# Krual-T/OutfitX

Hardware: AMD Instinct MI355X
Metric: outfits/sec CP forward (8-item sets, 224^2, bf16) (higher is better)
Workload: dtype f16

## Files before the change

### include/ofx.h

```cpp
#ifndef OFX_H
#define OFX_H
#include <stddef.h>
#include <stdint.h>

#ifdef __cplusplus
extern "C" {
#endif

#define OFX_ABI_VERSION 6

enum { OFX_OK = 0, OFX_EINVAL = -1, OFX_ESHAPE = -2, OFX_EHIP = -3, OFX_EWORKSPACE = -4, OFX_ESTATE = -5 };
enum ofx_dtype { OFX_F32 = 0, OFX_BF16 = 1, OFX_F16 = 2 };
enum ofx_act { OFX_ACT_NONE = 0, OFX_ACT_QUICK_GELU = 1, OFX_ACT_GELU = 2, OFX_ACT_MISH = 3, OFX_ACT_MISH_GRAD = 4 };
enum ofx_precision { OFX_PREC_BF16 = 0, OFX_PREC_F16 = 1, OFX_PREC_BF16X3 = 2, OFX_PREC_F16W2 = 3 };
enum ofx_out_kind { OFX_OUT_F32 = 0, OFX_OUT_OP = 1, OFX_OUT_SPLIT3 = 2 };

typedef struct ofx_handle ofx_handle;
typedef void* ofx_stream;

const char* ofx_last_error(void);
int ofx_abi_version(void);

typedef struct ofx_model_desc {
    int d_model, n_head, d_ffn, n_layers, max_items;
// ... 36 lines not shown
int ofx_clip_text_fwd_shared(ofx_handle* h, const int64_t* ids, const int64_t* attn_mask, const int* lengths_host,
                             int N, int T, float* emb, int emb_ld, int emb_col, int normalize, int shared_first, void* ws,
                             size_t ws_bytes, ofx_stream stream);

int ofx_fitb_argmin(const float* y_hat, const float* cand, int B, int C, int D, int64_t* idx, float* dist,
                    ofx_stream stream);
int ofx_fitb_argmin_indexed(const float* table, int ld, long long n_table, const int* cand_index, const float* y_hat, int B, int C, int D,
                            const int64_t* answer, int64_t* idx, float* dist, int* n_correct, ofx_stream stream);
int ofx_l2_topk(ofx_handle* h, const float* Q, const float* P, int nq, int np, int D, int k, int64_t index_base,
                int64_t* idx, float* dist, void* ws, size_t ws_bytes, ofx_stream stream);
size_t ofx_l2_topk_grouped_ws(int nq, int np, int max_group_rows);
int ofx_l2_topk_grouped(ofx_handle* h, const float* Q, const float* P, int nq, int np, int D, int k, const int* panels, int n_panels,
                        int max_group_rows, const int64_t* gt, int64_t* idx, float* dist, int* gt_pos, void* ws, size_t ws_bytes,
                        ofx_stream stream);
int ofx_topk_merge(const int64_t* idx_in, const float* dist_in, int parts, int nq, int k, int64_t* idx, float* dist,
                   ofx_stream stream);

size_t ofx_clip_preprocess_ws(const int* heights, const int* widths, int N, int channels, int size);
int ofx_clip_preprocess(const uint8_t* src, const long long* offsets, const int* heights, const int* widths, int N, int channels, int size,
                        const float* mean, const float* stdv, float* out, void* ws, size_t ws_bytes, ofx_stream stream);
int ofx_clip_preprocess_patches(const uint8_t* src, const long long* offsets, const int* heights, const int* widths, int N, int channels, int size,
                                int patch, const float* mean, const float* stdv, void* patches, int op_dtype, void* ws, size_t ws_bytes,
                                ofx_stream stream);
int ofx_patchify(const float* pixels, void* out, int N, int img, int patch, int op_dtype, ofx_stream stream);
size_t ofx_vit_b32_u8_ws_bytes(ofx_handle* h, const int* heights, const int* widths, int N, int channels);
int ofx_vit_b32_fwd_u8(ofx_handle* h, const uint8_t* src, const long long* offsets, const int* heights, const int* widths, int N, int channels,
                       const float* mean, const float* stdv, float* emb, int emb_ld, int emb_col, int normalize, void* ws, size_t ws_bytes,
                       ofx_stream stream);

int ofx_set_encoder_fwd_indexed(ofx_handle* h, const float* table, int ld, long long n_table, const int* item_index, const int* cu_items,
                                const float* prefix, int prefix_stride, int B, int max_len, float* out_row0, void* ws, size_t ws_bytes,
                                ofx_stream stream);

size_t ofx_cp_train_tape_bytes(ofx_handle* h, int B, int L);
size_t ofx_cp_train_ws_bytes(ofx_handle* h, int B, int L);
size_t ofx_cp_train_grad_floats(ofx_handle* h, size_t* offsets, int n_offsets);
int ofx_cp_train_fwd(ofx_handle* h, const float* x, const uint8_t* pad_mask, int B, int L, float* logits, void* tape, size_t tape_bytes,
                     void* ws, size_t ws_bytes, float dropout_p, unsigned seed, ofx_stream stream);
int ofx_cp_train_bwd(ofx_handle* h, void* tape, size_t tape_bytes, const float* dlogits, int B, int L, float* grads, size_t grad_floats,
                     void* ws, size_t ws_bytes, float dropout_p, unsigned seed, ofx_stream stream);
int ofx_cp_train_fwd_indexed(ofx_handle* h, const float* table, int ld, long long n_table, const int* item_index, const int* cu_items,
                             int B, int max_len, float* logits, void* tape, size_t tape_bytes, void* ws, size_t ws_bytes,
                             float dropout_p, unsigned seed, ofx_stream stream);
int ofx_cir_train_fwd(ofx_handle* h, const float* x, const uint8_t* pad_mask, const float* table, int ld, long long n_table,
                      const int* item_index, const int* cu_items, const float* target_text, int B, int L, float* y, void* tape,
                      size_t tape_bytes, void* ws, size_t ws_bytes, float dropout_p, unsigned seed, ofx_stream stream);
int ofx_cir_train_bwd(ofx_handle* h, void* tape, size_t tape_bytes, const float* dy, int B, int L, float* grads, size_t grad_floats,
                      void* ws, size_t ws_bytes, float dropout_p, unsigned seed, ofx_stream stream);
int ofx_cp_train_bwd_into(ofx_handle* h, void* tape, size_t tape_bytes, const float* dlogits, int B, int L, float* const* grad_ptrs,
                          int n_ptrs, int accumulate, void* ws, size_t ws_bytes, float dropout_p, unsigned seed, ofx_stream stream);
int ofx_cir_train_bwd_into(ofx_handle* h, void* tape, size_t tape_bytes, const float* dy, int B, int L, float* const* grad_ptrs,
                           int n_ptrs, int accumulate, void* ws, size_t ws_bytes, float dropout_p, unsigned seed, ofx_stream stream);
int ofx_train_arm_layer_events(ofx_handle* h, void* const* events, int n);
int ofx_dropout_mask(float dropout_p, unsigned seed, int site, int rows, int cols, float* out, ofx_stream stream);
int ofx_focal_loss(const float* logits, const float* labels, int B, float alpha, float gamma, float upstream, float* loss, float* dlogits,
                   ofx_stream stream);
int ofx_focal_loss_ex(const float* logits, const float* labels, int B, float alpha, float gamma, float upstream, int reduction, float* loss,
                      float* per_elem, float* dlogits, ofx_stream stream);
size_t ofx_set_rank_loss_ws_bytes(int B, int K, int D);
int ofx_set_rank_loss(const float* y, const float* y_hat, const float* neg, const uint8_t* neg_mask, int B, int K, int D, float margin,
                      float upstream, float* loss, float* dy_hat, float* d_pos, float* d_neg, void* ws, size_t ws_bytes, ofx_stream stream);
int ofx_set_rank_loss_indexed(const float* table, int ld, long long n_table, const int* pos_index, const int* neg_index, const float* y_hat,
                              int B, int K, int D, float margin, float upstream, float* loss, float* dy_hat, float* d_pos, float* d_neg,
                              void* ws, size_t ws_bytes, ofx_stream stream);

int ofx_cir_sample_batch(const int* outfit_cu, const int* outfit_rows, int n_outfits, int n_outfit_rows, const int* pos_cu, const int* pos_slots,
                         int n_pos_slots, const int* pool_cu, const int* pool_rows, int n_pools, int n_pool_rows, const int* row_pool,
                         const int* row_slot, int n_table, const int* outfit_ids, int B, unsigned seed, unsigned draw, int K, int max_len,
                         int* item_index, int* cu_seqlens, int* target_item_index, int* neg_items_index, ofx_stream stream);

typedef struct ofx_opt_segment { float* param; long long offset; long long numel; } ofx_opt_segment;
size_t ofx_adamw_step_ws_bytes(long long n_arena);
int ofx_adamw_step(const ofx_opt_segment* segments, int n_segments, float* grad, float* exp_avg, float* exp_avg_sq, long long n_arena,
                   float* step, double lr, double beta1, double beta2, double eps, double weight_decay, double max_norm, double grad_scale,
                   float* grad_norm, int* skipped, void* ws, size_t ws_bytes, ofx_stream stream);

void ofx_profile_enable(int on);
int ofx_profile_read(double* ms, double* flops, long long* launches);
typedef struct ofx_prof_record { int cat, M, N, K, kind, kmul; float ms; double flops; double bytes; } ofx_prof_record;
int ofx_profile_records(ofx_prof_record* out, int cap);

int ofx_tune(int knob, int value);
unsigned ofx_config_generation(void);
int ofx_profile_enabled(void);
int ofx_stream_create_low_priority(int device, ofx_stream* out);
int ofx_stream_destroy(ofx_stream stream);

int ofx_gemm(const void* A, const void* W, void* C, const float* bias, const float* resid, int M, int N, int K,
             int lda, int ldc, int ldr, int act, int out_kind, int op_dtype, ofx_stream stream);
int ofx_gemm_w2(const void* A, const void* W2, void* C, const float* bias, const float* resid, int M, int N, int K,
                int lda, int ldc, int ldr, int act, int out_kind, int op_dtype, ofx_stream stream);
int ofx_gemm_x3(const void* A3, const void* W3, void* C, const float* bias, const float* resid, int M, int N, int K,
                int lda, int ldc, int ldr, int act, int out_kind, int op_dtype, ofx_stream stream);
int ofx_pack_lo8(const void* W2, void* W8, void* scale8, int N, int K, ofx_stream stream);
int ofx_gemm_w2f8(const void* A, const void* W2, const void* W8, const void* scale8, void* C, const float* bias, const float* resid, int M, int N, int K,
                  int lda, int ldc, int ldr, int act, int out_kind, ofx_stream stream);
int ofx_gemm_w2f8_fold(const void* A, const void* W2, const void* W8, const void* scale8, void* C, const float* bias, const float* row_stat, const float* col_sum,
                       int M, int N, int K, int lda, int ldc, int act, ofx_stream stream);
size_t ofx_gemm_tn_ws(int M, int N, int K);
int ofx_gemm_tn(const void* A, int lda, const void* B, int ldb, float* C, int ldc, int M, int N, int K, const int* k_dev,
                void* slab, size_t slab_bytes, int op_dtype, ofx_stream stream);
size_t ofx_gemm_splitk_ws(int M, int N, int K);
int ofx_gemm_splitk(const void* A, const void* W, void* C, const float* bias, const float* resid, int M, int N, int K,
                    int lda, int ldc, int ldr, int act, int out_kind, int op_dtype, void* slab, size_t slab_bytes, ofx_stream stream);
int ofx_gemm_train(const void* A, const void* W, void* C, const float* bias, const float* resid, float* aux_out, int M, const int* m_dev,
                   int N, int K, int lda, int ldc, int ldr, int act, int out_kind, float dropout_p, unsigned seed, int site, int op_dtype,
                   void* slab, size_t slab_bytes, ofx_stream stream);
int ofx_gemm_tn_into(const void* A, int lda, const void* B, int ldb, float* C, int ldc, int M, int N, int K, const int* k_dev,
                     int m_valid, int n_valid, int accumulate, void* slab, size_t slab_bytes, int op_dtype, ofx_stream stream);
int ofx_transpose_cast(const float* src, void* dst, int R, int C, int ldd, void* row_dst, int ld_row, int op_dtype, ofx_stream stream);
size_t ofx_layernorm_bwd_ws(int D);
int ofx_layernorm_bwd(const float* dy, const float* x, const float* stats, const float* gamma, const float* add, const int* add_map,
                      float* dx, void* dx_op, float* dgamma, float* dbeta, float* dcols, int M, const int* m_dev, int D, float dropout_p,
                      unsigned seed, int site, int accumulate, int op_dtype, void* ws, size_t ws_bytes, ofx_stream stream);
size_t ofx_colsum_ws(int C);
int ofx_colsum(const void* x, int x_kind, int ld, const int* gather, const float* row_scale, float* out0, float* out1, float* out2, int seg,
               int C, int valid, int M, const int* m_dev, int accumulate, int op_dtype, void* ws, size_t ws_bytes, ofx_stream stream);
int ofx_head_bwd(const float* dlogits, const float* w, const int* cu, float* dX, void* dXb, float* db, int B, int D, float dropout_p,
                 unsigned seed, int head_site, int below_site, int accumulate, int op_dtype, ofx_stream stream);
int ofx_gemm_fold_producer(const void* A, const void* W, const void* W8, const void* scale8, void* xb, void* xlo, float* stat_part, const float* bias,
                           const float* resid, int M, int N, int K, int lda, int ldr, int act, int w_form, int op_dtype, ofx_stream stream);
int ofx_gemm_fold(const void* A, const void* W, void* C, const float* bias, const float* row_stat, int stat_ld, const float* col_sum, int M, int N, int K,
                  int lda, int ldc, int act, int w_form, int op_dtype, ofx_stream stream);
int ofx_stats_finalize(const float* stat_part, int slots, int W, float eps, float* stat, int rows, ofx_stream stream);
int ofx_row_stats_cast(const float* x, void* xb, void* xlo, float* stat, int rows, int W, float eps, int op_dtype, ofx_stream stream);
int ofx_fold_pack(const float* w, const float* gamma, const float* beta, const float* bias, void* wf, float* col_sum, float* bias_f, int N, int K, int split,
                  int op_dtype, ofx_stream stream);
int ofx_vit_embed_ln(const float* patch_out, const float* cls, const float* pos, const float* gamma, const float* beta, float* x, void* xb, void* xlo,
                     float* stat, int N, int S, int D, float eps, int op_dtype, ofx_stream stream);
int ofx_gather_hilo(const void* hi, const void* lo, const int* idx, float* dst, int rows, int W, int op_dtype, ofx_stream stream);
int ofx_layernorm(const float* x, const int* row_idx, const float* gamma, const float* beta, void* y, int rows,
                  int D, int ldy, int out_kind, int op_dtype, float eps, ofx_stream stream);
int ofx_attention(const void* qkv, void* out, const int64_t* key_mask, int nseq, int seq_len, int n_head, int ld,
                  int ldo, int k_off, int v_off, int mask_ld, int causal, float scale, int op_dtype, ofx_stream stream);
int ofx_attention_ex(const void* qkv, void* out, const int64_t* key_mask, int nseq, int seq_len, int n_head, int ld, int ldo, int k_off,
                     int v_off, int mask_ld, int causal, int only_row0, int split3_w, float scale, int op_dtype, ofx_stream stream);
int ofx_set_attention(const float* qkv, void* out, const int* cu_seqlens, int nseq, int n_head, int D, int ldo,
                      int out_kind, int max_len, int only_row0, float scale, int op_dtype, ofx_stream stream);
int ofx_set_attention_slabs(const float* slabs, size_t plane_floats, int splits, const float* bias, void* out, const int* cu_seqlens, int nseq,
                            int n_head, int D, int ldo, int out_kind, int max_len, int only_row0, float scale, int op_dtype, ofx_stream stream);
int ofx_splitk_reduce_ln(const float* slab, size_t plane_floats, int splits, const float* bias, const float* resid, int ldr, float* x, int ldx,
                         const float* gamma, const float* beta, void* y, int ldy, int out_kind, float eps, int rows, const int* m_dev, int D,
                         int op_dtype, ofx_stream stream);
int ofx_attention_varlen(const void* qkv, void* out, const int* cu_seqlens, int nseq, int max_len, int n_head, int ld, int ldo, int k_off,
                         int v_off, int only_row0, float scale, float dropout_p, unsigned seed, int site, int op_dtype, ofx_stream stream);
int ofx_set_attention_op(const void* qkv, void* out, const int* cu_seqlens, int nseq, int n_head, int D, int ldo, int out_kind, int max_len,
                         int only_row0, float scale, float dropout_p, unsigned seed, int site, int op_dtype, ofx_stream stream);
int ofx_set_attention_bwd(const void* qkv, const float* d_o, void* dqkv, const int* cu_seqlens, int nseq, int n_head, int D, int max_len,
                          int only_row0, float scale, float dropout_p, unsigned seed, int site, int mfma, int op_dtype, ofx_stream stream);
int ofx_fused_qkv_attention(const void* X, const void* Wqkv, const float* bias, const float* row_stat, const float* col_sum, void* out,
                            int nseq, int seq_len, int width, int n_head, int ldx, int ldo, float scale, int op_dtype, ofx_stream stream);
int ofx_fused_qkv_attention_w2(const void* X, const void* Wqkv2, const float* bias, const float* row_stat, const float* col_sum, void* out,
                               int nseq, int seq_len, int width, int n_head, int ldx, int ldo, float scale, int op_dtype, ofx_stream stream);
int ofx_attention_f32(const float* qkv, void* out, const int64_t* key_mask, int nseq, int seq_len, int n_head, int D, int ldo, int out_kind,
                      int mask_ld, int causal, float scale, int op_dtype, ofx_stream stream);
int ofx_convert(const float* src, void* dst, int rows, int cols, int mode, int op_dtype, ofx_stream stream);

#ifdef __cplusplus
}
#endif
#endif
```

### outfitx_amd/_lib.py

```python
from __future__ import annotations

import ctypes as C
import os

_HERE = os.path.dirname(os.path.abspath(__file__))
LIB_PATH = os.environ.get("OFX_LIB") or os.path.join(_HERE, "libofx_hip.so")

OFX_OK = 0
ABI_VERSION = 6
F32, BF16, F16 = 0, 1, 2
ACT_NONE, ACT_QUICK_GELU, ACT_GELU, ACT_MISH = 0, 1, 2, 3
PREC_BF16, PREC_F16, PREC_BF16X3 = 0, 1, 2
OUT_F32, OUT_OP, OUT_SPLIT3 = 0, 1, 2
OP_SET_ENCODER, OP_VIT, OP_TEXT, OP_TOPK = 0, 1, 2, 3
PREC_F16W2 = 3
PRECISIONS = {"bf16": PREC_BF16, "f16": PREC_F16, "fp16": PREC_F16, "bf16x3": PREC_BF16X3, "f16w2": PREC_F16W2}
W2_PATCH, W2_QKV, W2_OUT, W2_FC1, W2_FC2 = 1, 2, 4, 8, 16
TOWER_SCHEMES = {
    "bf16": (PREC_BF16, 0, 0, 0, 0), "f16": (PREC_F16, 0, 0, 0, 0), "fp16": (PREC_F16, 0, 0, 0, 0),
    "f16w2": (PREC_F16, W2_PATCH | W2_OUT | W2_FC2, 1, 1, 0),
    "bf16w2": (PREC_BF16, W2_PATCH | W2_OUT | W2_FC2, 1, 1, 0),
    "f16w2q": (PREC_F16, W2_PATCH | W2_QKV | W2_OUT | W2_FC2, 1, 1, 0),
    "f16w2f": (PREC_F16, W2_PATCH | W2_OUT | W2_FC1 | W2_FC2, 1, 1, 0),
    "f16w2x": (PREC_F16, W2_PATCH | W2_QKV | W2_OUT | W2_FC1 | W2_FC2, 1, 1, 0),
    "f16x3": (PREC_F16, W2_PATCH, 1, 1, 1), "bf16x3": (PREC_BF16, W2_PATCH, 1, 1, 1),
}
SCHEME_ALIASES = {"f16w2h": "f16w2x@qkv=0-5"}
DEFAULT_TOWER_PRECISION = "f16w2x"


def _layer_bits(spec: str) -> int:
    m = 0
    for part in spec.split(","):
        a, _, b = part.partition("-")
        for l in range(int(a), int(b or a) + 1):
            m |= 1 << l
    return m


def tower_scheme(name: str) -> dict:
    name = SCHEME_ALIASES.get(name, name)
    base, _, opts = name.partition("@")
    if base not in TOWER_SCHEMES:
        raise ValueError(f"unknown tower_precision {name!r}; one of {sorted(list(TOWER_SCHEMES) + list(SCHEME_ALIASES))} [+ '@txt=w2;qkv=<layers>;fc1=<layers>']")
    prec, mask, txt_x3, proj_x3, vit_x3 = TOWER_SCHEMES[base]
    d = {"tower_precision": prec, "vit_w2_mask": mask, "txt_x3": txt_x3, "proj_x3": proj_x3, "vit_x3": vit_x3,
         "txt_w2_mask": 0, "vit_w2_qkv_layers": 0, "vit_w2_fc1_layers": 0, "vit_w2_out_layers": 0, "vit_w2_fc2_layers": 0}
    for o in filter(None, opts.split(";")):
        k, _, v = o.partition("=")
        try:
            if k == "txt" and v == "w2":
                d["txt_x3"], d["txt_w2_mask"] = 0, W2_QKV | W2_OUT | W2_FC1 | W2_FC2
            elif k in ("qkv", "fc1", "out", "fc2"):
                bits = _layer_bits(v) if v not in ("", "none") else 0
                if bits == 0:
                    d["vit_w2_mask"] &= ~{"qkv": W2_QKV, "fc1": W2_FC1, "out": W2_OUT, "fc2": W2_FC2}[k]
                d[f"vit_w2_{k}_layers"] = bits
            else:
                raise ValueError
        except ValueError:
            raise ValueError(f"tower_precision {name!r}: bad option {o!r} (txt=w2 | qkv= / fc1= / out= / fc2=<layers>, layers like 0-5,8 or none)") from None
    return d
ACTS = {"none": ACT_NONE, "quick_gelu": ACT_QUICK_GELU, "gelu": ACT_GELU, "mish": ACT_MISH}


class OfxError(RuntimeError):
    pass


class ModelDesc(C.Structure):
    _fields_ = [(n, C.c_int) for n in (
        "d_model", "n_head", "d_ffn", "n_layers", "max_items", "outfit_act", "outfit_precision",
        "vit_width", "vit_layers", "vit_heads", "vit_mlp", "vit_patch", "vit_image", "vit_act",
        "txt_width", "txt_layers", "txt_heads", "txt_mlp", "txt_vocab", "txt_max_pos", "txt_act", "txt_eos_id",
        "proj_dim", "tower_precision")] + [("ln_eps", C.c_float)] + [(n, C.c_int) for n in ("vit_w2_mask", "txt_x3", "proj_x3", "vit_x3", "txt_w2_mask", "vit_w2_qkv_layers", "vit_w2_fc1_layers", "vit_w2_out_layers", "vit_w2_fc2_layers")]


class OptSegment(C.Structure):
    _fields_ = [("param", C.c_void_p), ("offset", C.c_longlong), ("numel", C.c_longlong)]


class ProfRecord(C.Structure):
    _fields_ = [("cat", C.c_int), ("M", C.c_int), ("N", C.c_int), ("K", C.c_int), ("kind", C.c_int), ("kmul", C.c_int), ("ms", C.c_float), ("flops", C.c_double), ("bytes", C.c_double)]


_vp, _i, _f, _sz, _i64 = C.c_void_p, C.c_int, C.c_float, C.c_size_t, C.c_int64

SIGNATURES = {
    "ofx_last_error": (C.c_char_p, []),
    "ofx_abi_version": (_i, []),
    "ofx_stream_create_low_priority": (_i, [_i, C.POINTER(_vp)]),
    "ofx_stream_destroy": (_i, [_vp]),
    "ofx_default_desc": (None, [C.POINTER(ModelDesc)]),
    "ofx_create": (_vp, [_i, C.POINTER(ModelDesc)]),
    "ofx_destroy": (None, [_vp]),
    "ofx_pack_outfit_weights": (_i, [_vp, C.POINTER(_vp), _i, _vp]),
    "ofx_pack_vision_weights": (_i, [_vp, C.POINTER(_vp), _i, _vp]),
    "ofx_pack_text_weights": (_i, [_vp, C.POINTER(_vp), _i, _vp]),
    "ofx_workspace_bytes": (_sz, [_vp, _i, _i, _i]),
    "ofx_set_encoder_fwd": (_i, [_vp, _vp, _vp, _vp, _i, _i, _i, _vp, _vp, _sz, _vp]),
    "ofx_cp_head": (_i, [_vp, _vp, _i, _vp, _vp]),
    "ofx_cir_head": (_i, [_vp, _vp, _i, _vp, _vp, _sz, _vp]),
    "ofx_cir_prefix": (_i, [_vp, _vp, _i, _vp, _vp]),
    "ofx_vit_b32_fwd": (_i, [_vp, _vp, _i, _vp, _i, _i, _i, _vp, _sz, _vp]),
    "ofx_clip_text_fwd": (_i, [_vp, _vp, _vp, C.POINTER(_i), _i, _i, _vp, _i, _i, _i, _vp, _sz, _vp]),
    "ofx_clip_text_fwd_shared": (_i, [_vp, _vp, _vp, C.POINTER(_i), _i, _i, _vp, _i, _i, _i, _i, _vp, _sz, _vp]),
    "ofx_fitb_argmin": (_i, [_vp, _vp, _i, _i, _i, _vp, _vp, _vp]),
    "ofx_fitb_argmin_indexed": (_i, [_vp, _i, C.c_longlong, _vp, _vp, _i, _i, _i, _vp, _vp, _vp, _vp, _vp]),
    "ofx_l2_topk": (_i, [_vp, _vp, _vp, _i, _i, _i, _i, _i64, _vp, _vp, _vp, _sz, _vp]),
    "ofx_l2_topk_grouped_ws": (_sz, [_i, _i, _i]),
    "ofx_l2_topk_grouped": (_i, [_vp, _vp, _vp, _i, _i, _i, _i, _vp, _i, _i, _vp, _vp, _vp, _vp, _vp, _sz, _vp]),
    "ofx_topk_merge": (_i, [_vp, _vp, _i, _i, _i, _vp, _vp, _vp]),
    "ofx_clip_preprocess_ws": (_sz, [_vp, _vp, _i, _i, _i]),
    "ofx_clip_preprocess": (_i, [_vp, _vp, _vp, _vp, _i, _i, _i, _vp, _vp, _vp, _vp, _sz, _vp]),
    "ofx_clip_preprocess_patches": (_i, [_vp, _vp, _vp, _vp, _i, _i, _i, _i, _vp, _vp, _vp, _i, _vp, _sz, _vp]),
    "ofx_patchify": (_i, [_vp, _vp, _i, _i, _i, _i, _vp]),
    "ofx_vit_b32_u8_ws_bytes": (_sz, [_vp, _vp, _vp, _i, _i]),
    "ofx_vit_b32_fwd_u8": (_i, [_vp, _vp, _vp, _vp, _vp, _i, _i, _vp, _vp, _vp, _i, _i, _i, _vp, _sz, _vp]),
    "ofx_set_encoder_fwd_indexed": (_i, [_vp, _vp, _i, C.c_longlong, _vp, _vp, _vp, _i, _i, _i, _vp, _vp, _sz, _vp]),
    "ofx_cp_train_fwd_indexed": (_i, [_vp, _vp, _i, C.c_longlong, _vp, _vp, _i, _i, _vp, _vp, _sz, _vp, _sz, _f, C.c_uint, _vp]),
    "ofx_cp_train_tape_bytes": (_sz, [_vp, _i, _i]),
    "ofx_cp_train_ws_bytes": (_sz, [_vp, _i, _i]),
    "ofx_cp_train_grad_floats": (_sz, [_vp, C.POINTER(_sz), _i]),
    "ofx_cp_train_fwd": (_i, [_vp, _vp, _vp, _i, _i, _vp, _vp, _sz, _vp, _sz, _f, C.c_uint, _vp]),
    "ofx_cp_train_bwd": (_i, [_vp, _vp, _sz, _vp, _i, _i, _vp, _sz, _vp, _sz, _f, C.c_uint, _vp]),
    "ofx_cir_train_fwd": (_i, [_vp, _vp, _vp, _vp, _i, C.c_longlong, _vp, _vp, _vp, _i, _i, _vp, _vp, _sz, _vp, _sz, _f, C.c_uint, _vp]),
    "ofx_cir_train_bwd": (_i, [_vp, _vp, _sz, _vp, _i, _i, _vp, _sz, _vp, _sz, _f, C.c_uint, _vp]),
    "ofx_cp_train_bwd_into": (_i, [_vp, _vp, _sz, _vp, _i, _i, C.POINTER(_vp), _i, _i, _vp, _sz, _f, C.c_uint, _vp]),
    "ofx_cir_train_bwd_into": (_i, [_vp, _vp, _sz, _vp, _i, _i, C.POINTER(_vp), _i, _i, _vp, _sz, _f, C.c_uint, _vp]),
    "ofx_train_arm_layer_events": (_i, [_vp, C.POINTER(_vp), _i]),
    "ofx_dropout_mask": (_i, [_f, C.c_uint, _i, _i, _i, _vp, _vp]),
    "ofx_focal_loss": (_i, [_vp, _vp, _i, _f, _f, _f, _vp, _vp, _vp]),
    "ofx_focal_loss_ex": (_i, [_vp, _vp, _i, _f, _f, _f, _i, _vp, _vp, _vp, _vp]),
    "ofx_set_rank_loss_ws_bytes": (_sz, [_i, _i, _i]),
    "ofx_set_rank_loss": (_i, [_vp, _vp, _vp, _vp, _i, _i, _i, _f, _f, _vp, _vp, _vp, _vp, _vp, _sz, _vp]),
    "ofx_set_rank_loss_indexed": (_i, [_vp, _i, C.c_longlong, _vp, _vp, _vp, _i, _i, _i, _f, _f, _vp, _vp, _vp, _vp, _vp, _sz, _vp]),
    "ofx_cir_sample_batch": (_i, [_vp, _vp, _i, _i, _vp, _vp, _i, _vp, _vp, _i, _i, _vp, _vp, _i, _vp, _i, C.c_uint, C.c_uint, _i, _i, _vp, _vp, _vp, _vp, _vp]),
    "ofx_adamw_step_ws_bytes": (_sz, [C.c_longlong]),
    "ofx_adamw_step": (_i, [_vp, _i, _vp, _vp, _vp, C.c_longlong, _vp] + [C.c_double] * 7 + [_vp, _vp, _vp, _sz, _vp]),
    "ofx_profile_enable": (None, [_i]),
    "ofx_profile_read": (_i, [C.POINTER(C.c_double), C.POINTER(C.c_double), C.POINTER(C.c_longlong)]),
    "ofx_profile_records": (_i, [C.POINTER(ProfRecord), _i]),
    "ofx_tune": (_i, [_i, _i]),
    "ofx_config_generation": (C.c_uint, []),
    "ofx_profile_enabled": (_i, []),
    "ofx_gemm": (_i, [_vp, _vp, _vp, _vp, _vp, _i, _i, _i, _i, _i, _i, _i, _i, _i, _vp]),
    "ofx_gemm_w2": (_i, [_vp, _vp, _vp, _vp, _vp, _i, _i, _i, _i, _i, _i, _i, _i, _i, _vp]),
    "ofx_gemm_x3": (_i, [_vp, _vp, _vp, _vp, _vp, _i, _i, _i, _i, _i, _i, _i, _i, _i, _vp]),
    "ofx_pack_lo8": (_i, [_vp, _vp, _vp, _i, _i, _vp]),
    "ofx_gemm_w2f8": (_i, [_vp, _vp, _vp, _vp, _vp, _vp, _vp, _i, _i, _i, _i, _i, _i, _i, _i, _vp]),
    "ofx_gemm_w2f8_fold": (_i, [_vp, _vp, _vp, _vp, _vp, _vp, _vp, _vp, _i, _i, _i, _i, _i, _i, _vp]),
    "ofx_gemm_tn_ws": (_sz, [_i, _i, _i]),
    "ofx_gemm_tn": (_i, [_vp, _i, _vp, _i, _vp, _i, _i, _i, _i, _vp, _vp, _sz, _i, _vp]),
    "ofx_gemm_splitk_ws": (_sz, [_i, _i, _i]),
    "ofx_gemm_splitk": (_i, [_vp, _vp, _vp, _vp, _vp, _i, _i, _i, _i, _i, _i, _i, _i, _i, _vp, _sz, _vp]),
    "ofx_gemm_train": (_i, [_vp, _vp, _vp, _vp, _vp, _vp, _i, _vp, _i, _i, _i, _i, _i, _i, _i, _f, C.c_uint, _i, _i, _vp, _sz, _vp]),
    "ofx_gemm_tn_into": (_i, [_vp, _i, _vp, _i, _vp, _i, _i, _i, _i, _vp, _i, _i, _i, _vp, _sz, _i, _vp]),
    "ofx_transpose_cast": (_i, [_vp, _vp, _i, _i, _i, _vp, _i, _i, _vp]),
    "ofx_layernorm_bwd_ws": (_sz, [_i]),
    "ofx_layernorm_bwd": (_i, [_vp] * 11 + [_i, _vp, _i, _f, C.c_uint, _i, _i, _i, _vp, _sz, _vp]),
    "ofx_colsum_ws": (_sz, [_i]),
    "ofx_colsum": (_i, [_vp, _i, _i, _vp, _vp, _vp, _vp, _vp, _i, _i, _i, _i, _vp, _i, _i, _vp, _sz, _vp]),
    "ofx_head_bwd": (_i, [_vp, _vp, _vp, _vp, _vp, _vp, _i, _i, _f, C.c_uint, _i, _i, _i, _i, _vp]),
    "ofx_gemm_fold_producer": (_i, [_vp] * 9 + [_i] * 8 + [_vp]),
    "ofx_gemm_fold": (_i, [_vp, _vp, _vp, _vp, _vp, _i, _vp, _i, _i, _i, _i, _i, _i, _i, _i, _vp]),
    "ofx_stats_finalize": (_i, [_vp, _i, _i, _f, _vp, _i, _vp]),
    "ofx_row_stats_cast": (_i, [_vp, _vp, _vp, _vp, _i, _i, _f, _i, _vp]),
    "ofx_fold_pack": (_i, [_vp] * 7 + [_i, _i, _i, _i, _vp]),
    "ofx_vit_embed_ln": (_i, [_vp] * 9 + [_i, _i, _i, _f, _i, _vp]),
    "ofx_gather_hilo": (_i, [_vp, _vp, _vp, _vp, _i, _i, _i, _vp]),
    "ofx_layernorm": (_i, [_vp, _vp, _vp, _vp, _vp, _i, _i, _i, _i, _i, _f, _vp]),
    "ofx_attention": (_i, [_vp, _vp, _vp, _i, _i, _i, _i, _i, _i, _i, _i, _i, _f, _i, _vp]),
    "ofx_attention_ex": (_i, [_vp, _vp, _vp, _i, _i, _i, _i, _i, _i, _i, _i, _i, _i, _i, _f, _i, _vp]),
    "ofx_set_attention_slabs": (_i, [_vp, _sz, _i, _vp, _vp, _vp, _i, _i, _i, _i, _i, _i, _i, _f, _i, _vp]),
    "ofx_splitk_reduce_ln": (_i, [_vp, _sz, _i, _vp, _vp, _i, _vp, _i, _vp, _vp, _vp, _i, _i, _f, _i, _vp, _i, _i, _vp]),
    "ofx_fused_qkv_attention": (_i, [_vp, _vp, _vp, _vp, _vp, _vp, _i, _i, _i, _i, _i, _i, _f, _i, _vp]),
    "ofx_fused_qkv_attention_w2": (_i, [_vp, _vp, _vp, _vp, _vp, _vp, _i, _i, _i, _i, _i, _i, _f, _i, _vp]),
    "ofx_set_attention": (_i, [_vp, _vp, _vp, _i, _i, _i, _i, _i, _i, _i, _f, _i, _vp]),
    "ofx_attention_varlen": (_i, [_vp, _vp, _vp, _i, _i, _i, _i, _i, _i, _i, _i, _f, _f, C.c_uint, _i, _i, _vp]),
    "ofx_set_attention_op": (_i, [_vp, _vp, _vp, _i, _i, _i, _i, _i, _i, _i, _f, _f, C.c_uint, _i, _i, _vp]),
    "ofx_set_attention_bwd": (_i, [_vp, _vp, _vp, _vp, _i, _i, _i, _i, _i, _f, _f, C.c_uint, _i, _i, _i, _vp]),
    "ofx_attention_f32": (_i, [_vp, _vp, _vp, _i, _i, _i, _i, _i, _i, _i, _i, _f, _i, _vp]),
    "ofx_convert": (_i, [_vp, _vp, _i, _i, _i, _i, _vp]),
}

_lib = None


def load() -> C.CDLL:
    global _lib
    if _lib is not None:
        return _lib
    if not os.path.exists(LIB_PATH):
        raise OfxError(f"{LIB_PATH} not found: build it with `make` (or __graft_entry__.build()); "
                       "outfitx_amd has no CPU/PyTorch fallback for the scoring path")
    lib = C.CDLL(LIB_PATH)
    for name, (res, args) in SIGNATURES.items():
        fn = getattr(lib, name)
        fn.restype, fn.argtypes = res, args
    if lib.ofx_abi_version() != ABI_VERSION:
        raise OfxError("libofx_hip.so ABI version mismatch; rebuild")
    for kv in filter(None, os.environ.get("OFX_TUNE", "").split(",")):
        knob, _, val = kv.partition(":")
        if lib.ofx_tune(int(knob), int(val)) != OFX_OK:
            raise OfxError(f"OFX_TUNE: ofx_tune({knob}, {val}) was refused")
    _lib = lib
    return lib


def check(rc: int, what: str = "") -> None:
    if rc != OFX_OK:
        msg = load().ofx_last_error()
        raise OfxError(f"{what or 'ofx call'} failed (code {rc}): {msg.decode() if msg else ''}")


def default_desc() -> ModelDesc:
    d = ModelDesc()
    load().ofx_default_desc(C.byref(d))
    return d
```

### outfitx_amd/csrc/api.hip

```cpp
#include <stdarg.h>
#include <string.h>

#include <algorithm>
#include <vector>
#include <mutex>
#include <cstring>

#include "ofx_weights.h"

static thread_local char g_err[512] = "";
void ofx_set_error(const char* fmt, ...) {
    va_list ap;
    va_start(ap, fmt);
    vsnprintf(g_err, sizeof(g_err), fmt, ap);
    va_end(ap);
}
extern "C" const char* ofx_last_error(void) { return g_err; }
extern "C" int ofx_abi_version(void) { return OFX_ABI_VERSION; }
extern "C" int ofx_stream_create_low_priority(int device, ofx_stream* out) {
    OFX_REQUIRE(out, OFX_EINVAL, "stream_create_low_priority: NULL argument");
    int prev = 0, least = 0, greatest = 0;
    OFX_HIP(hipGetDevice(&prev));
    OFX_HIP(hipSetDevice(device));
    hipStream_t s = nullptr;
// ... 340 lines not shown
    size_t r = carve_clip(b, (size_t)n * Tc, n, d.txt_width, d.txt_mlp, d.proj_dim, 0, 0, w, h->txt_x3 ? 3 : 1, h->txt_x3 ? 3 : (h->txt_w2_mask ? 2 : 1), true);
    return align_up(r, 256);
}
constexpr int VIT_CHUNK_MAX = 2048;
}

extern "C" size_t ofx_workspace_bytes(ofx_handle* h, int op, int n, int len) {
    if (!h || n <= 0) return 0;
    switch (op) {
        case OFX_OP_SET_ENCODER: { Bump b(nullptr, ~(size_t)0); return align_up(carve_set(h, b, n, len, nullptr), 256); }
        case OFX_OP_VIT: return vit_bytes(h, std::min(n, VIT_CHUNK_MAX), nullptr, nullptr, ~(size_t)0);
        case OFX_OP_TEXT: return txt_bytes(h, n, len, nullptr, nullptr, ~(size_t)0);
        case OFX_OP_TOPK: return ofx_l2_topk_ws(n, len);
        default: return 0;
    }
}

int g_set_fuse = 3;
int g_train_mfma_attn = 1;

struct SetInput {
    const float* x = nullptr; const uint8_t* pad_mask = nullptr;
    const float* table = nullptr; int ld = 0; long long n_table = 0; const int* item_index = nullptr; const int* cu_items = nullptr;
};
static SetInput dense_set(const float* x, const uint8_t* pad_mask) { SetInput in; in.x = x; in.pad_mask = pad_mask; return in; }
static SetInput indexed_set(const float* table, int ld, long long n_table, const int* item_index, const int* cu_items) {
    SetInput in; in.table = table; in.ld = ld; in.n_table = n_table; in.item_index = item_index; in.cu_items = cu_items;
    return in;
}
static int build_set(const ofx_handle* h, const SetInput& in, const float* prefix, int prefix_stride, int* cu, float* X, int B, int L, hipStream_t s) {
    const int D = h->d.d_model;
    if (in.table) return ofx_launch_set_build_indexed(in.table, in.ld, in.n_table, in.item_index, in.cu_items, prefix, prefix_stride, cu, X, B, D, s);
    return ofx_launch_set_build(in.x, in.pad_mask, prefix, prefix_stride, cu, X, B, L, D, s);
}
static int set_encoder_core(ofx_handle* h, const SetInput& in, const float* prefix, int prefix_stride, int B, int L, float* out_row0, void* ws,
                            size_t ws_bytes, hipStream_t s);
static float set_attn_scale(const ofx_model_desc& d) { return 1.0f / sqrtf((float)(d.d_model / d.n_head)); }
static bool ln_bwd_d_ok(int D);
static bool train_shape_ok(const ofx_model_desc& d) { return d.d_model == d.n_head * 64 && ln_bwd_d_ok(d.d_model); }
#define OFX_REQUIRE_TRAIN_SHAPE(h, who) \
    OFX_REQUIRE(!(h) || train_shape_ok((h)->d), OFX_ESHAPE, who ": training needs heads of 64 and d_model in {512, 768, 1024} (d_model=%d, n_head=%d scores only)", (h)->d.d_model, (h)->d.n_head)

extern "C" int ofx_set_encoder_fwd(ofx_handle* h, const float* x, const uint8_t* pad_mask, const float* prefix,
                                   int prefix_stride, int B, int L, float* out_row0, void* ws, size_t ws_bytes,
                                   ofx_stream stream) {
    OFX_REQUIRE(h && h->out_ready, OFX_ESTATE, "set_encoder_fwd: outfit weights not packed");
    OFX_REQUIRE(B > 0 && L >= 0 && L <= 63, OFX_ESHAPE, "set_encoder_fwd: B=%d L=%d (L must be in [0,63])", B, L);
    OFX_REQUIRE((x || L == 0) && (pad_mask || L == 0) && out_row0 && ws, OFX_EINVAL, "set_encoder_fwd: NULL argument");
    return set_encoder_core(h, dense_set(x, pad_mask), prefix, prefix_stride, B, L, out_row0, ws, ws_bytes, (hipStream_t)stream);
}
extern "C" int ofx_set_encoder_fwd_indexed(ofx_handle* h, const float* table, int ld, long long n_table, const int* item_index, const int* cu_items,
                                           const float* prefix, int prefix_stride, int B, int max_len, float* out_row0, void* ws, size_t ws_bytes,
                                           ofx_stream stream) {
    OFX_REQUIRE(h && h->out_ready, OFX_ESTATE, "set_encoder_fwd_indexed: outfit weights not packed");
    OFX_REQUIRE(B > 0 && max_len >= 0 && max_len <= 63, OFX_ESHAPE, "set_encoder_fwd_indexed: B=%d max_len=%d (must be in [0,63])", B, max_len);
    OFX_REQUIRE(table && item_index && cu_items && out_row0 && ws && n_table > 0, OFX_EINVAL, "set_encoder_fwd_indexed: NULL argument");
    return set_encoder_core(h, indexed_set(table, ld, n_table, item_index, cu_items), prefix, prefix_stride, B, max_len, out_row0, ws, ws_bytes, (hipStream_t)stream);
}
static int set_encoder_core(ofx_handle* h, const SetInput& in, const float* prefix, int prefix_stride, int B, int L, float* out_row0, void* ws,
                            size_t ws_bytes, hipStream_t s) {
    const ofx_model_desc& d = h->d;
    Bump bump(ws, ws_bytes);
    SetWs w;
    carve_set(h, bump, B, L, &w);
    OFX_REQUIRE(bump.ok, OFX_EWORKSPACE, "set_encoder_fwd: workspace %zu < %zu bytes", ws_bytes, bump.off);
    const int D = d.d_model, km = a_kmul(h->ot_form), Fp = h->ot_ffn_pad, dt = h->ot_dtype, M = B * (L + 1);
    const int okind = km == 3 ? OFX_OUT_SPLIT3 : OFX_OUT_OP;
    const float scale = set_attn_scale(d);
    auto slab_gemm = [&](const PackedGemm& c, int K) { GemmArgs g{}; use_gemm(g, c, K); g.slab = w.slab; g.slab_bytes = w.slab_bytes; return g; };
    if (!prefix) { prefix = h->outfit_token; prefix_stride = 0; }
    TRY(build_set(h, in, prefix, prefix_stride, w.cu, w.X, B, L, s));
    const int* m_dev = w.cu + B;
    const bool fuse_att = (g_set_fuse & 1) != 0 && L + 1 <= 32, fuse = (g_set_fuse & 2) != 0;
    bool ln1_done = false;
    for (int l = 0; l < d.n_layers; ++l) {
        const OutfitLayer& Ly = h->ol[l];
        const bool last = l + 1 == d.n_layers;
        if (!ln1_done) {
            LnArgs ln{w.X, nullptr, Ly.g1, Ly.be1, w.H, M, D, km * D, okind, d.ln_eps};
            TRY(ofx_launch_layernorm_dev(ln, m_dev, dt, s));
        }
        ln1_done = false;
        GemmArgs g1 = slab_gemm(Ly.in, D);
        g1.A = w.H; g1.C = w.QKV; g1.m_dev = m_dev; g1.M = M; g1.N = 3 * D; g1.ldc = 3 * D;
        const bool mfma_attn = h->ot_form == W_PLAIN && g_train_mfma_attn && D == d.n_head * 64;
        g1.out_kind = mfma_attn ? OFX_OUT_OP : OFX_OUT_F32;
        int qkv_splits = 1;
        if (fuse_att && !mfma_attn) g1.defer_splits = &qkv_splits;
        TRY(ofx_launch_gemm(g1, dt, s));
        if (mfma_attn) {
            AttnArgs at{w.QKV, w.H, nullptr, B, L + 1, d.n_head, 3 * D, D, D, 2 * D, 0, 0, scale};
            at.cu_seqlens = w.cu; at.only_row0 = last ? 1 : 0;
            TRY(ofx_launch_attention_mfma(at, dt, s));
        } else {
            SetAttnArgs sa{w.QKV, w.H, w.cu, B, d.n_head, D, km * D, okind, L + 1, last ? 1 : 0, scale};
            if (qkv_splits > 1) { sa.qkv = w.slab; sa.splits = qkv_splits; sa.plane = (size_t)M * 3 * D; sa.bias = g1.bias; }
            TRY(ofx_launch_set_attention(sa, dt, s));
        }
        float* X = w.X; char* H = w.H; char* U = w.U; int Ml = M; const int* md = m_dev;
        if (last) {
            TRY(ofx_launch_gather_rows(w.H, w.cu, w.HP, B, km * D * 2, km * D * 2, s));
            TRY(ofx_launch_gather_rows(w.X, w.cu, out_row0, B, D * 4, D * 4, s));
            X = out_row0; H = w.HP; U = w.UP; Ml = B; md = nullptr;
        }
        GemmArgs g2 = slab_gemm(Ly.out, D);
        g2.A = H; g2.C = X; g2.resid = X; g2.m_dev = md; g2.M = Ml; g2.N = D; g2.ldc = D; g2.ldr = D; g2.out_kind = OFX_OUT_F32;
        bool ln2_done = false;
        if (fuse) { g2.ln_gamma = Ly.g2; g2.ln_beta = Ly.be2; g2.ln_out = H; g2.ln_ld = km * D; g2.ln_kind = okind; g2.ln_eps = d.ln_eps; g2.ln_done = &ln2_done; }
        TRY(ofx_launch_gemm(g2, dt, s));
        if (!ln2_done) {
            LnArgs ln2{X, nullptr, Ly.g2, Ly.be2, H, Ml, D, km * D, okind, d.ln_eps};
            TRY(ofx_launch_layernorm_dev(ln2, md, dt, s));
        }
        GemmArgs g3 = slab_gemm(Ly.l1, D);
        g3.A = H; g3.C = U; g3.m_dev = md; g3.M = Ml; g3.N = Fp; g3.ldc = km * Fp; g3.act = d.outfit_act; g3.out_kind = okind;
        TRY(ofx_launch_gemm(g3, dt, s));
        GemmArgs g4 = slab_gemm(Ly.l2, Fp);
        g4.A = U; g4.C = X; g4.resid = X; g4.m_dev = md; g4.M = Ml; g4.N = D; g4.ldc = D; g4.ldr = D; g4.out_kind = OFX_OUT_F32;
        if (fuse && !last) {
            const OutfitLayer& Nx = h->ol[l + 1];
            g4.ln_gamma = Nx.g1; g4.ln_beta = Nx.be1; g4.ln_out = w.H; g4.ln_ld = km * D; g4.ln_kind = okind; g4.ln_eps = d.ln_eps; g4.ln_done = &ln1_done;
        }
        TRY(ofx_launch_gemm(g4, dt, s));
    }
    return OFX_OK;
}

extern "C" int ofx_cp_head(ofx_handle* h, const float* row0, int B, float* logits, ofx_stream stream) {
    OFX_REQUIRE(h && h->out_ready, OFX_ESTATE, "cp_head: outfit weights not packed");
    OFX_REQUIRE(row0 && logits && B > 0, OFX_EINVAL, "cp_head: bad argument");
    return ofx_launch_cp_head(row0, h->cp_w, h->cp_b, logits, B, h->d.d_model, (hipStream_t)stream);
}

extern "C" int ofx_cir_head(ofx_handle* h, const float* row0, int B, float* emb, void* ws, size_t ws_bytes, ofx_stream stream) {
    OFX_REQUIRE(h && h->out_ready, OFX_ESTATE, "cir_head: outfit weights not packed");
    OFX_REQUIRE(row0 && emb && B > 0 && ws, OFX_EINVAL, "cir_head: bad argument");
    const int D = h->d.d_model, km = a_kmul(h->ot_form);
    OFX_REQUIRE(ws_bytes >= (size_t)B * km * D * 2, OFX_EWORKSPACE, "cir_head: workspace too small");
    hipStream_t s = (hipStream_t)stream;
    TRY(ofx_launch_pack_rows(row0, ws, B, B, D, D, D, km == 3 ? 1 : 0, h->ot_dtype, s));
    GemmArgs g{};
    use_cir_head(g, *h);
    g.A = ws; g.C = emb; g.M = B; g.N = D; g.ldc = D; g.out_kind = OFX_OUT_F32;
    return ofx_launch_gemm(g, h->ot_dtype, s);
}

extern "C" int ofx_cir_prefix(ofx_handle* h, const float* txt, int B, float* out, ofx_stream stream) {
    OFX_REQUIRE(h && h->out_ready, OFX_ESTATE, "cir_prefix: outfit weights not packed");
    OFX_REQUIRE(txt && out && B > 0, OFX_EINVAL, "cir_prefix: bad argument");
    return ofx_launch_cir_prefix(h->tgt_img_emb, txt, out, B, h->d.d_model, (hipStream_t)stream);
}

int g_fuse_qkv = 1;
int g_x3_vit_f32_attn = 0;
int g_prune_q = 1;

static int clip_layer(const ClipLayer& L, const ClipWs& w, int rows, int nseq, int S, int W, int MLP, int heads, int act,
                      float eps, int causal, const int64_t* key_mask, int mask_ld, int dt, const int* pool_idx, hipStream_t s, bool pool_first) {
    const bool fused = (g_fuse_qkv & (L.qkv.form == W_SPLIT ? 2 : 1)) && !pool_idx && !causal && !key_mask && S >= 33 && S <= 64 && (256 / S - 1) * S + 64 - 256 <= 16;
    if (fused) {
        TRY(ofx_launch_fused_qkv_attn(w.XB, L.qkv.w, L.qkv.bias, w.S, L.qkv.col_sum, w.H, nseq, S, W, heads, W, W, 0.125f, dt, s, L.qkv.form == W_SPLIT));
    } else {
        GemmArgs g1{}; g1.A = w.XB; g1.C = w.QKV; g1.row_stat = w.S; g1.M = rows; g1.N = 3 * W;
        g1.ldc = 3 * W; g1.act = OFX_ACT_NONE; g1.out_kind = OFX_OUT_OP;
        use_gemm(g1, L.qkv, W);
        const bool prune = pool_idx && pool_first && g_prune_q;
        if (prune) {
            GemmArgs kv = g1;
            kv.W = (const char*)g1.W + (size_t)W * g1.K * 2; kv.bias = g1.bias + W; kv.col_sum = g1.col_sum + W; kv.C = (char*)w.QKV + (size_t)W * 2; kv.N = 2 * W;
            if (g1.W8) { kv.W8 = (const char*)g1.W8 + (size_t)W * W; kv.w8_scale = (const char*)g1.w8_scale + W; }
            TRY(ofx_launch_gemm(kv, dt, s));
            GemmArgs q = g1;
            q.M = nseq; q.N = W; q.lda = S * W; q.ldc = S * 3 * W; q.stat_ld = S;
            TRY(ofx_launch_gemm(q, dt, s));
        } else
            TRY(ofx_launch_gemm(g1, dt, s));
        AttnArgs at{w.QKV, w.H, key_mask, nseq, S, heads, 3 * W, W, W, 2 * W, mask_ld, causal, 0.125f};
        at.only_row0 = prune ? 1 : 0;
        TRY(ofx_launch_attention_mfma(at, dt, s));
    }
    char* H = w.H; char* U = w.U; int M = rows;
    if (pool_idx) {
        TRY(ofx_launch_gather_rows(w.H, pool_idx, w.HP, nseq, W * 2, W * 2, s));
        TRY(ofx_launch_gather_hilo(w.XB, w.XLO, pool_idx, w.XP, nseq, W, dt, s));
        H = w.HP; U = w.UP; M = nseq;
    }
    auto to_stream = [&](GemmArgs& g) {
        g.M = M; g.N = W; g.ldc = W; g.ldr = W; g.act = OFX_ACT_NONE;
        if (pool_idx) { g.C = w.XP; g.resid = w.XP; g.out_kind = OFX_OUT_F32; g.slab = w.slab; g.slab_bytes = w.slab_bytes; }
        else { g.C = w.XB; g.xb_out = w.XB; g.xlo = w.XLO; g.stat_part = w.P; g.out_kind = OFX_OUT_OP; }
    };
    GemmArgs g2{}; g2.A = H;
    use_gemm(g2, L.o, W); to_stream(g2);
    TRY(ofx_launch_gemm(g2, dt, s));
    GemmArgs g3{}; g3.C = U; g3.M = M; g3.N = MLP; g3.ldc = MLP; g3.act = act; g3.out_kind = OFX_OUT_OP;
    if (pool_idx) {
        LnArgs ln2{w.XP, nullptr, L.g2, L.be2, H, M, W, W, OFX_OUT_OP, eps};
        TRY(ofx_launch_layernorm(ln2, dt, s));
        g3.A = H; g3.slab = w.slab; g3.slab_bytes = w.slab_bytes;
    } else {
        TRY(ofx_launch_stats_finalize(w.P, W / 64, W, eps, w.S, M, s));
        g3.A = w.XB; g3.row_stat = w.S;
    }
    use_gemm(g3, L.fc1, W);
    TRY(ofx_launch_gemm(g3, dt, s));
    GemmArgs g4{}; g4.A = U;
    use_gemm(g4, L.fc2, MLP); to_stream(g4);
    TRY(ofx_launch_gemm(g4, dt, s));
    if (!pool_idx) TRY(ofx_launch_stats_finalize(w.P, W / 64, W, eps, w.S, M, s));
    return OFX_OK;
}

static int clip_layer_x3(const ClipLayer& L, const ClipWs& w, int rows, int nseq, int S, int W, int MLP, int heads, int act,
                         float eps, int causal, const int64_t* key_mask, int mask_ld, int dt, const int* pool_idx, hipStream_t s, bool mfma_attn = false,
                         int shared_first = 0) {
    LnArgs ln{w.X, nullptr, L.g1, L.be1, w.H, rows, W, 3 * W, OFX_OUT_SPLIT3, eps};
    TRY(ofx_launch_layernorm(ln, dt, s));
    GemmArgs g1{}; g1.A = w.H; g1.C = w.QKV; g1.M = rows; g1.N = 3 * W;
    use_gemm(g1, L.qkv, W);
    const bool f32_attn = S <= 64 && !mfma_attn;
    OFX_REQUIRE(!shared_first || f32_attn, OFX_EINVAL, "clip_layer_x3: a shared first row needs the fp32 set attention");
    g1.ldc = 3 * W; g1.act = OFX_ACT_NONE; g1.out_kind = f32_attn ? OFX_OUT_F32 : OFX_OUT_OP;
    TRY(ofx_launch_gemm(g1, dt, s));
    if (f32_attn) {
        SetAttnArgs sa{w.QKV, w.H, nullptr, nseq, heads, W, 3 * W, OFX_OUT_SPLIT3, S, 0, 0.125f};
        sa.fixed_len = S; sa.causal = causal; sa.key_mask = key_mask; sa.mask_ld = mask_ld; sa.shared_first = shared_first;
        TRY(ofx_launch_set_attention(sa, dt, s));
    } else {
        AttnArgs at{w.QKV, w.H, key_mask, nseq, S, heads, 3 * W, 3 * W, W, 2 * W, mask_ld, causal, 0.125f};
        at.split3_w = W;
        TRY(ofx_launch_attention_mfma(at, dt, s));
    }
    float* X = w.X; char* H = w.H; char* U = w.U; int M = rows;
    if (pool_idx) {
        TRY(ofx_launch_gather_rows(w.H, pool_idx, w.HP, nseq, 3 * W * 2, 3 * W * 2, s));
        TRY(ofx_launch_gather_rows(w.X, pool_idx, w.XP, nseq, W * 4, W * 4, s));
        X = w.XP; H = w.HP; U = w.UP; M = nseq;
    }
    GemmArgs g2{}; g2.A = H; g2.C = X; g2.resid = X; g2.M = M; g2.N = W; g2.ldc = W; g2.ldr = W; g2.act = OFX_ACT_NONE; g2.out_kind = OFX_OUT_F32;
    use_gemm(g2, L.o, W);
    if (pool_idx) { g2.slab = w.slab; g2.slab_bytes = w.slab_bytes; }
    TRY(ofx_launch_gemm(g2, dt, s));
    LnArgs ln2{X, nullptr, L.g2, L.be2, H, M, W, 3 * W, OFX_OUT_SPLIT3, eps};
    TRY(ofx_launch_layernorm(ln2, dt, s));
    GemmArgs g3{}; g3.A = H; g3.C = U; g3.M = M; g3.N = MLP; g3.ldc = 3 * MLP; g3.act = act; g3.out_kind = OFX_OUT_SPLIT3;
    use_gemm(g3, L.fc1, W);
    if (pool_idx) { g3.slab = w.slab; g3.slab_bytes = w.slab_bytes; }
    TRY(ofx_launch_gemm(g3, dt, s));
    GemmArgs g4{}; g4.A = U; g4.C = X; g4.resid = X; g4.M = M; g4.N = W; g4.ldc = W; g4.ldr = W; g4.act = OFX_ACT_NONE; g4.out_kind = OFX_OUT_F32;
    use_gemm(g4, L.fc2, MLP);
    if (pool_idx) { g4.slab = w.slab; g4.slab_bytes = w.slab_bytes; }
    return ofx_launch_gemm(g4, dt, s);
}

static int clip_layers(const std::vector<ClipLayer>& Ls, const ClipWs& w, int rows, int nseq, int S, int W, int MLP,
                       int heads, int act, float eps, int causal, const int64_t* key_mask, int mask_ld, int dt,
                       const int* pool_idx, hipStream_t s, bool pool_first, bool x3, int shared_first = 0) {
    OFX_REQUIRE(!shared_first || x3, OFX_EINVAL, "clip_layers: a shared first row exists in the three-product path only");
    if (x3) {
        for (size_t l = 0; l < Ls.size(); ++l)
            TRY(clip_layer_x3(Ls[l], w, rows, nseq, S, W, MLP, heads, act, eps, causal, key_mask, mask_ld, dt, l + 1 == Ls.size() ? pool_idx : nullptr, s, !causal && !key_mask && !g_x3_vit_f32_attn,
                              shared_first));
        return OFX_OK;
    }
    for (size_t l = 0; l < Ls.size(); ++l)
        TRY(clip_layer(Ls[l], w, rows, nseq, S, W, MLP, heads, act, eps, causal, key_mask, mask_ld, dt,
                       l + 1 == Ls.size() ? pool_idx : nullptr, s, pool_first));
    return OFX_OK;
}

struct RawImages {
    const uint8_t* src; const long long* offsets; const int* heights; const int* widths; int channels; const float* mean; const float* stdv;
    void* ws; size_t ws_bytes;
};

static int vit_core(ofx_handle* h, const float* pixels, const RawImages* raw, int N, float* emb, int emb_ld, int emb_col,
                    int normalize, void* ws, size_t ws_bytes, ofx_stream stream) {
    OFX_REQUIRE(h && h->vis_ready, OFX_ESTATE, "vit_b32_fwd: vision weights not packed");
    OFX_REQUIRE((pixels || raw) && emb && ws && N > 0, OFX_EINVAL, "vit_b32_fwd: bad argument");
    const ofx_model_desc& d = h->d;
    OFX_REQUIRE(emb_ld >= emb_col + d.proj_dim && emb_ld % 4 == 0 && emb_col % 4 == 0, OFX_ESHAPE, "vit_b32_fwd: bad emb_ld/emb_col");
    hipStream_t s = (hipStream_t)stream;
    const int g = d.vit_image / d.vit_patch, S = g * g + 1, W = d.vit_width, KP = 3 * d.vit_patch * d.vit_patch, dt = h->tw_dtype;
    int chunk = std::min(N, VIT_CHUNK_MAX);
    while (chunk > 1 && vit_bytes(h, chunk, nullptr, nullptr, ~(size_t)0) > ws_bytes) chunk = (chunk + 1) / 2;
    OFX_REQUIRE(vit_bytes(h, chunk, nullptr, nullptr, ~(size_t)0) <= ws_bytes, OFX_EWORKSPACE, "vit_b32_fwd: workspace %zu bytes cannot hold one image", ws_bytes);
    const size_t px_per_img = (size_t)3 * d.vit_image * d.vit_image;
    for (int n0 = 0; n0 < N; n0 += chunk) {
        const int n = std::min(chunk, N - n0);
        ClipWs w;
        vit_bytes(h, n, &w, ws, ws_bytes);
        const int rows = n * S;
        if (raw)
            TRY(ofx_preprocess_to(raw->src, raw->offsets + n0, raw->heights + n0, raw->widths + n0, n, raw->channels, d.vit_image, raw->mean, raw->stdv,
                                  nullptr, w.U, d.vit_patch, dt, raw->ws, raw->ws_bytes, s));
        else
            TRY(ofx_launch_patchify(pixels + (size_t)n0 * px_per_img, w.U, n, d.vit_image, d.vit_patch, dt, s));
        GemmArgs gp{}; gp.A = w.U; gp.C = w.QKV; gp.M = n * g * g; gp.N = W; gp.ldc = W;
        gp.act = OFX_ACT_NONE; gp.out_kind = OFX_OUT_F32;
        use_gemm(gp, h->v_patch, KP);
        TRY(ofx_launch_gemm(gp, dt, s));
        TRY(ofx_launch_vit_embed_ln((const float*)w.QKV, h->v_cls, h->v_pos, h->v_pre_g, h->v_pre_b, w.X, n, S, W, d.ln_eps, s, w.XB, w.S, dt, w.XLO));
        TRY(ofx_launch_iota_rows(w.idx, n, S, s));
        TRY(clip_layers(h->vl, w, rows, n, S, W, d.vit_mlp, d.vit_heads, d.vit_act, d.ln_eps, 0, nullptr, 0, dt, w.idx, s, true, h->vit_x3 != 0));
        const int pk = h->proj_x3 ? 3 : 1;
        LnArgs ln{w.XP, nullptr, h->v_post_g, h->v_post_b, w.PL, n, W, pk * W, pk == 3 ? OFX_OUT_SPLIT3 : OFX_OUT_OP, d.ln_eps};
        TRY(ofx_launch_layernorm(ln, dt, s));
        GemmArgs gj{}; gj.A = w.PL; gj.C = w.E; gj.M = n; gj.N = d.proj_dim; gj.ldc = d.proj_dim;
        use_gemm(gj, h->v_proj, W);
        gj.act = OFX_ACT_NONE; gj.out_kind = OFX_OUT_F32; gj.slab = w.slab; gj.slab_bytes = w.slab_bytes;
        TRY(ofx_launch_gemm(gj, dt, s));
        TRY(ofx_launch_l2norm_store(w.E, emb + (size_t)n0 * emb_ld, n, d.proj_dim, emb_ld, emb_col, normalize, s));
    }
    return OFX_OK;
}

extern "C" int ofx_vit_b32_fwd(ofx_handle* h, const float* pixels, int N, float* emb, int emb_ld, int emb_col,
                               int normalize, void* ws, size_t ws_bytes, ofx_stream stream) {
// ... 316 lines not shown
        return ofx_launch_gemm_tn(dY, n_w, X, k_w, out, ldc ? ldc : k_w, n_w, k_w, rows, md, w.slab, w.slab_bytes, dt, s, mv, nv, acc);
    };
    auto dgrad = [&](int rows, const int* md, const void* dY, const PackedGemm& rec, void* C, int n, int k, int out_kind = OFX_OUT_F32, int act = OFX_ACT_NONE,
                     const float* resid = nullptr, const DropArgs& drop = DropArgs()) {
        PackedGemm wt; wt.w = rec.wt;
        GemmArgs g{}; use_gemm(g, wt, k); g.slab = w.slab; g.slab_bytes = w.slab_bytes;
        g.A = dY; g.C = C; g.M = rows; g.N = n; g.ldc = n; g.out_kind = out_kind; g.act = act; g.resid = resid; g.ldr = resid ? n : 0; g.m_dev = md; g.drop = drop;
        return ofx_launch_gemm(g, dt, s);
    };
    const auto attention_bwd = g_train_mfma_attn ? ofx_launch_set_attention_bwd_mfma : ofx_launch_set_attention_bwd;
    float* dX = w.dXa; float* dX2 = w.dXb_f;
    const int lastl = d.n_layers - 1;
    if (head == 1) {
        TRY(ofx_launch_pack_rows(dlogits, w.dyb, B, B, D, D, D, 0, dt, s));
        TRY(wgrad(B, nullptr, w.dyb, D, T.row0b, D, G(4)));
        TRY(dgrad(B, nullptr, w.dyb, h->cir, w.d_row0, D, D));
        TRY(ofx_launch_cp_head_bwd(nullptr, w.d_row0, nullptr, w.d_row0, w.gXb, nullptr, B, D, dt, nodrop, site(lastl, 3), s));
    } else {
        TRY(ofx_launch_cp_head_bwd(dlogits, h->cp_w, nullptr, w.d_row0, w.gXb, G(3), B, D, dt, site(d.n_layers, 0), site(lastl, 3), s, acc));
        TRY(ofx_launch_colsum(T.row0, 0, D, nullptr, dlogits, G(2), nullptr, nullptr, D, w.part, D, nullptr, B, dt, s, 0, acc));
    }
    TRY(ofx_launch_row_map(T.cu, w.rowmap, B, M, s));
    for (int l = lastl; l >= 0; --l) {
        const OutfitLayer& Ly = h->ol[l];
        const TapeLayer& t = T.L[l];
        const int g0 = 5 + 12 * l;
        const bool last = l == lastl;
        const int rows = last ? B : M;
        const int* md = last ? nullptr : m_dev;
        const void* O = last ? T.pO : t.O;
        const float* dXout = last ? w.d_row0 : dX;
        if (last) TRY(ofx_launch_colsum(w.gXb, 1, D, nullptr, nullptr, G(g0 + 7), nullptr, nullptr, D, w.part, D, nullptr, B, dt, s, 0, acc));
        TRY(wgrad(rows, md, w.gXb, D, t.A, Fp, G(g0 + 6), Fv, D, Fv));
        TRY(dgrad(rows, md, w.gXb, Ly.l2, w.dU, Fp, D, OFX_OUT_OP, OFX_ACT_MISH_GRAD, t.Upre, site(l, 2)));
        TRY(ofx_launch_colsum(w.dU, 1, Fp, nullptr, nullptr, G(g0 + 5), nullptr, nullptr, Fp, w.part, Fp, md, rows, dt, s, Fv, acc));
        TRY(wgrad(rows, md, w.dU, Fp, t.H2, D, G(g0 + 4), D, Fv, D));
        TRY(dgrad(rows, md, w.dU, Ly.l1, w.dH, D, Fp));
        TRY(ofx_launch_ln_bwd(w.dH, t.Xmid, t.st2, Ly.g2, dXout, nullptr, dX2, w.gXb, G(g0 + 10), G(g0 + 11), G(g0 + 3), w.part, D, md, rows, dt, site(l, 1), s, acc));
        TRY(wgrad(rows, md, w.gXb, D, O, D, G(g0 + 2)));
        TRY(dgrad(rows, md, w.gXb, Ly.out, w.dO, D, D));
        TRY(attention_bwd(t.QKV, w.dO, w.gQb, T.cu, B, d.n_head, D, L + 1, set_attn_scale(d), dt, site(l, 0), last ? 1 : 0, s));
        TRY(ofx_launch_colsum(w.gQb, 1, 3 * D, nullptr, nullptr, G(g0 + 1), nullptr, nullptr, 3 * D, w.part, 3 * D, m_dev, M, dt, s, 0, acc));
        TRY(wgrad(M, m_dev, w.gQb, 3 * D, t.H1, D, G(g0 + 0)));
        TRY(dgrad(M, m_dev, w.gQb, Ly.in, w.dH, D, 3 * D));
        TRY(ofx_launch_ln_bwd(w.dH, t.Xin, t.st1, Ly.g1, dX2, last ? w.rowmap : nullptr, dX, w.gXb, G(g0 + 8), G(g0 + 9), l > 0 ? G(g0 - 12 + 7) : nullptr, w.part, D,
                              m_dev, M, dt, l > 0 ? site(l - 1, 3) : nodrop, s, acc));
        if (!layer_ev.empty()) OFX_HIP(hipEventRecord(layer_ev[l], s));
    }
    if (head == 1) return ofx_launch_colsum(dX, 0, D, T.cu, nullptr, G(1), nullptr, nullptr, D / 2, w.part, D / 2, nullptr, B, dt, s, 0, acc);
    return ofx_launch_colsum(dX, 0, D, T.cu, nullptr, G(0), nullptr, nullptr, D, w.part, D, nullptr, B, dt, s, 0, acc);
}

extern "C" int ofx_dropout_mask(float dropout_p, unsigned seed, int site, int rows, int cols, float* out, ofx_stream stream) {
    OFX_REQUIRE(out && rows > 0 && cols > 0 && dropout_p >= 0.f && dropout_p < 1.f, OFX_EINVAL, "dropout_mask: bad argument");
    hipStream_t s = (hipStream_t)stream;
    TRY(ofx_launch_fill_f32(out, (size_t)rows * cols, 1.0f, s));
    return ofx_launch_drop_rows(out, rows, cols, make_drop(dropout_p, seed, (unsigned)site), s);
}

extern "C" int ofx_focal_loss(const float* logits, const float* labels, int B, float alpha, float gamma, float upstream, float* loss, float* dlogits,
                              ofx_stream stream) {
    OFX_REQUIRE(logits && labels && B > 0, OFX_EINVAL, "focal_loss: bad argument");
    return ofx_launch_focal_loss(logits, labels, B, alpha, gamma, upstream, loss, dlogits, (hipStream_t)stream);
}
extern "C" int ofx_focal_loss_ex(const float* logits, const float* labels, int B, float alpha, float gamma, float upstream, int reduction, float* loss,
                                 float* per_elem, float* dlogits, ofx_stream stream) {
    OFX_REQUIRE(logits && labels && B > 0 && reduction >= 0 && reduction <= 2, OFX_EINVAL, "focal_loss_ex: bad argument");
    OFX_REQUIRE(reduction != 0 || per_elem, OFX_EINVAL, "focal_loss_ex: reduction 'none' needs per_elem");
    return ofx_launch_focal_loss(logits, labels, B, alpha, gamma, upstream, loss, dlogits, (hipStream_t)stream, reduction, per_elem);
}

static bool rank_loss_shape_ok(int B, int K, int D) { return B >= 1 && K >= 0 && D >= 4 && D <= 4096 && D % 4 == 0; }
extern "C" size_t ofx_set_rank_loss_ws_bytes(int B, int K, int D) { return rank_loss_shape_ok(B, K, D) ? ofx_set_rank_loss_ws(B, K) : 0; }
extern "C" int ofx_set_rank_loss(const float* y, const float* y_hat, const float* neg, const uint8_t* neg_mask, int B, int K, int D, float margin,
                                 float upstream, float* loss, float* dy_hat, float* d_pos, float* d_neg, void* ws, size_t ws_bytes, ofx_stream stream) {
    OFX_REQUIRE(rank_loss_shape_ok(B, K, D), OFX_ESHAPE, "set_rank_loss: B = %d, K = %d, D = %d; needs B >= 1, K >= 0, D %% 4 == 0, 4 <= D <= 4096", B, K, D);
    OFX_REQUIRE(y && y_hat && loss && ws && (neg || K == 0), OFX_EINVAL, "set_rank_loss: NULL argument");
    OFX_REQUIRE((((uintptr_t)y | (uintptr_t)y_hat | (uintptr_t)neg | (uintptr_t)dy_hat | (uintptr_t)ws) & 15) == 0, OFX_EINVAL,
                "set_rank_loss: y, y_hat, neg, dy_hat and ws must be 16-byte aligned");
    OFX_REQUIRE(ws_bytes >= ofx_set_rank_loss_ws(B, K), OFX_EWORKSPACE, "set_rank_loss: workspace %zu < %zu bytes", ws_bytes, ofx_set_rank_loss_ws(B, K));
    return ofx_launch_set_rank_loss(y, y_hat, neg, neg_mask, B, K, D, margin, upstream, loss, dy_hat, d_pos, d_neg, ws, (hipStream_t)stream);
}

extern "C" int ofx_set_rank_loss_indexed(const float* table, int ld, long long n_table, const int* pos_index, const int* neg_index, const float* y_hat,
                                         int B, int K, int D, float margin, float upstream, float* loss, float* dy_hat, float* d_pos, float* d_neg,
                                         void* ws, size_t ws_bytes, ofx_stream stream) {
    OFX_REQUIRE(rank_loss_shape_ok(B, K, D), OFX_ESHAPE,
                "set_rank_loss_indexed: B = %d, K = %d, D = %d; needs B >= 1, K >= 0, D %% 4 == 0, 4 <= D <= 4096", B, K, D);
    OFX_REQUIRE(ld >= D && ld % 4 == 0 && n_table >= 1 && n_table <= INT_MAX, OFX_ESHAPE,
                "set_rank_loss_indexed: ld = %d, n_table = %lld; needs ld >= D = %d, ld %% 4 == 0, 1 <= n_table <= INT_MAX", ld, n_table, D);
    OFX_REQUIRE(table && pos_index && y_hat && loss && ws && (neg_index || K == 0), OFX_EINVAL, "set_rank_loss_indexed: NULL argument");
    OFX_REQUIRE((((uintptr_t)table | (uintptr_t)y_hat | (uintptr_t)dy_hat | (uintptr_t)ws) & 15) == 0 &&
                    (((uintptr_t)pos_index | (uintptr_t)neg_index) & 3) == 0,
                OFX_EINVAL, "set_rank_loss_indexed: table, y_hat, dy_hat and ws must be 16-byte aligned, the index arrays 4-byte aligned");
    OFX_REQUIRE(ws_bytes >= ofx_set_rank_loss_ws(B, K), OFX_EWORKSPACE, "set_rank_loss_indexed: workspace %zu < %zu bytes", ws_bytes,
                ofx_set_rank_loss_ws(B, K));
    return ofx_launch_set_rank_loss_indexed(table, ld, (int)n_table, pos_index, neg_index, y_hat, B, K, D, margin, upstream, loss, dy_hat, d_pos, d_neg, ws,
                                            (hipStream_t)stream);
}

extern "C" int ofx_cir_sample_batch(const int* outfit_cu, const int* outfit_rows, int n_outfits, int n_outfit_rows, const int* pos_cu, const int* pos_slots,
                                    int n_pos_slots, const int* pool_cu, const int* pool_rows, int n_pools, int n_pool_rows, const int* row_pool,
                                    const int* row_slot, int n_table, const int* outfit_ids, int B, unsigned seed, unsigned draw, int K, int max_len,
                                    int* item_index, int* cu_seqlens, int* target_item_index, int* neg_items_index, ofx_stream stream) {
    OFX_REQUIRE(B >= 1, OFX_EINVAL, "cir_sample_batch: B = %d; needs B >= 1", B);
    OFX_REQUIRE(K >= 0 && K <= 64 && max_len >= 1 && max_len <= 31, OFX_ESHAPE, "cir_sample_batch: K = %d, max_len = %d; needs 0 <= K <= 64, 1 <= max_len <= 31",
                K, max_len);
    OFX_REQUIRE(n_outfits >= 1 && n_table >= 1 && n_outfit_rows >= 0 && n_pos_slots >= 0 && n_pools >= 0 && n_pool_rows >= 0, OFX_ESHAPE,
                "cir_sample_batch: n_outfits = %d, n_table = %d (both >= 1), n_outfit_rows = %d, n_pos_slots = %d, n_pools = %d, n_pool_rows = %d (all >= 0)",
                n_outfits, n_table, n_outfit_rows, n_pos_slots, n_pools, n_pool_rows);
    OFX_REQUIRE((long long)B * std::max(K, max_len) <= INT_MAX, OFX_ESHAPE, "cir_sample_batch: B * max(K, max_len) = %lld exceeds INT_MAX",
                (long long)B * std::max(K, max_len));
    const void* ptrs[] = {outfit_cu, outfit_rows, pos_cu, pos_slots, pool_cu, pool_rows, row_pool, row_slot, outfit_ids, item_index, cu_seqlens, target_item_index};
    uintptr_t bits = (uintptr_t)neg_items_index;
    for (const void* p : ptrs) {
        OFX_REQUIRE(p, OFX_EINVAL, "cir_sample_batch: NULL argument");
        bits |= (uintptr_t)p;
    }
    OFX_REQUIRE(neg_items_index || K == 0, OFX_EINVAL, "cir_sample_batch: NULL neg_items_index with K = %d", K);
    OFX_REQUIRE((bits & 15) == 0, OFX_EINVAL, "cir_sample_batch: every array must be 16-byte aligned");
    CirSampleArgs a{outfit_cu, outfit_rows, pos_cu, pos_slots, pool_cu, pool_rows, row_pool, row_slot, outfit_ids,
                    n_outfits, n_outfit_rows, n_pos_slots, n_pools, n_pool_rows, n_table, B, K, max_len, seed, draw,
                    item_index, cu_seqlens, target_item_index, neg_items_index};
    return ofx_launch_cir_sample_batch(a, (hipStream_t)stream);
}

static bool adamw_shape_ok(long long n_arena) { return n_arena > 0 && n_arena % 64 == 0; }
extern "C" size_t ofx_adamw_step_ws_bytes(long long n_arena) { return adamw_shape_ok(n_arena) ? ofx_adamw_step_ws(n_arena) : 0; }
extern "C" int ofx_adamw_step(const ofx_opt_segment* segments, int n_segments, float* grad, float* exp_avg, float* exp_avg_sq, long long n_arena,
                              float* step, double lr, double beta1, double beta2, double eps, double weight_decay, double max_norm, double grad_scale,
                              float* grad_norm, int* skipped, void* ws, size_t ws_bytes, ofx_stream stream) {
    OFX_REQUIRE(segments && grad && exp_avg && exp_avg_sq && step && grad_norm && skipped && ws, OFX_EINVAL, "adamw_step: NULL argument");
    OFX_REQUIRE(n_segments >= 1 && n_segments <= 1024, OFX_ESHAPE, "adamw_step: n_segments = %d; needs 1 <= n_segments <= 1024", n_segments);
    OFX_REQUIRE(adamw_shape_ok(n_arena), OFX_ESHAPE, "adamw_step: n_arena = %lld; needs a positive multiple of 64", n_arena);
    OFX_REQUIRE((((uintptr_t)grad | (uintptr_t)exp_avg | (uintptr_t)exp_avg_sq | (uintptr_t)ws) & 15) == 0 && ((uintptr_t)segments & 7) == 0, OFX_EINVAL,
                "adamw_step: grad, exp_avg, exp_avg_sq and ws must be 16-byte aligned, segments 8-byte aligned");
    OFX_REQUIRE(ws_bytes >= ofx_adamw_step_ws(n_arena), OFX_EWORKSPACE, "adamw_step: workspace %zu < %zu bytes", ws_bytes, ofx_adamw_step_ws(n_arena));
    return ofx_launch_adamw_step(segments, n_segments, grad, exp_avg, exp_avg_sq, n_arena, step, lr, beta1, beta2, eps, weight_decay, max_norm,
                                 grad_scale, grad_norm, skipped, ws, (hipStream_t)stream);
}

extern "C" int ofx_tune(int knob, int value) {
    ++g_config_generation;
    switch (knob) {
        case 2: case 5: case 11: case 15: case 16: case 18: return ofx_gemm_tune(knob, value);
        case 6: if (value != 2) { ofx_set_error("ofx_tune(6): %d is not 2 (the towers' LayerNorms are always folded)", value); return OFX_EINVAL; } return OFX_OK;
        case 7: g_train_mfma_attn = value; return OFX_OK;
        case 8: g_prune_q = value; return OFX_OK;
        case 9: g_fuse_qkv = value; return OFX_OK;
        case 10: g_set_fuse = value; return OFX_OK;
        case 17: g_topk_filter = value != 0; return OFX_OK;
        case 20: g_x3_vit_f32_attn = value != 0; return OFX_OK;
        case 21: g_text_shared_first = value != 0; return OFX_OK;
        default: ofx_set_error("ofx_tune: unknown knob %d", knob); return OFX_EINVAL;
    }
}

static GemmArgs op_gemm(const void* A, const void* W, void* C, const float* bias, const float* resid, int M, int N, int K, int lda, int ldc, int ldr,
                        int act, int out_kind) {
    GemmArgs g{}; g.A = A; g.W = W; g.C = C; g.bias = bias; g.resid = resid; g.M = M; g.N = N; g.K = K; g.lda = lda; g.ldc = ldc;
    g.ldr = ldr; g.act = act; g.out_kind = out_kind;
    return g;
}
extern "C" int ofx_gemm(const void* A, const void* W, void* C, const float* bias, const float* resid, int M, int N, int K,
                        int lda, int ldc, int ldr, int act, int out_kind, int op_dtype, ofx_stream stream) {
    return ofx_launch_gemm(op_gemm(A, W, C, bias, resid, M, N, K, lda, ldc, ldr, act, out_kind), op_dtype, (hipStream_t)stream);
}
extern "C" int ofx_gemm_w2(const void* A, const void* W2, void* C, const float* bias, const float* resid, int M, int N, int K,
                           int lda, int ldc, int ldr, int act, int out_kind, int op_dtype, ofx_stream stream) {
    GemmArgs g = op_gemm(A, W2, C, bias, resid, M, N, 2 * K, lda, ldc, ldr, act, out_kind); g.a_wrap = K;
    return ofx_launch_gemm(g, op_dtype, (hipStream_t)stream);
}
extern "C" int ofx_gemm_x3(const void* A3, const void* W3, void* C, const float* bias, const float* resid, int M, int N, int K,
                           int lda, int ldc, int ldr, int act, int out_kind, int op_dtype, ofx_stream stream) {
    GemmArgs g = op_gemm(A3, W3, C, bias, resid, M, N, 3 * K, lda, ldc, ldr, act, out_kind); g.k_mult = 3;
    return ofx_launch_gemm(g, op_dtype, (hipStream_t)stream);
}
extern "C" int ofx_pack_lo8(const void* W2, void* W8, void* scale8, int N, int K, ofx_stream stream) {
    return ofx_launch_pack_lo8(W2, W8, scale8, N, K, (hipStream_t)stream);
}
extern "C" int ofx_gemm_w2f8(const void* A, const void* W2, const void* W8, const void* scale8, void* C, const float* bias, const float* resid, int M, int N, int K,
                             int lda, int ldc, int ldr, int act, int out_kind, ofx_stream stream) {
    GemmArgs g = op_gemm(A, W2, C, bias, resid, M, N, 2 * K, lda, ldc, ldr, act, out_kind); g.a_wrap = K; g.W8 = W8; g.w8_scale = scale8;
    return ofx_launch_gemm(g, OFX_F16, (hipStream_t)stream);
}
extern "C" int ofx_gemm_w2f8_fold(const void* A, const void* W2, const void* W8, const void* scale8, void* C, const float* bias, const float* row_stat, const float* col_sum,
                                  int M, int N, int K, int lda, int ldc, int act, ofx_stream stream) {
    OFX_REQUIRE(row_stat && col_sum, OFX_EINVAL, "gemm_w2f8_fold: row_stat and col_sum are required");
    GemmArgs g = op_gemm(A, W2, C, bias, nullptr, M, N, 2 * K, lda, ldc, 0, act, OFX_OUT_OP); g.a_wrap = K; g.W8 = W8; g.w8_scale = scale8;
    g.row_stat = row_stat; g.col_sum = col_sum; g.stat_ld = 1;
    return ofx_launch_gemm(g, OFX_F16, (hipStream_t)stream);
}
extern "C" size_t ofx_gemm_splitk_ws(int M, int N, int K) { return ofx_gemm_splitk_bytes(M, N, K); }
extern "C" int ofx_gemm_splitk(const void* A, const void* W, void* C, const float* bias, const float* resid, int M, int N, int K,
                               int lda, int ldc, int ldr, int act, int out_kind, int op_dtype, void* slab, size_t slab_bytes, ofx_stream stream) {
    GemmArgs g = op_gemm(A, W, C, bias, resid, M, N, K, lda, ldc, ldr, act, out_kind); g.slab = slab; g.slab_bytes = slab_bytes;
    return ofx_launch_gemm(g, op_dtype, (hipStream_t)stream);
}
extern "C" size_t ofx_gemm_tn_ws(int M, int N, int K) { return ofx_gemm_tn_slab_bytes(M, N, K); }
extern "C" int ofx_gemm_tn(const void* A, int lda, const void* B, int ldb, float* C, int ldc, int M, int N, int K, const int* k_dev,
                           void* slab, size_t slab_bytes, int op_dtype, ofx_stream stream) {
    return ofx_launch_gemm_tn(A, lda, B, ldb, C, ldc, M, N, K, k_dev, slab, slab_bytes, op_dtype, (hipStream_t)stream);
}
static bool op_dtype_ok(int op_dtype) { return op_dtype == OFX_BF16 || op_dtype == OFX_F16; }
static bool drop_p_ok(float p) { return p >= 0.f && p < 1.f; }
static bool aligned_to(size_t mask, std::initializer_list<const void*> ptrs) {
    for (const void* p : ptrs) if ((uintptr_t)p & mask) return false;
    return true;
}
extern "C" int ofx_gemm_train(const void* A, const void* W, void* C, const float* bias, const float* resid, float* aux_out, int M, const int* m_dev,
                              int N, int K, int lda, int ldc, int ldr, int act, int out_kind, float dropout_p, unsigned seed, int site, int op_dtype,
                              void* slab, size_t slab_bytes, ofx_stream stream) {
    OFX_REQUIRE(A && W && C && drop_p_ok(dropout_p) && (act != OFX_ACT_MISH_GRAD || resid), OFX_EINVAL, "gemm_train: bad argument");
    OFX_REQUIRE(aligned_to(15, {bias, resid, aux_out, slab}) && aligned_to(3, {m_dev}), OFX_EINVAL,
                "gemm_train: bias, resid, aux_out and slab must be 16-byte aligned");
    GemmArgs g = op_gemm(A, W, C, bias, resid, M, N, K, lda, ldc, ldr, act, out_kind); g.slab = slab; g.slab_bytes = slab_bytes;
    g.aux_out = aux_out; g.m_dev = m_dev; g.drop = make_drop(dropout_p, seed, (unsigned)site);
    return ofx_launch_gemm(g, op_dtype, (hipStream_t)stream);
}
extern "C" int ofx_gemm_tn_into(const void* A, int lda, const void* B, int ldb, float* C, int ldc, int M, int N, int K, const int* k_dev,
                                int m_valid, int n_valid, int accumulate, void* slab, size_t slab_bytes, int op_dtype, ofx_stream stream) {
    OFX_REQUIRE(A && B && C && m_valid >= 0 && n_valid >= 0, OFX_EINVAL, "gemm_tn_into: bad argument");
    OFX_REQUIRE(aligned_to(15, {slab}) && aligned_to(3, {k_dev}), OFX_EINVAL, "gemm_tn_into: slab must be 16-byte aligned");
    return ofx_launch_gemm_tn(A, lda, B, ldb, C, ldc, M, N, K, k_dev, slab, slab_bytes, op_dtype, (hipStream_t)stream, m_valid, n_valid, accumulate ? 1 : 0);
}
extern "C" int ofx_transpose_cast(const float* src, void* dst, int R, int C, int ldd, void* row_dst, int ld_row, int op_dtype, ofx_stream stream) {
    OFX_REQUIRE(src && dst && op_dtype_ok(op_dtype), OFX_EINVAL, "transpose_cast: bad argument");
    OFX_REQUIRE(aligned_to(3, {src}) && aligned_to(1, {dst, row_dst}), OFX_EINVAL, "transpose_cast: misaligned pointer");
    OFX_REQUIRE(R > 0 && C > 0, OFX_ESHAPE, "transpose_cast: R=%d C=%d", R, C);
    return ofx_launch_transpose_cast(src, dst, R, C, ldd, op_dtype, (hipStream_t)stream, row_dst, ld_row);
}
static bool ln_bwd_d_ok(int D) { return D == 512 || D == 768 || D == 1024; }
extern "C" size_t ofx_layernorm_bwd_ws(int D) { return ln_bwd_d_ok(D) ? ofx_ln_bwd_part_floats(D) * sizeof(float) : 0; }
extern "C" int ofx_layernorm_bwd(const float* dy, const float* x, const float* stats, const float* gamma, const float* add, const int* add_map,
                                 float* dx, void* dx_op, float* dgamma, float* dbeta, float* dcols, int M, const int* m_dev, int D, float dropout_p,
                                 unsigned seed, int site, int accumulate, int op_dtype, void* ws, size_t ws_bytes, ofx_stream stream) {
    OFX_REQUIRE(dy && x && stats && gamma && dx && dx_op && ws && (add || !add_map) && drop_p_ok(dropout_p) && op_dtype_ok(op_dtype), OFX_EINVAL,
                "layernorm_bwd: bad argument");
    OFX_REQUIRE(M > 0 && ln_bwd_d_ok(D), OFX_ESHAPE, "layernorm_bwd: M = %d, D = %d; needs M >= 1, D in {512, 768, 1024}", M, D);
    OFX_REQUIRE(aligned_to(15, {dy, x, gamma, add, dx, ws}) && aligned_to(7, {dx_op}) && aligned_to(3, {stats, add_map, dgamma, dbeta, dcols, m_dev}), OFX_EINVAL,
                "layernorm_bwd: dy, x, gamma, add, dx and ws must be 16-byte aligned, dx_op 8-byte aligned");
    OFX_REQUIRE(ws_bytes >= ofx_layernorm_bwd_ws(D), OFX_EWORKSPACE, "layernorm_bwd: workspace %zu < %zu bytes", ws_bytes, ofx_layernorm_bwd_ws(D));
    return ofx_launch_ln_bwd(dy, x, stats, gamma, add, add_map, dx, dx_op, dgamma, dbeta, dcols, (float*)ws, D, m_dev, M, op_dtype,
                             make_drop(dropout_p, seed, (unsigned)site), (hipStream_t)stream, accumulate ? 1 : 0);
}
static bool colsum_c_ok(int C) { return C > 0 && C % 4 == 0; }
extern "C" size_t ofx_colsum_ws(int C) { return colsum_c_ok(C) ? ofx_colsum_part_floats(C) * sizeof(float) : 0; }
extern "C" int ofx_colsum(const void* x, int x_kind, int ld, const int* gather, const float* row_scale, float* out0, float* out1, float* out2, int seg,
                          int C, int valid, int M, const int* m_dev, int accumulate, int op_dtype, void* ws, size_t ws_bytes, ofx_stream stream) {
    OFX_REQUIRE(x && ws && (out0 || out1 || out2) && (x_kind == 0 || (x_kind == 1 && op_dtype_ok(op_dtype))), OFX_EINVAL, "colsum: bad argument");
    OFX_REQUIRE(colsum_c_ok(C) && M > 0 && ld >= C && ld % 4 == 0 && seg > 0 && C <= 3 * (long long)seg && valid >= 0 && valid <= seg, OFX_ESHAPE,
                "colsum: C = %d, ld = %d, seg = %d, valid = %d, M = %d; needs C %% 4 == 0, ld >= C, ld %% 4 == 0, C <= 3 seg, valid <= seg, M >= 1", C, ld,
                seg, valid, M);
    OFX_REQUIRE(aligned_to(x_kind == 0 ? 15 : 7, {x}) && aligned_to(15, {ws}) && aligned_to(3, {gather, row_scale, out0, out1, out2, m_dev}), OFX_EINVAL,
                "colsum: x must be aligned to four of its elements, ws to 16 bytes");
    OFX_REQUIRE(ws_bytes >= ofx_colsum_ws(C), OFX_EWORKSPACE, "colsum: workspace %zu < %zu bytes", ws_bytes, ofx_colsum_ws(C));
    return ofx_launch_colsum(x, x_kind, ld, gather, row_scale, out0, out1, out2, seg, (float*)ws, C, m_dev, M, op_dtype, (hipStream_t)stream, valid,
                             accumulate ? 1 : 0);
}
extern "C" int ofx_head_bwd(const float* dlogits, const float* w, const int* cu, float* dX, void* dXb, float* db, int B, int D, float dropout_p,
                            unsigned seed, int head_site, int below_site, int accumulate, int op_dtype, ofx_stream stream) {
    OFX_REQUIRE(w && dX && dXb && (dlogits || !db) && drop_p_ok(dropout_p) && op_dtype_ok(op_dtype), OFX_EINVAL, "head_bwd: bad argument");
    OFX_REQUIRE(B > 0 && D > 0 && D % 4 == 0, OFX_ESHAPE, "head_bwd: B = %d, D = %d; needs B >= 1, D a positive multiple of 4", B, D);
    OFX_REQUIRE(aligned_to(15, {w, dX}) && aligned_to(7, {dXb}) && aligned_to(3, {dlogits, cu, db}), OFX_EINVAL,
                "head_bwd: w and dX must be 16-byte aligned, dXb 8-byte aligned");
    const DropArgs none;
    return ofx_launch_cp_head_bwd(dlogits, w, cu, dX, dXb, db, B, D, op_dtype, head_site < 0 ? none : make_drop(dropout_p, seed, (unsigned)head_site),
                                  below_site < 0 ? none : make_drop(dropout_p, seed, (unsigned)below_site), (hipStream_t)stream, accumulate ? 1 : 0);
}
static int fold_gemm_args(GemmArgs& g, const char* who, const void* A, const void* W, const void* W8, const void* scale8, int K, int w_form, int& op_dtype) {
    OFX_REQUIRE(w_form >= 0 && w_form <= 2 && op_dtype_ok(op_dtype) && (w_form != 2 || op_dtype == OFX_F16), OFX_EINVAL,
                "%s: w_form = %d (0 plain, 1 split, 2 split + fp8 lo copy, f16 only), op_dtype = %d", who, w_form, op_dtype);
    OFX_REQUIRE(A && W && (w_form != 2 || (W8 && scale8)), OFX_EINVAL, "%s: NULL operand", who);
    const WeightForm f = w_form ? W_SPLIT : W_PLAIN;
    g.A = A; g.W = W; g.K = w_kmul(f) * K;
    if (f == W_SPLIT) g.a_wrap = K;
    if (w_form == 2) { g.W8 = W8; g.w8_scale = scale8; }
    return OFX_OK;
}
extern "C" int ofx_gemm_fold_producer(const void* A, const void* W, const void* W8, const void* scale8, void* xb, void* xlo, float* stat_part,
                                      const float* bias, const float* resid, int M, int N, int K, int lda, int ldr, int act, int w_form, int op_dtype,
                                      ofx_stream stream) {
    GemmArgs g = op_gemm(nullptr, nullptr, xb, bias, resid, M, N, K, lda, N, ldr, act, OFX_OUT_OP);
    TRY(fold_gemm_args(g, "gemm_fold_producer", A, W, W8, scale8, K, w_form, op_dtype));
    OFX_REQUIRE(xb && xlo && stat_part, OFX_EINVAL, "gemm_fold_producer: xb, xlo and stat_part are all required");
    OFX_REQUIRE(aligned_to(15, {A, W, W8, xb, xlo, bias, resid}) && aligned_to(7, {stat_part}), OFX_EINVAL,
                "gemm_fold_producer: A, W, W8, xb, xlo, bias must be 16-byte aligned, stat_part 8-byte aligned");
    g.xb_out = xb; g.xlo = xlo; g.stat_part = stat_part;
    return ofx_launch_gemm(g, op_dtype, (hipStream_t)stream);
}
extern "C" int ofx_gemm_fold(const void* A, const void* W, void* C, const float* bias, const float* row_stat, int stat_ld, const float* col_sum,
                             int M, int N, int K, int lda, int ldc, int act, int w_form, int op_dtype, ofx_stream stream) {
    GemmArgs g = op_gemm(nullptr, nullptr, C, bias, nullptr, M, N, K, lda, ldc, 0, act, OFX_OUT_OP);
    OFX_REQUIRE(w_form != 2, OFX_EINVAL, "gemm_fold: w_form 2 is ofx_gemm_w2f8_fold");
    TRY(fold_gemm_args(g, "gemm_fold", A, W, nullptr, nullptr, K, w_form, op_dtype));
    OFX_REQUIRE(C && row_stat && col_sum, OFX_EINVAL, "gemm_fold: C, row_stat and col_sum are required");
    OFX_REQUIRE(aligned_to(15, {A, W, C, bias, col_sum}) && aligned_to(7, {row_stat}), OFX_EINVAL,
                "gemm_fold: A, W, C, bias and col_sum must be 16-byte aligned, row_stat 8-byte aligned");
    OFX_REQUIRE(stat_ld >= 1, OFX_ESHAPE, "gemm_fold: stat_ld = %d; needs >= 1", stat_ld);
    g.row_stat = row_stat; g.col_sum = col_sum; g.stat_ld = stat_ld;
    return ofx_launch_gemm(g, op_dtype, (hipStream_t)stream);
}
extern "C" int ofx_stats_finalize(const float* stat_part, int slots, int W, float eps, float* stat, int rows, ofx_stream stream) {
    OFX_REQUIRE(stat_part && stat && aligned_to(7, {stat_part, stat}), OFX_EINVAL, "stats_finalize: stat_part and stat are required, 8-byte aligned");
    OFX_REQUIRE(rows > 0 && slots > 0 && W > 0, OFX_ESHAPE, "stats_finalize: rows = %d, slots = %d, W = %d; all must be positive", rows, slots, W);
    return ofx_launch_stats_finalize(stat_part, slots, W, eps, stat, rows, (hipStream_t)stream);
}
extern "C" int ofx_row_stats_cast(const float* x, void* xb, void* xlo, float* stat, int rows, int W, float eps, int op_dtype, ofx_stream stream) {
    OFX_REQUIRE(x && xb && xlo && stat && op_dtype_ok(op_dtype), OFX_EINVAL, "row_stats_cast: bad argument");
    OFX_REQUIRE(aligned_to(15, {x}) && aligned_to(7, {xb, xlo, stat}), OFX_EINVAL, "row_stats_cast: x must be 16-byte aligned, xb, xlo and stat 8-byte aligned");
    OFX_REQUIRE(rows > 0 && W > 0 && W % 4 == 0, OFX_ESHAPE, "row_stats_cast: rows = %d, W = %d; needs rows >= 1, W a positive multiple of 4", rows, W);
    return ofx_launch_row_stats_cast(x, xb, xlo, stat, rows, W, eps, op_dtype, (hipStream_t)stream);
}
extern "C" int ofx_fold_pack(const float* w, const float* gamma, const float* beta, const float* bias, void* wf, float* col_sum, float* bias_f, int N, int K,
                             int split, int op_dtype, ofx_stream stream) {
    OFX_REQUIRE(w && gamma && beta && bias && wf && col_sum && bias_f && op_dtype_ok(op_dtype), OFX_EINVAL, "fold_pack: bad argument");
    OFX_REQUIRE(aligned_to(3, {w, gamma, beta, bias, col_sum, bias_f}) && aligned_to(1, {wf}), OFX_EINVAL, "fold_pack: misaligned pointer");
    OFX_REQUIRE(N > 0 && K > 0, OFX_ESHAPE, "fold_pack: N = %d, K = %d; both must be positive", N, K);
    return ofx_launch_fold_pack(w, gamma, beta, bias, wf, col_sum, bias_f, N, K, op_dtype, (hipStream_t)stream, split ? 1 : 0);
}
extern "C" int ofx_vit_embed_ln(const float* patch_out, const float* cls, const float* pos, const float* gamma, const float* beta, float* x, void* xb,
                                void* xlo, float* stat, int N, int S, int D, float eps, int op_dtype, ofx_stream stream) {
    OFX_REQUIRE(patch_out && cls && pos && gamma && beta && op_dtype_ok(op_dtype), OFX_EINVAL, "vit_embed_ln: bad argument");
    OFX_REQUIRE(x ? !xb && !xlo && !stat : xb && xlo && stat, OFX_EINVAL, "vit_embed_ln: writes either x or (xb, xlo, stat)");
    OFX_REQUIRE(aligned_to(15, {patch_out, cls, pos, gamma, beta, x}) && aligned_to(7, {xb, xlo, stat}), OFX_EINVAL,
                "vit_embed_ln: the fp32 arrays must be 16-byte aligned, xb, xlo and stat 8-byte aligned");
    OFX_REQUIRE(N > 0 && S > 0 && (long long)N * S <= INT_MAX, OFX_ESHAPE, "vit_embed_ln: N = %d, S = %d", N, S);
    return ofx_launch_vit_embed_ln(patch_out, cls, pos, gamma, beta, x, N, S, D, eps, (hipStream_t)stream, xb, stat, op_dtype, xlo);
}
extern "C" int ofx_gather_hilo(const void* hi, const void* lo, const int* idx, float* dst, int rows, int W, int op_dtype, ofx_stream stream) {
    OFX_REQUIRE(hi && lo && idx && dst && op_dtype_ok(op_dtype), OFX_EINVAL, "gather_hilo: bad argument");
    OFX_REQUIRE(aligned_to(7, {hi, lo}) && aligned_to(15, {dst}) && aligned_to(3, {idx}), OFX_EINVAL,
                "gather_hilo: hi and lo must be 8-byte aligned, dst 16-byte aligned");
    OFX_REQUIRE(rows > 0 && W > 0 && W % 4 == 0, OFX_ESHAPE, "gather_hilo: rows = %d, W = %d; needs rows >= 1, W a positive multiple of 4", rows, W);
    return ofx_launch_gather_hilo(hi, lo, idx, dst, rows, W, op_dtype, (hipStream_t)stream);
}
extern "C" int ofx_clip_preprocess_patches(const uint8_t* src, const long long* offsets, const int* heights, const int* widths, int N, int channels, int size,
                                           int patch, const float* mean, const float* stdv, void* patches, int op_dtype, void* ws, size_t ws_bytes,
                                           ofx_stream stream) {
    OFX_REQUIRE(src && offsets && heights && widths && mean && stdv && patches && ws && op_dtype_ok(op_dtype), OFX_EINVAL,
                "clip_preprocess_patches: bad argument (a NULL pointer or op_dtype = %d)", op_dtype);
    OFX_REQUIRE(patch > 0 && size > 0 && size % patch == 0, OFX_ESHAPE, "clip_preprocess_patches: size=%d patch=%d", size, patch);
    return ofx_preprocess_to(src, offsets, heights, widths, N, channels, size, mean, stdv, nullptr, patches, patch, op_dtype, ws, ws_bytes, (hipStream_t)stream);
}
extern "C" int ofx_patchify(const float* pixels, void* out, int N, int img, int patch, int op_dtype, ofx_stream stream) {
    OFX_REQUIRE(pixels && out && op_dtype_ok(op_dtype), OFX_EINVAL, "patchify: bad argument (a NULL pointer or op_dtype = %d)", op_dtype);
    OFX_REQUIRE(aligned_to(15, {pixels, out}), OFX_EINVAL, "patchify: pixels and out must be 16-byte aligned");
    OFX_REQUIRE(N > 0 && img > 0 && patch > 0, OFX_ESHAPE, "patchify: N = %d, img = %d, patch = %d; all must be positive", N, img, patch);
    return ofx_launch_patchify(pixels, out, N, img, patch, op_dtype, (hipStream_t)stream);
}
extern "C" int ofx_layernorm(const float* x, const int* row_idx, const float* gamma, const float* beta, void* y, int rows,
                             int D, int ldy, int out_kind, int op_dtype, float eps, ofx_stream stream) {
    LnArgs a{x, row_idx, gamma, beta, y, rows, D, ldy, out_kind, eps};
    return ofx_launch_layernorm(a, op_dtype, (hipStream_t)stream);
}
extern "C" int ofx_attention(const void* qkv, void* out, const int64_t* key_mask, int nseq, int seq_len, int n_head, int ld,
                             int ldo, int k_off, int v_off, int mask_ld, int causal, float scale, int op_dtype, ofx_stream stream) {
    AttnArgs a{qkv, out, key_mask, nseq, seq_len, n_head, ld, ldo, k_off, v_off, mask_ld, causal, scale};
    return ofx_launch_attention_mfma(a, op_dtype, (hipStream_t)stream);
}
extern "C" int ofx_attention_ex(const void* qkv, void* out, const int64_t* key_mask, int nseq, int seq_len, int n_head, int ld, int ldo, int k_off,
                                int v_off, int mask_ld, int causal, int only_row0, int split3_w, float scale, int op_dtype, ofx_stream stream) {
    OFX_REQUIRE(qkv && out && op_dtype_ok(op_dtype), OFX_EINVAL, "attention_ex: bad argument (a NULL pointer or op_dtype = %d)", op_dtype);
    OFX_REQUIRE(split3_w >= 0 && (!key_mask || mask_ld >= seq_len), OFX_ESHAPE, "attention_ex: split3_w=%d mask_ld=%d", split3_w, mask_ld);
    AttnArgs a{qkv, out, key_mask, nseq, seq_len, n_head, ld, ldo, k_off, v_off, mask_ld, causal ? 1 : 0, scale};
    a.only_row0 = only_row0 ? 1 : 0; a.split3_w = split3_w;
    return ofx_launch_attention_mfma(a, op_dtype, (hipStream_t)stream);
}
extern "C" int ofx_set_attention_slabs(const float* slabs, size_t plane_floats, int splits, const float* bias, void* out, const int* cu_seqlens, int nseq,
                                       int n_head, int D, int ldo, int out_kind, int max_len, int only_row0, float scale, int op_dtype, ofx_stream stream) {
    OFX_REQUIRE(slabs && out && cu_seqlens && nseq > 0 && n_head > 0 && splits >= 1 && op_dtype_ok(op_dtype) && aligned_to(15, {slabs, bias, out}) && plane_floats % 4 == 0,
                OFX_EINVAL, "set_attention_slabs: bad argument (a NULL or misaligned pointer, nseq = %d, splits = %d, op_dtype = %d)", nseq, splits, op_dtype);
    OFX_REQUIRE(out_kind >= 0 && out_kind <= 2, OFX_ESHAPE, "set_attention_slabs: out_kind=%d", out_kind);
    SetAttnArgs a{slabs, out, cu_seqlens, nseq, n_head, D, ldo, out_kind, max_len, only_row0 ? 1 : 0, scale};
    a.splits = splits; a.plane = plane_floats; a.bias = bias;
    return ofx_launch_set_attention(a, op_dtype, (hipStream_t)stream);
}
extern "C" int ofx_splitk_reduce_ln(const float* slab, size_t plane_floats, int splits, const float* bias, const float* resid, int ldr, float* x, int ldx,
                                    const float* gamma, const float* beta, void* y, int ldy, int out_kind, float eps, int rows, const int* m_dev, int D,
                                    int op_dtype, ofx_stream stream) {
    OFX_REQUIRE(slab && x && gamma && beta && y && op_dtype_ok(op_dtype) && aligned_to(15, {slab, bias, resid, x, gamma, beta}) && aligned_to(out_kind == 0 ? 15 : 7, {y}) && aligned_to(3, {m_dev}) &&
                    plane_floats % 4 == 0,
                OFX_EINVAL, "splitk_reduce_ln: bad argument (a NULL or misaligned pointer or op_dtype = %d)", op_dtype);
    OFX_REQUIRE(out_kind >= 0 && out_kind <= 2 && (splits <= 1 || plane_floats >= (size_t)rows * D), OFX_ESHAPE, "splitk_reduce_ln: out_kind=%d, or slabs that overlap", out_kind);
    SplitKLnArgs a{slab, plane_floats, splits, bias, resid, ldr, x, ldx, gamma, beta, y, ldy, out_kind, eps, rows, D, m_dev};
    return ofx_launch_splitk_reduce_ln(a, op_dtype, (hipStream_t)stream);
}
extern "C" int ofx_fused_qkv_attention(const void* X, const void* Wqkv, const float* bias, const float* row_stat, const float* col_sum, void* out,
                                       int nseq, int seq_len, int width, int n_head, int ldx, int ldo, float scale, int op_dtype, ofx_stream stream) {
    return ofx_launch_fused_qkv_attn(X, Wqkv, bias, row_stat, col_sum, out, nseq, seq_len, width, n_head, ldx, ldo, scale, op_dtype, (hipStream_t)stream);
}
extern "C" int ofx_fused_qkv_attention_w2(const void* X, const void* Wqkv2, const float* bias, const float* row_stat, const float* col_sum, void* out,
                                          int nseq, int seq_len, int width, int n_head, int ldx, int ldo, float scale, int op_dtype, ofx_stream stream) {
    return ofx_launch_fused_qkv_attn(X, Wqkv2, bias, row_stat, col_sum, out, nseq, seq_len, width, n_head, ldx, ldo, scale, op_dtype, (hipStream_t)stream, true);
}
extern "C" int ofx_set_attention(const float* qkv, void* out, const int* cu_seqlens, int nseq, int n_head, int D, int ldo,
                                 int out_kind, int max_len, int only_row0, float scale, int op_dtype, ofx_stream stream) {
    SetAttnArgs a{qkv, out, cu_seqlens, nseq, n_head, D, ldo, out_kind, max_len, only_row0, scale};
    return ofx_launch_set_attention(a, op_dtype, (hipStream_t)stream);
}
static bool train_attn_args_ok(const void* a, const void* b, const void* c, int nseq, float dropout_p) {
    return a && b && c && nseq > 0 && dropout_p >= 0.f && dropout_p < 1.f;
}
extern "C" int ofx_attention_varlen(const void* qkv, void* out, const int* cu_seqlens, int nseq, int max_len, int n_head, int ld, int ldo, int k_off,
                                    int v_off, int only_row0, float scale, float dropout_p, unsigned seed, int site, int op_dtype, ofx_stream stream) {
    OFX_REQUIRE(train_attn_args_ok(qkv, out, cu_seqlens, nseq, dropout_p), OFX_EINVAL, "attention_varlen: bad argument");
    OFX_REQUIRE(n_head > 0 && k_off == n_head * 64 && v_off == 2 * k_off && ld >= 3 * k_off, OFX_ESHAPE,
                "attention_varlen: q | k | v rows of D = n_head * 64 columns (k_off=%d v_off=%d ld=%d n_head=%d); heads of 96 take ofx_set_attention", k_off, v_off, ld, n_head);
    AttnArgs a{qkv, out, nullptr, nseq, max_len, n_head, ld, ldo, k_off, v_off, 0, 0, scale};
    a.cu_seqlens = cu_seqlens; a.only_row0 = only_row0 ? 1 : 0; a.drop = make_drop(dropout_p, seed, (unsigned)site);
    return ofx_launch_attention_mfma(a, op_dtype, (hipStream_t)stream);
}
extern "C" int ofx_set_attention_op(const void* qkv, void* out, const int* cu_seqlens, int nseq, int n_head, int D, int ldo, int out_kind, int max_len,
                                    int only_row0, float scale, float dropout_p, unsigned seed, int site, int op_dtype, ofx_stream stream) {
    OFX_REQUIRE(train_attn_args_ok(qkv, out, cu_seqlens, nseq, dropout_p) && n_head > 0, OFX_EINVAL, "set_attention_op: bad argument");
    SetAttnArgs a{qkv, out, cu_seqlens, nseq, n_head, D, ldo, out_kind, max_len, only_row0 ? 1 : 0, scale};
    a.drop = make_drop(dropout_p, seed, (unsigned)site); a.qkv_op = 1;
    return ofx_launch_set_attention(a, op_dtype, (hipStream_t)stream);
}
extern "C" int ofx_set_attention_bwd(const void* qkv, const float* d_o, void* dqkv, const int* cu_seqlens, int nseq, int n_head, int D, int max_len,
                                     int only_row0, float scale, float dropout_p, unsigned seed, int site, int mfma, int op_dtype, ofx_stream stream) {
    OFX_REQUIRE(train_attn_args_ok(qkv, d_o, dqkv, nseq, dropout_p) && cu_seqlens && n_head > 0, OFX_EINVAL, "set_attention_bwd: bad argument");
    const auto launch = mfma ? ofx_launch_set_attention_bwd_mfma : ofx_launch_set_attention_bwd;
    return launch(qkv, d_o, dqkv, cu_seqlens, nseq, n_head, D, max_len, scale, op_dtype, make_drop(dropout_p, seed, (unsigned)site), only_row0 ? 1 : 0, (hipStream_t)stream);
}
extern "C" int ofx_attention_f32(const float* qkv, void* out, const int64_t* key_mask, int nseq, int seq_len, int n_head, int D, int ldo, int out_kind,
                                 int mask_ld, int causal, float scale, int op_dtype, ofx_stream stream) {
    SetAttnArgs a{qkv, out, nullptr, nseq, n_head, D, ldo, out_kind, seq_len, 0, scale};
    a.fixed_len = seq_len; a.causal = causal; a.key_mask = key_mask; a.mask_ld = mask_ld;
    return ofx_launch_set_attention(a, op_dtype, (hipStream_t)stream);
}
extern "C" int ofx_convert(const float* src, void* dst, int rows, int cols, int mode, int op_dtype, ofx_stream stream) {
    return ofx_launch_pack_rows(src, dst, rows, rows, cols, cols, cols, mode, op_dtype, (hipStream_t)stream);
}
```

### outfitx_amd/csrc/fused_qkv_attn.hip

```cpp
#include "attn_wave.h"
#include "gemm_common.h"

namespace {

struct FusedK {
    const char* X;
    const char* Wqkv;
    char* out;
    const float* bias;
    const float* row_stat;
    const float* col_sum;
    int n_img, S, Wm, heads, ldx, ldo, G, nwg;
    float scale;
};

constexpr int FQ_TM = 256, FQ_TN = 192, FQ_STAGE = (FQ_TM + FQ_TN) * BK * 2;
constexpr int FQ_QK_ROW = 144;
constexpr int FQ_NT = 4;
static_assert(FQ_TN == 3 * ATTN_D && 16 * FQ_NT == ATTN_D, "the tail runs the attention core at NT = 4 on one head's 64 q, 64 k and 64 v columns");
constexpr int FQ_Q_OFF = 0, FQ_K_OFF = FQ_TM * FQ_QK_ROW, FQ_V_OFF = 2 * FQ_TM * FQ_QK_ROW;
constexpr int FQ_LDS = 2 * FQ_STAGE + 16 * ATTN_V_ROW;
constexpr int FQ2_BK = 32, FQ2_A = FQ_TM * FQ2_BK * 2, FQ2_W = FQ_TN * FQ2_BK * 2, FQ2_STAGE = FQ2_A + 2 * FQ2_W, FQ2_NST = 3;
constexpr int FQ2_LDS = FQ2_NST * FQ2_STAGE;
static_assert(FQ2_LDS >= FQ_LDS, "q | k | v image must fit the dual-weight stages");

template <typename T, bool W2 = false>
__global__ __launch_bounds__(512, 2) void fused_qkv_attn_kernel(FusedK p) {
    typedef typename OpT<T>::v8 v8;
    typedef typename OpT<T>::v4 v4;
    extern __shared__ __attribute__((aligned(16))) char smem[];
    OFX_LDS char* lds = (OFX_LDS char*)smem;
    const int tid = threadIdx.x, lane = tid & 63;
    const int wave = __builtin_amdgcn_readfirstlane(tid >> 6);
    const int wr = wave >> 2, wc = wave & 3;

    const int bid = xcd_remap(blockIdx.x, p.nwg);
    const int hh = p.heads % 2 == 0 ? p.heads / 2 : p.heads, halves = p.heads / hh, per_unit = 6 * hh;
    const int unit = bid / per_unit, in_unit = bid % per_unit;
    const int grp = (unit / halves) * 6 + in_unit / hh, head = (unit % halves) * hh + in_unit % hh;
    if (grp * p.G >= p.n_img) return;
    const int M = p.n_img * p.S;
    const int m0 = grp * p.G * p.S;
    const int n_live_img = min(p.G, p.n_img - grp * p.G);

    f32x4 acc[8][3];
#pragma unroll
    for (int i = 0; i < 8; ++i)
#pragma unroll
        for (int j = 0; j < 3; ++j) acc[i][j] = f32x4{0.f, 0.f, 0.f, 0.f};
    const int fr = lane & 15, fq = lane >> 4;

    if constexpr (W2) {
    const PpLane32 L(lane);
    const int prow = L.prow, pchk = L.pchk;
    const char* a_base = p.X + (size_t)m0 * p.ldx * 2;
    const char* w_base = p.Wqkv + (size_t)head * 64 * (2 * p.Wm) * 2;
    unsigned a_off[2], w_off[3];
#pragma unroll
    for (int i = 0; i < 2; ++i) {
        const int row = (wave * 2 + i) * 16 + prow;
        const int rr = m0 + row < M ? row : M - 1 - m0;
        a_off[i] = ((unsigned)rr * p.ldx + pchk * 8) * 2;
    }
    int w_dst[3];
#pragma unroll
    for (int i = 0; i < 3; ++i) {
        const int q = wave * 3 + i;
        const int row = (q % 12) * 16 + prow;
        const unsigned grow = (unsigned)(row >> 6) * p.Wm + (row & 63);
        w_off[i] = (grow * (2 * p.Wm) + (q >= 12 ? p.Wm : 0) + pchk * 8) * 2;
        w_dst[i] = FQ2_A + (q >= 12 ? FQ2_W : 0) + (q % 12) * 1024;
    }
    const int a_dst = wave * 2 * 1024;
    const int nk = p.Wm / FQ2_BK;
    auto issue_all = [&](int step) {
        const int sc = step < nk ? step : nk - 1;
        OFX_LDS char* base = lds + (step % FQ2_NST) * FQ2_STAGE;
        const char* ak = a_base + (size_t)sc * FQ2_BK * 2;
        const char* wk = w_base + (size_t)sc * FQ2_BK * 2;
#pragma unroll
        for (int i = 0; i < 2; ++i) glds16(ak + a_off[i], base + a_dst + i * 1024);
#pragma unroll
        for (int i = 0; i < 3; ++i) glds16(wk + w_off[i], base + w_dst[i]);
    };
    const int a_frag = (wr * 128 + fr) * 64 + L.fchk;
    const int w_frag = FQ2_A + (wc * 48 + fr) * 64 + L.fchk;
    v8 af[8], wh[3], wl[3];
    auto read = [&](int t) { pp_w2_read<3>(lds + (t % FQ2_NST) * FQ2_STAGE, a_frag, w_frag, FQ2_W, af, wh, wl); };
    auto mfma = [&] { pp_w2_mfma<T, 3>(acc, af, wh, wl); };
    issue_all(0); issue_all(1);
    asm volatile("s_waitcnt vmcnt(5)" ::: "memory");
    __builtin_amdgcn_s_barrier();
    if (wr == 0) {
        for (int t = 0; t < nk; ++t) pp_slot<0, 5>([&] { issue_all(t + 2); }, [&] { read(t); }, mfma);
        pp_group_end<0>();
    } else {
        pp_group_begin<1>();
        for (int t = 0; t < nk; ++t) pp_slot<1, 5>([&] { issue_all(t + 2); }, [&] { read(t); }, mfma);
    }
    asm volatile("s_waitcnt vmcnt(0)" ::: "memory");
    __builtin_amdgcn_s_barrier();
    if (tid < 16 * ATTN_V_ROW / 16) *(OFX_LDS f32x4*)(lds + 2 * FQ_STAGE + tid * 16) = f32x4{0.f, 0.f, 0.f, 0.f};
    } else {
    if (tid < 16 * ATTN_V_ROW / 16) *(OFX_LDS f32x4*)(lds + 2 * FQ_STAGE + tid * 16) = f32x4{0.f, 0.f, 0.f, 0.f};

    const int lrow = lane >> 3, lchk = lane & 7;
    const char* a_base = p.X + (size_t)m0 * p.ldx * 2;
    const char* w_base = p.Wqkv + (size_t)head * 64 * p.Wm * 2;
    unsigned a_off[4], w_off[3];
#pragma unroll
    for (int i = 0; i < 4; ++i) {
        const int row = (wave * 4 + i) * 8 + lrow;
        const int rr = m0 + row < M ? row : M - 1 - m0;
        a_off[i] = ((unsigned)rr * p.ldx + (lchk ^ ((row >> 1) & 7)) * 8) * 2;
    }
#pragma unroll
    for (int i = 0; i < 3; ++i) {
        const int row = (wave * 3 + i) * 8 + lrow;
        const unsigned grow = (unsigned)(row >> 6) * p.Wm + (row & 63);
        w_off[i] = (grow * p.Wm + (lchk ^ ((row >> 1) & 7)) * 8) * 2;
    }
    const int a_dst = wave * 4 * 1024, w_dst = FQ_TM * BK * 2 + wave * 3 * 1024;
    auto issue_all = [&](int kt, int stage) {
        OFX_LDS char* base = lds + stage * FQ_STAGE;
        const char* ak = a_base + (size_t)kt * BK * 2;
        const char* wk = w_base + (size_t)kt * BK * 2;
#pragma unroll
        for (int i = 0; i < 4; ++i) glds16(ak + a_off[i], base + a_dst + i * 1024);
#pragma unroll
        for (int i = 0; i < 3; ++i) glds16(wk + w_off[i], base + w_dst + i * 1024);
    };

    const int fsw = fr >> 1;
    const int a_frag = (wr * 128 + fr) * 128;
    const int w_frag = FQ_TM * BK * 2 + (wc * 48 + fr) * 128;
    v8 af[2][8], wf[2][3];

#define FQ_READ_FRAGS(STG)                                                                                    \
    {                                                                                                         \
        OFX_LDS char* base_ = lds + (STG) * FQ_STAGE;                                                         \
        _Pragma("unroll") for (int ks = 0; ks < 2; ++ks) {                                                    \
            const int chk = ((ks * 4 + fq) ^ fsw) * 16;                                                       \
            _Pragma("unroll") for (int j = 0; j < 3; ++j) wf[ks][j] = *(OFX_LDS v8*)(base_ + w_frag + j * 16 * 128 + chk); \
            _Pragma("unroll") for (int i = 0; i < 8; ++i) af[ks][i] = *(OFX_LDS v8*)(base_ + a_frag + i * 16 * 128 + chk); \
        }                                                                                                     \
    }

    const int nk = p.Wm / BK;
    issue_all(0, 0);
    issue_all(nk > 1 ? 1 : 0, 1);
    asm volatile("s_waitcnt vmcnt(7)" ::: "memory");
    __builtin_amdgcn_s_barrier();
    if (wr == 0) {
        for (int t = 0; t < nk; ++t) {
            if (t >= 1 && t + 1 < nk) issue_all(t + 1, (t + 1) & 1);
            FQ_READ_FRAGS(t & 1)
            asm volatile("s_waitcnt lgkmcnt(0)" ::: "memory");
            __builtin_amdgcn_s_barrier();
            __builtin_amdgcn_s_setprio(1);
#pragma unroll
            for (int m = 0; m < 48; ++m) {
                const int ks = m / 24, i = (m % 24) / 3, j = m % 3;
                acc[i][j] = OpT<T>::mfma16(wf[ks][j], af[ks][i], acc[i][j]);
            }
            __builtin_amdgcn_s_setprio(0);
            asm volatile("s_waitcnt vmcnt(0)" ::: "memory");
            __builtin_amdgcn_s_barrier();
        }
        __builtin_amdgcn_s_barrier();
    } else {
        __builtin_amdgcn_s_barrier();
        for (int t = 0; t < nk; ++t) {
            FQ_READ_FRAGS(t & 1)
            asm volatile("s_waitcnt vmcnt(0)" ::: "memory");
            asm volatile("s_waitcnt lgkmcnt(0)" ::: "memory");
            __builtin_amdgcn_s_barrier();
            OFX_LDS char* nbase = lds + (t & 1) * FQ_STAGE;
            const int kn = t + 2 < nk ? t + 2 : nk - 1;
            const char* ak = a_base + (size_t)kn * BK * 2;
            const char* wk = w_base + (size_t)kn * BK * 2;
            __builtin_amdgcn_s_setprio(1);
#pragma unroll
            for (int m = 0; m < 48; ++m) {
                if (m % 6 == 0 && m / 6 < 7) {
                    const int q = m / 6;
                    if (q < 4) glds16(ak + a_off[q], nbase + a_dst + q * 1024);
                    else glds16(wk + w_off[q - 4], nbase + w_dst + (q - 4) * 1024);
                }
                const int ks = m / 24, i = (m % 24) / 3, j = m % 3;
                acc[i][j] = OpT<T>::mfma16(wf[ks][j], af[ks][i], acc[i][j]);
            }
            __builtin_amdgcn_s_setprio(0);
            __builtin_amdgcn_s_barrier();
        }
    }
#undef FQ_READ_FRAGS
    asm volatile("s_waitcnt vmcnt(0)" ::: "memory");
    __builtin_amdgcn_s_barrier();
    }

    {
        float mu[8], rs[8];
#pragma unroll
        for (int i = 0; i < 8; ++i) {
            mu[i] = 0.f; rs[i] = 1.f;
            if (p.row_stat) {
                const int gm = min(m0 + wr * 128 + i * 16 + fr, M - 1);
                const f32x2 ms = *(const f32x2*)(p.row_stat + 2 * (size_t)gm);
                mu[i] = ms[0]; rs[i] = ms[1];
            }
        }
#pragma unroll
        for (int j = 0; j < 3; ++j) {
            const int c = wc * 48 + j * 16 + fq * 4, which = c >> 6, d = c & 63;
            const int gn = which * p.Wm + head * 64 + d;
            const f32x4 b4 = *(const f32x4*)(p.bias + gn);
            f32x4 cs4 = {0.f, 0.f, 0.f, 0.f};
            if (p.row_stat) cs4 = *(const f32x4*)(p.col_sum + gn);
            OFX_LDS char* reg = lds + (which == 0 ? FQ_Q_OFF : which == 1 ? FQ_K_OFF : FQ_V_OFF);
            const int stride = which == 2 ? ATTN_V_ROW : FQ_QK_ROW;
#pragma unroll
            for (int i = 0; i < 8; ++i) {
                const int row = wr * 128 + i * 16 + fr;
                const f32x4 v = (acc[i][j] - cs4 * mu[i]) * rs[i] + b4;
                v4 o;
#pragma unroll
                for (int e = 0; e < 4; ++e) o[e] = (T)v[e];
                *(OFX_LDS v4*)(reg + row * stride + d * 2) = o;
            }
        }
    }
    asm volatile("s_waitcnt lgkmcnt(0)" ::: "memory");
    __builtin_amdgcn_s_barrier();

    if (wave >= n_live_img) return;
    constexpr int NT = FQ_NT;
    const int S = p.S, r0 = wave * S;
    const int r16 = lane & 15, q4 = lane >> 4;
    OFX_LDS char* ql = lds + FQ_Q_OFF + r0 * FQ_QK_ROW;
    OFX_LDS char* kl = lds + FQ_K_OFF + r0 * FQ_QK_ROW;
    OFX_LDS char* vl = lds + FQ_V_OFF + r0 * ATTN_V_ROW;
    v8 kf[NT][2], qf[NT][2];
#pragma unroll
    for (int t = 0; t < NT; ++t) {
        int row = 16 * t + r16;
        row = row < S ? row : S - 1;
#pragma unroll
        for (int ks = 0; ks < 2; ++ks) {
            kf[t][ks] = *(OFX_LDS v8*)(kl + row * FQ_QK_ROW + (q4 * 8 + ks * 32) * 2);
            qf[t][ks] = *(OFX_LDS v8*)(ql + row * FQ_QK_ROW + (q4 * 8 + ks * 32) * 2);
        }
    }
    float neg[NT][4];
#pragma unroll
    for (int t = 0; t < NT; ++t)
#pragma unroll
        for (int r = 0; r < 4; ++r) neg[t][r] = (16 * t + 4 * q4 + r >= S) ? -INFINITY : 0.f;
    f32x4 st[NT][NT];
    attn_scores<T, NT>(st, kf, qf, neg, NT);
    v8 pf[NT][attn_ksteps(NT)];
    attn_softmax_p<T, NT, false>(pf, st, p.scale, NT);
    attn_pv_store<T, NT>(vl, pf, NT, true, (T*)p.out, m0 + r0, p.ldo, head * 64, S, 0);
}

}

int ofx_launch_fused_qkv_attn(const void* X, const void* Wqkv, const float* bias, const float* row_stat, const float* col_sum, void* out,
                              int n_img, int S, int Wm, int heads, int ldx, int ldo, float scale, int op_dtype, hipStream_t s, bool w2) {
    OFX_REQUIRE(X && Wqkv && bias && out && n_img > 0, OFX_EINVAL, "fused_qkv_attn: NULL argument");
    OFX_REQUIRE(S >= 33 && S <= 64 && Wm == heads * 64 && Wm % BK == 0 && Wm / BK >= 2, OFX_ESHAPE, "fused_qkv_attn: S=%d must be in [33,64], width %d = heads * 64", S, Wm);
    OFX_REQUIRE((FQ_TM / S - 1) * S + 64 - FQ_TM <= 16, OFX_ESHAPE, "fused_qkv_attn: S=%d would read %d key rows past the tile's 16 pad rows (supported: 33, 34, 37..41, 43..64)", S,
                (FQ_TM / S - 1) * S + 64 - FQ_TM);
    OFX_REQUIRE(ldx >= Wm && ldx % 8 == 0 && ldo >= Wm && ldo % 8 == 0, OFX_ESHAPE, "fused_qkv_attn: bad strides");
    OFX_REQUIRE(!row_stat || col_sum, OFX_EINVAL, "fused_qkv_attn: row_stat needs col_sum");
    FusedK k;
    k.X = (const char*)X; k.Wqkv = (const char*)Wqkv; k.out = (char*)out; k.bias = bias; k.row_stat = row_stat; k.col_sum = col_sum;
    k.n_img = n_img; k.S = S; k.Wm = Wm; k.heads = heads; k.ldx = ldx; k.ldo = ldo; k.G = FQ_TM / S; k.scale = scale;
    const int groups = (n_img + k.G - 1) / k.G;
    k.nwg = ((groups + 5) / 6) * 6 * heads;
    static DeviceOnce attr;
    TRY(attr.run([]() -> int {
        OFX_HIP(hipFuncSetAttribute((const void*)fused_qkv_attn_kernel<bf16_t, false>, hipFuncAttributeMaxDynamicSharedMemorySize, FQ_LDS));
        OFX_HIP(hipFuncSetAttribute((const void*)fused_qkv_attn_kernel<f16_t, false>, hipFuncAttributeMaxDynamicSharedMemorySize, FQ_LDS));
        OFX_HIP(hipFuncSetAttribute((const void*)fused_qkv_attn_kernel<bf16_t, true>, hipFuncAttributeMaxDynamicSharedMemorySize, FQ2_LDS));
        OFX_HIP(hipFuncSetAttribute((const void*)fused_qkv_attn_kernel<f16_t, true>, hipFuncAttributeMaxDynamicSharedMemorySize, FQ2_LDS));
        return OFX_OK;
    }));
    if (g_ofx_prof_on) ofx_prof_set_tag(n_img * S, 3 * Wm, Wm, 7, w2 ? 2 : 1, 2.0 * n_img * S * Wm + 2.0 * (w2 ? 2 : 1) * 3.0 * Wm * Wm + 2.0 * n_img * S * Wm);
    ProfScope prof(PROF_GEMM, s, (w2 ? 2.0 : 1.0) * 2.0 * n_img * S * 3.0 * Wm * Wm + 4.0 * n_img * S * S * Wm, true);
    if (w2) {
        if (op_dtype == OFX_F16) OFX_PLAUNCH(true, (fused_qkv_attn_kernel<f16_t, true>), dim3(k.nwg), dim3(512), FQ2_LDS, s, k);
        else OFX_PLAUNCH(true, (fused_qkv_attn_kernel<bf16_t, true>), dim3(k.nwg), dim3(512), FQ2_LDS, s, k);
    } else {
        if (op_dtype == OFX_F16) OFX_PLAUNCH(true, (fused_qkv_attn_kernel<f16_t, false>), dim3(k.nwg), dim3(512), FQ_LDS, s, k);
        else OFX_PLAUNCH(true, (fused_qkv_attn_kernel<bf16_t, false>), dim3(k.nwg), dim3(512), FQ_LDS, s, k);
    }
    OFX_LAUNCH_CHECK();
    return OFX_OK;
}
```

### outfitx_amd/csrc/gemm.hip

```cpp
#include "gemm_common.h"

namespace {
template <typename T, int MT = 4>
__global__ __launch_bounds__(256, 2) void gemm_128x128_kernel(KArgs p) {
    constexpr int BMT = 32 * MT, STAGE_T = (BMT + BN) * BK * 2, EPI_T = 16 * MT * EPI_STRIDE * 4;
    typedef typename OpT<T>::v8 v8;
    extern __shared__ __attribute__((aligned(16))) char smem[];
    OFX_LDS char* lds = (OFX_LDS char*)smem;

    const int tid = threadIdx.x, lane = tid & 63;
    const int wave = __builtin_amdgcn_readfirstlane(tid >> 6);
    const int wm = wave >> 1, wn = wave & 1;

    int tm, tn;
    grouped_tile(xcd_remap(blockIdx.x, p.nwg), p.group_m, p.tiles_m, p.tiles_n, tm, tn);
    const int m0 = tm * BMT, n0 = tn * BN;
    if (clamp_live_rows(p.m_dev, p.M, m0)) return;

    const int lrow = lane >> 3, lchk = lane & 7;
    const char* a_src[MT];
    const char* w_src[4];
#pragma unroll
    for (int i = 0; i < 4; ++i) {
        const int c = wave * 4 + i;
        const int row = c * 8 + lrow;
        const int kch = lchk ^ ((row >> 1) & 7);
        w_src[i] = p.W + ((size_t)(n0 + row) * p.K + kch * 8) * 2;
    }
#pragma unroll
    for (int i = 0; i < MT; ++i) {
        const int row = (wave * MT + i) * 8 + lrow;
        const int kch = lchk ^ ((row >> 1) & 7);
        int gm = m0 + row; gm = gm < p.M ? gm : p.M - 1;
        a_src[i] = p.A + ((size_t)gm * p.lda + kch * 8) * 2;
    }
    const int a_dst = wave * MT * 1024, w_dst = BMT * BK * 2 + wave * 4 * 1024;

    auto issue = [&](int kt, int stage) {
        OFX_LDS char* base = lds + stage * STAGE_T;
        const size_t koff = (size_t)kt * BK * 2, koff_a = (size_t)(kt % p.ka_tiles) * BK * 2;
#pragma unroll
        for (int i = 0; i < MT; ++i) glds16(a_src[i] + koff_a, base + a_dst + i * 1024);
#pragma unroll
        for (int i = 0; i < 4; ++i) glds16(w_src[i] + koff, base + w_dst + i * 1024);
    };

    const int fr = lane & 15, fq = lane >> 4, fsw = fr >> 1;
    const int a_frag = (wm * 16 * MT + fr) * 128;
    const int w_frag = BMT * BK * 2 + (wn * 64 + fr) * 128;

    f32x4 acc[MT][4];
#pragma unroll
    for (int i = 0; i < MT; ++i)
#pragma unroll
        for (int j = 0; j < 4; ++j) acc[i][j] = f32x4{0.f, 0.f, 0.f, 0.f};

    v8 af[2][MT], wf[2][4];
    const int kt0 = p.splits > 1 ? blockIdx.y * p.kt_per_split : 0;
    const int nk = p.splits > 1 ? min(p.K / BK, kt0 + p.kt_per_split) : p.K / BK;
    issue(kt0, kt0 & 1);
    for (int kt = kt0; kt < nk; ++kt) {
        const int cur = kt & 1;
        if (kt + 1 < nk) {
            issue(kt + 1, cur ^ 1);
            if (MT == 4) asm volatile("s_waitcnt vmcnt(8)" ::: "memory");
            else asm volatile("s_waitcnt vmcnt(6)" ::: "memory");
        } else {
            asm volatile("s_waitcnt vmcnt(0)" ::: "memory");
        }
        __builtin_amdgcn_s_barrier();
        OFX_LDS char* base = lds + cur * STAGE_T;
#pragma unroll
        for (int ks = 0; ks < 2; ++ks) {
            const int chk = ((ks * 4 + fq) ^ fsw) * 16;
#pragma unroll
            for (int j = 0; j < 4; ++j) wf[ks][j] = *(OFX_LDS v8*)(base + w_frag + j * 16 * 128 + chk);
#pragma unroll
            for (int i = 0; i < MT; ++i) af[ks][i] = *(OFX_LDS v8*)(base + a_frag + i * 16 * 128 + chk);
        }
        __builtin_amdgcn_s_setprio(1);
#pragma unroll
        for (int ks = 0; ks < 2; ++ks)
#pragma unroll
            for (int i = 0; i < MT; ++i)
#pragma unroll
                for (int j = 0; j < 4; ++j) acc[i][j] = OpT<T>::mfma16(wf[ks][j], af[ks][i], acc[i][j]);
        __builtin_amdgcn_s_setprio(0);
        asm volatile("s_waitcnt lgkmcnt(0)" ::: "memory");
        __builtin_amdgcn_s_barrier();
    }

    OFX_LDS float* ep = (OFX_LDS float*)(lds + wave * EPI_T);
#pragma unroll
    for (int i = 0; i < MT; ++i)
#pragma unroll
        for (int j = 0; j < 4; ++j)
            *(OFX_LDS f32x4*)(ep + (i * 16 + fr) * EPI_STRIDE + j * 16 + fq * 4) = acc[i][j];
    asm volatile("s_waitcnt lgkmcnt(0)" ::: "memory");
    if (p.splits > 1) {
        KArgs q = p;
        q.C = (char*)(p.slab + (size_t)blockIdx.y * p.m_slab * p.N); q.ldc = p.N; q.out_kind = 0; q.bias = nullptr; q.resid = nullptr; q.aux_out = nullptr; q.drop.thresh = 0;
        epilogue<T, OFX_ACT_NONE>(q, ep, m0 + wm * 16 * MT, n0 + wn * 64, lane, 16 * MT);
        return;
    }
    switch (p.act) {
        case OFX_ACT_QUICK_GELU: epilogue<T, OFX_ACT_QUICK_GELU>(p, ep, m0 + wm * 16 * MT, n0 + wn * 64, lane, 16 * MT); break;
        case OFX_ACT_GELU: epilogue<T, OFX_ACT_GELU>(p, ep, m0 + wm * 16 * MT, n0 + wn * 64, lane, 16 * MT); break;
        case OFX_ACT_MISH: epilogue<T, OFX_ACT_MISH>(p, ep, m0 + wm * 16 * MT, n0 + wn * 64, lane, 16 * MT); break;
        case OFX_ACT_MISH_GRAD: epilogue<T, OFX_ACT_MISH_GRAD>(p, ep, m0 + wm * 16 * MT, n0 + wn * 64, lane, 16 * MT); break;
        default: epilogue<T, OFX_ACT_NONE>(p, ep, m0 + wm * 16 * MT, n0 + wn * 64, lane, 16 * MT); break;
    }
}


}

static GemmKnobs g_knobs;
int ofx_gemm_tune(int knob, int value) {
    switch (knob) {
        case 2: g_knobs.kernel = value; return OFX_OK;
        case 5:
            if (value >= 2 && (value & 0xff) == 0) { ofx_set_error("ofx_tune(5): %d forces a split-K plan of 0 slices (low byte = slices, 1-16)", value); return OFX_EINVAL; }
            g_knobs.splitk = value; return OFX_OK;
        case 11: g_knobs.w2_persist = value; return OFX_OK;
        case 15: g_knobs.x3_kernel = value; return OFX_OK;
        case 16: g_knobs.x3_persist = value != 0; return OFX_OK;
        case 18: if (value != 0 && value != 1) { ofx_set_error("ofx_tune(18): %d is not 0 or 1", value); return OFX_EINVAL; } g_knobs.epi_direct = value; return OFX_OK;
        default: ofx_set_error("ofx_tune: unknown knob %d", knob); return OFX_EINVAL;
    }
}
size_t ofx_gemm_splitk_bytes(int M, int N, int K) { return gemm_splitk_slab_bytes(M, N, K, g_knobs); }

int ofx_launch_gemm(const GemmArgs& g, int op_dtype, hipStream_t s) {
    OFX_REQUIRE(g.M > 0 && g.N > 0 && g.K > 0, OFX_ESHAPE, "gemm: empty problem M=%d N=%d K=%d", g.M, g.N, g.K);
    OFX_REQUIRE(g.N % BN == 0, OFX_ESHAPE, "gemm: N=%d must be a multiple of %d (pad the weight at pack time)", g.N, BN);
    OFX_REQUIRE(g.K % BK == 0, OFX_ESHAPE, "gemm: K=%d must be a multiple of %d", g.K, BK);
    OFX_REQUIRE(g.a_wrap == 0 || (g.a_wrap > 0 && g.a_wrap % BK == 0 && g.K % g.a_wrap == 0), OFX_ESHAPE, "gemm: a_wrap=%d must be a multiple of %d dividing K=%d", g.a_wrap, BK, g.K);
    const int ka = g.a_wrap ? g.a_wrap : g.K;
    OFX_REQUIRE(g.lda >= ka && g.lda % 8 == 0, OFX_ESHAPE, "gemm: lda=%d must be >= K and a multiple of 8", g.lda);
    OFX_REQUIRE(g.ldc % (g.out_kind == 0 ? 4 : 8) == 0 && g.ldc >= (g.out_kind == 2 ? 3 * g.N : g.N), OFX_ESHAPE, "gemm: bad ldc=%d", g.ldc);
    OFX_REQUIRE(!g.resid || (g.ldr % 4 == 0 && g.ldr >= g.N), OFX_ESHAPE, "gemm: bad ldr=%d", g.ldr);
    OFX_REQUIRE(((uintptr_t)g.A % 16 == 0) && ((uintptr_t)g.W % 16 == 0) && ((uintptr_t)g.C % 16 == 0), OFX_EINVAL,
                "gemm: operands must be 16-byte aligned");
    OFX_REQUIRE(op_dtype == OFX_BF16 || op_dtype == OFX_F16, OFX_EINVAL, "gemm: operand dtype must be bf16 or f16");
    if (g.defer_splits) *g.defer_splits = 1;
    if (g.ln_done) *g.ln_done = false;
    const bool producer = g.xb_out || g.stat_part || g.xlo;
    OFX_REQUIRE(!producer || (g.xb_out && g.stat_part && g.xlo && g.C == g.xb_out && g.out_kind == 1 && g.ldc == g.N && g.N % 64 == 0), OFX_EINVAL,
                "gemm: a LayerNorm-fold producer takes xb_out, stat_part and xlo together, with C == xb_out in the operand type");
    OFX_REQUIRE(!g.row_stat || g.col_sum, OFX_EINVAL, "gemm: row_stat needs col_sum");
    OFX_REQUIRE(!(g.row_stat || producer) || (!g.aux_out && !g.drop.thresh && g.act != OFX_ACT_MISH && g.act != OFX_ACT_MISH_GRAD), OFX_EINVAL,
                "gemm: LayerNorm folding does not combine with the training epilogue features");
    OFX_REQUIRE(!(g.row_stat || producer) || !g.resid, OFX_EINVAL, "gemm: LayerNorm folding takes no residual (a producer's stream is (xb_out, xlo))");
    OFX_REQUIRE(!producer || g.act == OFX_ACT_NONE, OFX_EINVAL, "gemm: a LayerNorm-fold producer has no activation");

    GemmShape sh;
    sh.M = g.M; sh.N = g.N; sh.K = g.K; sh.lda = g.lda; sh.a_wrap = g.a_wrap; sh.k_mult = g.k_mult;
    sh.f16 = op_dtype == OFX_F16; sh.has_w8 = g.W8 && g.w8_scale; sh.has_m_dev = g.m_dev != nullptr;
    sh.can_split = g.slab && !producer && !g.row_stat; sh.defer = g.defer_splits != nullptr;
    sh.ln_fusable = g.ln_gamma && g.out_kind == 0 && g.act == OFX_ACT_NONE && !g.aux_out && !g.drop.thresh;
    sh.out_kind = g.out_kind; sh.resid = g.resid != nullptr; sh.aux = g.aux_out != nullptr; sh.xlo = g.xlo != nullptr;
    const GemmPlan pl = gemm_plan(sh, g_knobs, device_cu_count());
    if (pl.splits > 1) OFX_REQUIRE(g.slab_bytes >= (size_t)pl.splits * g.M * g.N * 4, OFX_EWORKSPACE, "gemm: split-K slab too small");

    if (g_ofx_prof_on) ofx_prof_set_tag(g.M, g.N, pl.k_logical, pl.kind, pl.kmul, pl.bytes);
    ProfScope prof(PROF_GEMM, s, pl.flops, true);
    KArgs k;
    k.A = (const char*)g.A; k.W = (const char*)g.W; k.C = (char*)g.C; k.bias = g.bias; k.resid = g.resid; k.aux_out = g.aux_out; k.m_dev = g.m_dev;
    k.M = g.M; k.N = g.N; k.K = g.K; k.lda = g.lda; k.ldc = g.ldc; k.ldr = g.ldr; k.act = g.act; k.out_kind = g.out_kind; k.drop = g.drop; k.n_valid = g.N;
    k.ka_tiles = ka / BK;
    k.xb_out = (char*)g.xb_out; k.stat_part = g.stat_part; k.row_stat = g.row_stat; k.col_sum = g.col_sum; k.stat_ld = g.stat_ld > 0 ? g.stat_ld : 1; k.xlo = (char*)g.xlo;
    k.tiles_m = pl.tiles_m; k.tiles_n = pl.tiles_n; k.nwg = pl.nwg; k.group_m = pl.group_m; k.epi_direct = pl.epi_direct;
    k.splits = pl.splits; k.kt_per_split = pl.kt_per_split; k.slab = (float*)g.slab; k.m_slab = g.M;
    if (gemm_kind_big_tile(pl.kind)) {
        if (pl.kind == GEMM_W2F8) { k.W8 = (const char*)g.W8; k.w8_scale = (const char*)g.w8_scale; TRY(ofx_gemm_launch_w2f8(&k, pl, s)); }
        else if (pl.kind == GEMM_X3) TRY(ofx_gemm_launch_x3(&k, pl, op_dtype, s));
        else if (pl.kind == GEMM_W2) TRY(ofx_gemm_launch_w2(&k, pl, op_dtype, s));
        else if (pl.kind == GEMM_PP) TRY(ofx_gemm_launch_pp(&k, pl, op_dtype, s));
        else TRY(ofx_gemm_launch_big(&k, pl, op_dtype, s));
        OFX_LAUNCH_CHECK();
        return OFX_OK;
    }
    static DeviceOnce attr_set;
    TRY(attr_set.run([]() -> int {
        OFX_HIP(hipFuncSetAttribute((const void*)gemm_128x128_kernel<bf16_t>, hipFuncAttributeMaxDynamicSharedMemorySize, GEMM_LDS_BYTES));
        OFX_HIP(hipFuncSetAttribute((const void*)gemm_128x128_kernel<f16_t>, hipFuncAttributeMaxDynamicSharedMemorySize, GEMM_LDS_BYTES));
        OFX_HIP(hipFuncSetAttribute((const void*)gemm_128x128_kernel<bf16_t, 2>, hipFuncAttributeMaxDynamicSharedMemorySize, GEMM64_LDS_BYTES));
        OFX_HIP(hipFuncSetAttribute((const void*)gemm_128x128_kernel<f16_t, 2>, hipFuncAttributeMaxDynamicSharedMemorySize, GEMM64_LDS_BYTES));
        return OFX_OK;
    }));
    const dim3 grid(pl.grid_x, pl.grid_y);
    const bool one = pl.second_pass == GEMM_PASS_NONE || pl.second_pass == GEMM_PASS_DEFERRED;
    if (pl.tile_m == 64) {
        if (op_dtype == OFX_F16) OFX_PLAUNCH(one, (gemm_128x128_kernel<f16_t, 2>), grid, dim3(256), GEMM64_LDS_BYTES, s, k);
        else OFX_PLAUNCH(one, (gemm_128x128_kernel<bf16_t, 2>), grid, dim3(256), GEMM64_LDS_BYTES, s, k);
    } else if (op_dtype == OFX_F16) OFX_PLAUNCH(one, gemm_128x128_kernel<f16_t>, grid, dim3(256), GEMM_LDS_BYTES, s, k);
    else OFX_PLAUNCH(one, gemm_128x128_kernel<bf16_t>, grid, dim3(256), GEMM_LDS_BYTES, s, k);
    if (pl.second_pass == GEMM_PASS_DEFERRED) *g.defer_splits = pl.splits;
    else if (pl.second_pass == GEMM_PASS_REDUCE_LN) {
        SplitKLnArgs a{(const float*)g.slab, (size_t)g.M * g.N, pl.splits, g.bias, g.resid, g.ldr, (float*)g.C, g.ldc,
                       g.ln_gamma, g.ln_beta, g.ln_out, g.ln_ld, g.ln_kind, g.ln_eps, g.M, g.N, g.m_dev};
        TRY(ofx_launch_splitk_reduce_ln(a, op_dtype, s, true));
        if (g.ln_done) *g.ln_done = true;
    } else if (pl.second_pass == GEMM_PASS_REDUCE) {
        if (op_dtype == OFX_F16) OFX_PLAUNCH(true, splitk_reduce_kernel<f16_t>, dim3(pl.reduce_grid), dim3(256), 0, s, k);
        else OFX_PLAUNCH(true, splitk_reduce_kernel<bf16_t>, dim3(pl.reduce_grid), dim3(256), 0, s, k);
    }
    OFX_LAUNCH_CHECK();
    return OFX_OK;
}
```

### outfitx_amd/csrc/ofx_common.h

```cpp
#pragma once
#include <hip/hip_runtime.h>
#include <hip/hip_ext.h>
#include <mutex>
#include <stdint.h>
#include <stdio.h>

#include "../../include/ofx.h"
#include "gemm_plan.h"

typedef __bf16 bf16_t;
typedef _Float16 f16_t;
typedef __bf16 bf16x8 __attribute__((ext_vector_type(8)));
typedef __bf16 bf16x4 __attribute__((ext_vector_type(4)));
typedef _Float16 f16x8 __attribute__((ext_vector_type(8)));
typedef _Float16 f16x4 __attribute__((ext_vector_type(4)));
typedef float f32x4 __attribute__((ext_vector_type(4)));
typedef float f32x2 __attribute__((ext_vector_type(2)));
typedef float f32x16 __attribute__((ext_vector_type(16)));
typedef short s16x4 __attribute__((ext_vector_type(4)));
typedef short s16x8 __attribute__((ext_vector_type(8)));

#define OFX_LDS __attribute__((address_space(3)))
#define OFX_GLB __attribute__((address_space(1)))

// ... 100 lines not shown
}

__device__ __forceinline__ float row16_sum_to_lane15(float v) {
    v += __builtin_bit_cast(float, __builtin_amdgcn_update_dpp(0, __builtin_bit_cast(int, v), 0x111, 0xf, 0xf, true));
    v += __builtin_bit_cast(float, __builtin_amdgcn_update_dpp(0, __builtin_bit_cast(int, v), 0x112, 0xf, 0xf, true));
    v += __builtin_bit_cast(float, __builtin_amdgcn_update_dpp(0, __builtin_bit_cast(int, v), 0x114, 0xf, 0xf, true));
    v += __builtin_bit_cast(float, __builtin_amdgcn_update_dpp(0, __builtin_bit_cast(int, v), 0x118, 0xf, 0xf, true));
    return v;
}
__device__ __forceinline__ float row8_sum(float v) {
    v += __builtin_bit_cast(float, __builtin_amdgcn_update_dpp(0, __builtin_bit_cast(int, v), 0xB1, 0xf, 0xf, true));
    v += __builtin_bit_cast(float, __builtin_amdgcn_update_dpp(0, __builtin_bit_cast(int, v), 0x4E, 0xf, 0xf, true));
    v += __builtin_bit_cast(float, __builtin_amdgcn_update_dpp(0, __builtin_bit_cast(int, v), 0x141, 0xf, 0xf, true));
    return v;
}
__device__ __forceinline__ float wave_sum(float v) {
#pragma unroll
    for (int o = 32; o > 0; o >>= 1) v += __shfl_xor(v, o, 64);
    return v;
}
__device__ __forceinline__ float wave_max(float v) {
#pragma unroll
    for (int o = 32; o > 0; o >>= 1) v = fmaxf(v, __shfl_xor(v, o, 64));
    return v;
}

enum { PROF_GEMM = 0, PROF_NORM = 1, PROF_ATTN = 2, PROF_OTHER = 3, PROF_NCAT = 4 };
extern bool g_ofx_prof_on;
extern int g_ofx_prof_mask;
void ofx_prof_begin(int cat, hipStream_t s, double flops);
void ofx_prof_end(hipStream_t s);
void ofx_prof_set_tag(int M, int N, int K, int kind, int kmul, double bytes);
bool ofx_prof_ext_begin(int cat, double flops);
void ofx_prof_ext_end();
extern hipEvent_t g_ofx_launch_e0, g_ofx_launch_e1;
struct ProfScope {
    hipStream_t s; bool on, ext;
    ProfScope(int cat, hipStream_t st, double flops = 0.0, bool ext_ = false, bool enable = true) : s(st), on(enable && g_ofx_prof_on && ((g_ofx_prof_mask >> cat) & 1)), ext(ext_) {
        if (on && ext) on = ofx_prof_ext_begin(cat, flops);
        else if (on) ofx_prof_begin(cat, s, flops);
    }
    ~ProfScope() {
        if (on && ext) ofx_prof_ext_end();
        else if (on) ofx_prof_end(s);
    }
};
#define OFX_PLAUNCH(last, kernel, grid, block, lds, stream, ...)                                                                  \
    do {                                                                                                                          \
        hipEvent_t pe0_ = g_ofx_launch_e0, pe1_ = (last) ? g_ofx_launch_e1 : nullptr;                                             \
        g_ofx_launch_e0 = nullptr;                                                                                                \
        if (last) g_ofx_launch_e1 = nullptr;                                                                                      \
        if (pe0_ || pe1_) hipExtLaunchKernelGGL(kernel, grid, block, lds, stream, pe0_, pe1_, 0, __VA_ARGS__);                      \
        else hipLaunchKernelGGL(kernel, grid, block, lds, stream, __VA_ARGS__);                                                   \
    } while (0)

inline size_t align_up(size_t v, size_t a) { return (v + a - 1) / a * a; }
inline int pad128(int v) { return (v + 127) / 128 * 128; }

struct DeviceOnce {
    std::mutex mu;
    unsigned long long done = 0;
    template <typename F>
    int run(F&& f) {
        int dev = 0;
        if (hipGetDevice(&dev) != hipSuccess) dev = 0;
        const unsigned long long bit = 1ull << (dev & 63);
        std::lock_guard<std::mutex> lk(mu);
        if (done & bit) return OFX_OK;
        const int rc = f();
        if (rc == OFX_OK) done |= bit;
        return rc;
    }
};
template <typename K>
int set_max_dynamic_lds(DeviceOnce& once, K kernel, int bytes) {
    return once.run([&]() -> int {
        OFX_HIP(hipFuncSetAttribute((const void*)kernel, hipFuncAttributeMaxDynamicSharedMemorySize, bytes));
        return OFX_OK;
    });
}

int device_cu_count();

struct Bump {
    char* base; size_t cap, off = 0; bool ok = true;
    Bump(void* p, size_t c) : base((char*)p), cap(c) {}
    template <typename T> T* take(size_t n) {
        off = align_up(off, 256);
        T* r = (T*)(base + off);
        off += n * sizeof(T);
        if (off > cap) ok = false;
        return r;
    }
};
#define TRY(x) do { int rc_ = (x); if (rc_ != OFX_OK) return rc_; } while (0)

struct DropArgs {
    unsigned seed = 0, site = 0, thresh = 0;
    float scale = 1.0f;
};
__host__ __device__ __forceinline__ unsigned ofx_fmix32(unsigned h) {
    h ^= h >> 16; h *= 0x85EBCA6Bu; h ^= h >> 13; h *= 0xC2B2AE35u; h ^= h >> 16;
    return h;
}
__host__ __device__ __forceinline__ float drop_mul(const DropArgs& d, unsigned row, unsigned col) {
    unsigned h = ofx_fmix32(d.seed + d.site * 0x9E3779B9u + row * 0x632BE5ABu);
    h = ofx_fmix32(h ^ (col * 0x9E3779B1u + 0x7F4A7C15u));
    return h >= d.thresh ? d.scale : 0.0f;
}
__host__ __device__ __forceinline__ unsigned ofx_draw_u32(unsigned seed, unsigned draw, unsigned stream, unsigned b, unsigned i) {
    unsigned h = ofx_fmix32(seed + 0x6A09E667u);
    h = ofx_fmix32(h ^ draw);
    h = ofx_fmix32(h + stream * 0x9E3779B9u + 0x7F4A7C15u);
    h = ofx_fmix32(h ^ (b * 0x632BE5ABu));
    return ofx_fmix32(h + i * 0x9E3779B1u);
}
__host__ __device__ __forceinline__ unsigned ofx_draw_below(unsigned u, unsigned n) { return (unsigned)(((unsigned long long)u * n) >> 32); }
inline DropArgs make_drop(float p, unsigned seed, unsigned site) {
    DropArgs d;
    if (p > 0.f) { d.seed = seed; d.site = site; d.thresh = (unsigned)((double)p * 4294967296.0); d.scale = 1.0f / (1.0f - p); }
    return d;
}

struct GemmArgs {
    const void* A;
    const void* W;
    void* C;
    const float* bias;
    const float* resid;
    const int* m_dev = nullptr;
    float* aux_out = nullptr;
    void* slab = nullptr;
    size_t slab_bytes = 0;
    int M, N, K, lda, ldc, ldr;
    int act;
    int out_kind;
    DropArgs drop;
    void* xb_out = nullptr;
    float* stat_part = nullptr;
    const float* row_stat = nullptr;
    int stat_ld = 1;
    void* xlo = nullptr;
    const float* col_sum = nullptr;
    int a_wrap = 0;
    const void* W8 = nullptr; const void* w8_scale = nullptr;
    int k_mult = 1;
    int* defer_splits = nullptr;
    const float* ln_gamma = nullptr; const float* ln_beta = nullptr; void* ln_out = nullptr; int ln_ld = 0, ln_kind = 0; float ln_eps = 0.f;
    bool* ln_done = nullptr;
};
int ofx_launch_gemm(const GemmArgs& g, int op_dtype , hipStream_t s);
size_t ofx_gemm_splitk_bytes(int M, int N, int K);
int ofx_gemm_tune(int knob, int value);

struct LnArgs {
    const float* x;
    const int* row_idx;
    const float* gamma;
    const float* beta;
    void* y;
    int rows, D, ldy;
    int out_kind;
    float eps;
    float* stats = nullptr;
};
size_t ofx_gemm_tn_slab_bytes(int M, int N, int K);
int ofx_launch_gemm_tn(const void* A, int lda, const void* B, int ldb, float* C, int ldc, int M, int N, int K, const int* k_dev,
                       void* slab, size_t slab_bytes, int op_dtype, hipStream_t s, int m_valid = 0, int n_valid = 0, int accumulate = 0);
int ofx_launch_layernorm(const LnArgs& a, int op_dtype, hipStream_t s);
struct SplitKLnArgs {
    const float* slab; size_t plane; int splits;
    const float* bias; const float* resid; int ldr;
    float* x; int ldx;
    const float* gamma; const float* beta; void* y; int ldy, out_kind; float eps;
    int rows, D; const int* m_dev;
};
int ofx_launch_splitk_reduce_ln(const SplitKLnArgs& a, int op_dtype, hipStream_t s, bool in_gemm_scope = false);
int ofx_launch_layernorm_dev(const LnArgs& a, const int* rows_dev, int op_dtype, hipStream_t s);
int ofx_launch_pack_lo8(const void* w2_rows, void* dst8, void* scale8, int N, int K, hipStream_t s);
int ofx_launch_pack_rows(const float* src, void* dst, int rows_src, int rows_dst, int K_src, int K_dst, int ld_src,
                         int mode, int op_dtype, hipStream_t s);
int ofx_launch_patchify(const float* px, void* out, int N, int img, int patch, int op_dtype, hipStream_t s);
int ofx_launch_vit_embed_ln(const float* patch_out, const float* cls, const float* pos, const float* g, const float* b,
                            float* x, int N, int S, int D, float eps, hipStream_t s, void* xb, float* stat, int op_dtype, void* xlo);
int ofx_launch_text_embed(const int64_t* ids, const float* tok, const float* pos, float* x, int N, int T, int Tc, int D,
                          int vocab, int shared_first, hipStream_t s);
int ofx_launch_text_eos_index(const int64_t* ids, int* row_idx, int N, int T, int Tc, int eos_id, int shared_first, hipStream_t s);
int ofx_launch_iota_rows(int* idx, int n, int stride, hipStream_t s);
int ofx_launch_l2norm_store(const float* src, float* dst, int rows, int D, int ld, int col, int normalize, hipStream_t s);
int ofx_launch_set_build(const float* x, const uint8_t* mask, const float* prefix, int prefix_stride, int* cu, float* X,
                         int B, int L, int D, hipStream_t s);
int ofx_launch_gather_rows(const void* src, const int* idx, void* dst, int rows, int row_bytes, int src_ld_bytes, hipStream_t s);
int ofx_launch_set_build_indexed(const float* table, int ld, long long n_table, const int* idx, const int* cu_items, const float* prefix,
                                 int prefix_stride, int* cu_rows, float* X, int B, int D, hipStream_t s);
int ofx_preprocess_to(const uint8_t* src, const long long* offsets, const int* heights, const int* widths, int N, int channels, int size,
                      const float* mean, const float* stdv, float* out, void* patches, int patch, int op_dtype, void* ws, size_t ws_bytes, hipStream_t stream);
int ofx_launch_row_stats_cast(const float* X, void* Xb, void* Xlo, float* stat, int rows, int W, float eps, int op_dtype, hipStream_t s);
int ofx_launch_gather_hilo(const void* hi, const void* lo, const int* idx, float* dst, int rows, int W, int op_dtype, hipStream_t s);
int ofx_launch_stats_finalize(const float* part, int slots, int W, float eps, float* stat, int rows, hipStream_t s);
int ofx_launch_fold_pack(const float* Wsrc, const float* gamma, const float* beta, const float* bias, void* Wf, float* col_sum, float* bias_f,
                         int N, int K, int op_dtype, hipStream_t s, int split = 0);
int ofx_launch_cir_prefix(const float* img_emb, const float* txt, float* out, int B, int D, hipStream_t s);
int ofx_launch_cp_head(const float* row0, const float* w, const float* bias, float* logits, int B, int D, hipStream_t s);

struct CirSampleArgs {
    const int *outfit_cu, *outfit_rows, *pos_cu, *pos_slots, *pool_cu, *pool_rows, *row_pool, *row_slot, *outfit_ids;
    int n_outfits, n_outfit_rows, n_pos_slots, n_pools, n_pool_rows, n_table, B, K, max_len;
    unsigned seed, draw;
    int *item_index, *cu_seqlens, *target_item_index, *neg_items_index;
};
int ofx_launch_cir_sample_batch(const CirSampleArgs& a, hipStream_t s);

struct AttnArgs {
    const void* qkv;
    void* out;
    const int64_t* key_mask;
    int nseq, seq_len, n_head, ld, ldo, k_off, v_off, mask_ld;
    int causal;
    float scale;
    const int* cu_seqlens = nullptr;
    int only_row0 = 0;
    DropArgs drop;
    int split3_w = 0;
};
int ofx_launch_attention_mfma(const AttnArgs& a, int op_dtype, hipStream_t s);

struct SetAttnArgs {
    const void* qkv;
    void* out;
    const int* cu_seqlens;
    int nseq, n_head, D, ldo, out_kind;
    int max_len;
    int only_row0;
    float scale;
    DropArgs drop;
    int qkv_op = 0;
    int fixed_len = 0, causal = 0, mask_ld = 0;
    const int64_t* key_mask = nullptr;
    int shared_first = 0;
    int splits = 1; size_t plane = 0; const float* bias = nullptr;
};
int ofx_launch_set_attention(const SetAttnArgs& a, int op_dtype, hipStream_t s);
int ofx_launch_fused_qkv_attn(const void* X, const void* Wqkv, const float* bias, const float* row_stat, const float* col_sum, void* out,
                              int n_img, int S, int Wm, int heads, int ldx, int ldo, float scale, int op_dtype, hipStream_t s, bool w2 = false);

int ofx_launch_multi_copy(const void* table_host, int n, hipStream_t s);
int ofx_launch_fill_f32(float* p, size_t n, float v, hipStream_t s);
int ofx_launch_transpose_cast(const float* src, void* dst, int R, int C, int ldd, int op_dtype, hipStream_t s, void* row_dst = nullptr, int ld_row = 0);
size_t ofx_colsum_part_floats(int C);
int ofx_launch_colsum(const void* x, int x_kind, int ld, const int* gather, const float* row_scale, float* out0, float* out1, float* out2, int seg,
                      float* part, int C, const int* m_dev, int M, int op_dtype, hipStream_t s, int valid = 0, int accumulate = 0);
size_t ofx_ln_bwd_part_floats(int D);
int ofx_launch_row_map(const int* cu, int* map, int B, int M, hipStream_t s);
int ofx_launch_ln_bwd(const float* dy, const float* x, const float* stats, const float* gamma, const float* add, const int* add_map, float* dx_out, void* dx_op,
                      float* dgamma, float* dbeta, float* dcols, float* part, int D, const int* m_dev, int M, int op_dtype, const DropArgs& drop, hipStream_t s,
                      int accumulate = 0);
int ofx_launch_set_attention_bwd(const void* qkv, const float* d_o, void* dqkv, const int* cu, int nseq, int n_head, int D, int max_len,
                                 float scale, int op_dtype, const DropArgs& drop, int only_row0, hipStream_t s);
int ofx_launch_set_attention_bwd_mfma(const void* qkv, const float* d_o, void* dqkv, const int* cu, int nseq, int n_head, int D, int max_len,
                                      float scale, int op_dtype, const DropArgs& drop, int only_row0, hipStream_t s);
int ofx_launch_drop_rows(float* x, int rows, int cols, const DropArgs& d, hipStream_t s);
int ofx_launch_focal_loss(const float* logits, const float* labels, int B, float alpha, float gamma, float upstream, float* loss, float* dlogits, hipStream_t s,
                          int reduction = 1, float* per_elem = nullptr);
size_t ofx_set_rank_loss_ws(int B, int K);
int ofx_launch_set_rank_loss(const float* y, const float* y_hat, const float* neg, const uint8_t* mask, int B, int K, int D, float margin, float upstream,
                             float* loss, float* dy_hat, float* d_pos, float* d_neg, void* ws, hipStream_t s);
int ofx_launch_set_rank_loss_indexed(const float* table, int ld, int n_table, const int* pos_index, const int* neg_index, const float* y_hat, int B, int K,
                                     int D, float margin, float upstream, float* loss, float* dy_hat, float* d_pos, float* d_neg, void* ws, hipStream_t s);
size_t ofx_adamw_step_ws(long long n_arena);
int ofx_launch_adamw_step(const ofx_opt_segment* segments, int n_segments, float* grad, float* exp_avg, float* exp_avg_sq, long long n_arena,
                          float* step, double lr, double beta1, double beta2, double eps, double weight_decay, double max_norm, double grad_scale,
                          float* grad_norm, int* skipped, void* ws, hipStream_t s);
int ofx_launch_cp_head_bwd(const float* dlogits, const float* w_or_rows, const int* cu, float* dX, void* dXb, float* db, int B, int D, int op_dtype,
                           const DropArgs& head, const DropArgs& below, hipStream_t s, int accumulate = 0);
int ofx_launch_fitb(const float* y, const float* cand, int B, int C, int D, int64_t* idx, float* dist, hipStream_t s);
int ofx_launch_fitb_indexed(const float* table, int ld, int n_table, const int* cand_index, const float* y, int B, int C, int D, const int64_t* answer,
                            int64_t* idx, float* dist, int* n_correct, hipStream_t s);
int ofx_launch_l2_topk(const float* Q, const float* P, int nq, int np, int D, int k, int64_t index_base, int64_t* idx,
                       float* dist, void* ws, size_t ws_bytes, hipStream_t s);
size_t ofx_l2_topk_ws(int nq, int np);
int ofx_launch_l2_topk_grouped(const float* Q, const float* P, int nq, int np, int D, int k, const int* panels, int n_panels, int max_group_rows,
                               const int64_t* gt, int64_t* idx, float* dist, int* gt_pos, void* ws, size_t ws_bytes, hipStream_t s);
int ofx_launch_topk_merge(const int64_t* idx_in, const float* dist_in, int parts, int nq, int k, int64_t* idx, float* dist,
                          hipStream_t s);

extern int g_topk_filter;
```

Baseline: 8140.

## Add persistent fused QKV-attention kernel using w2 fp8 weight scheme

Adds a fused QKV-projection-plus-attention kernel for the split-weight (w2) form whose low-order weight part is stored in fp8 with per-block scales. It is persistent, prefetches the next tile's constants, and converts activations to bf8 on the fly to feed the fp8 residual product. It is enabled by default when the GEMM planner would pick the W2F8 path and the shape fits. The aim is to replace the separate QKV GEMM plus attention with a single kernel that moves fewer weight bytes, at the cost of a complex LDS layout and a new precision path.

```diff
diff --git a/include/ofx.h b/include/ofx.h
--- a/include/ofx.h
+++ b/include/ofx.h
@@ -212,6 +212,9 @@
                             int nseq, int seq_len, int width, int n_head, int ldx, int ldo, float scale, int op_dtype, ofx_stream stream);
 int ofx_fused_qkv_attention_w2(const void* X, const void* Wqkv2, const float* bias, const float* row_stat, const float* col_sum, void* out,
                                int nseq, int seq_len, int width, int n_head, int ldx, int ldo, float scale, int op_dtype, ofx_stream stream);
+int ofx_fused_qkv_attention_w2f8(const void* X, const void* Wqkv2, const void* W8, const void* scale8, const float* bias, const float* row_stat,
+                                 const float* col_sum, void* out, int nseq, int seq_len, int width, int n_head, int ldx, int ldo, float scale,
+                                 ofx_stream stream);
 int ofx_attention_f32(const float* qkv, void* out, const int64_t* key_mask, int nseq, int seq_len, int n_head, int D, int ldo, int out_kind,
                       int mask_ld, int causal, float scale, int op_dtype, ofx_stream stream);
 int ofx_convert(const float* src, void* dst, int rows, int cols, int mode, int op_dtype, ofx_stream stream);
diff --git a/outfitx_amd/_lib.py b/outfitx_amd/_lib.py
--- a/outfitx_amd/_lib.py
+++ b/outfitx_amd/_lib.py
@@ -176,6 +176,7 @@
     "ofx_splitk_reduce_ln": (_i, [_vp, _sz, _i, _vp, _vp, _i, _vp, _i, _vp, _vp, _vp, _i, _i, _f, _i, _vp, _i, _i, _vp]),
     "ofx_fused_qkv_attention": (_i, [_vp, _vp, _vp, _vp, _vp, _vp, _i, _i, _i, _i, _i, _i, _f, _i, _vp]),
     "ofx_fused_qkv_attention_w2": (_i, [_vp, _vp, _vp, _vp, _vp, _vp, _i, _i, _i, _i, _i, _i, _f, _i, _vp]),
+    "ofx_fused_qkv_attention_w2f8": (_i, [_vp, _vp, _vp, _vp, _vp, _vp, _vp, _vp, _i, _i, _i, _i, _i, _i, _f, _vp]),
     "ofx_set_attention": (_i, [_vp, _vp, _vp, _i, _i, _i, _i, _i, _i, _i, _f, _i, _vp]),
     "ofx_attention_varlen": (_i, [_vp, _vp, _vp, _i, _i, _i, _i, _i, _i, _i, _i, _f, _f, C.c_uint, _i, _i, _vp]),
     "ofx_set_attention_op": (_i, [_vp, _vp, _vp, _i, _i, _i, _i, _i, _i, _i, _f, _f, C.c_uint, _i, _i, _vp]),
diff --git a/outfitx_amd/csrc/api.hip b/outfitx_amd/csrc/api.hip
--- a/outfitx_amd/csrc/api.hip
+++ b/outfitx_amd/csrc/api.hip
@@ -516,18 +516,24 @@
 }
 
 int g_fuse_qkv = 1;
+int g_fuse_qkv_w2f8 = 1;
 int g_x3_vit_f32_attn = 0;
 int g_prune_q = 1;
 
 static int clip_layer(const ClipLayer& L, const ClipWs& w, int rows, int nseq, int S, int W, int MLP, int heads, int act,
                       float eps, int causal, const int64_t* key_mask, int mask_ld, int dt, const int* pool_idx, hipStream_t s, bool pool_first) {
-    const bool fused = (g_fuse_qkv & (L.qkv.form == W_SPLIT ? 2 : 1)) && !pool_idx && !causal && !key_mask && S >= 33 && S <= 64 && (256 / S - 1) * S + 64 - 256 <= 16;
-    if (fused) {
-        TRY(ofx_launch_fused_qkv_attn(w.XB, L.qkv.w, L.qkv.bias, w.S, L.qkv.col_sum, w.H, nseq, S, W, heads, W, W, 0.125f, dt, s, L.qkv.form == W_SPLIT));
+    const bool fits = !pool_idx && !causal && !key_mask && S >= 33 && S <= 64 && (256 / S - 1) * S + 64 - 256 <= 16;
+    const bool fused = (g_fuse_qkv & (L.qkv.form == W_SPLIT ? 2 : 1)) && fits;
+    GemmArgs g1{}; g1.A = w.XB; g1.C = w.QKV; g1.row_stat = w.S; g1.M = rows; g1.N = 3 * W;
+    g1.ldc = 3 * W; g1.act = OFX_ACT_NONE; g1.out_kind = OFX_OUT_OP;
+    use_gemm(g1, L.qkv, W);
+    const bool fused8 = !fused && g_fuse_qkv_w2f8 && fits && L.qkv.form == W_SPLIT && L.qkv.f8.w8 && L.qkv.f8.s8 && dt == OFX_F16 && W % 128 == 0 &&
+                        ofx_gemm_plan_kind(g1, dt) == GEMM_W2F8;
+    if (fused8) {
+        TRY(ofx_launch_fused_qkv_attn(w.XB, L.qkv.w, L.qkv.bias, w.S, L.qkv.col_sum, w.H, nseq, S, W, heads, W, W, 0.125f, dt, s, FUSED_QKV_W2F8, L.qkv.f8.w8, L.qkv.f8.s8));
+    } else if (fused) {
+        TRY(ofx_launch_fused_qkv_attn(w.XB, L.qkv.w, L.qkv.bias, w.S, L.qkv.col_sum, w.H, nseq, S, W, heads, W, W, 0.125f, dt, s, L.qkv.form == W_SPLIT ? FUSED_QKV_W2 : FUSED_QKV_PLAIN));
     } else {
-        GemmArgs g1{}; g1.A = w.XB; g1.C = w.QKV; g1.row_stat = w.S; g1.M = rows; g1.N = 3 * W;
-        g1.ldc = 3 * W; g1.act = OFX_ACT_NONE; g1.out_kind = OFX_OUT_OP;
-        use_gemm(g1, L.qkv, W);
         const bool prune = pool_idx && pool_first && g_prune_q;
         if (prune) {
             GemmArgs kv = g1;
@@ -1150,6 +1156,7 @@
         case 17: g_topk_filter = value != 0; return OFX_OK;
         case 20: g_x3_vit_f32_attn = value != 0; return OFX_OK;
         case 21: g_text_shared_first = value != 0; return OFX_OK;
+        case 22: g_fuse_qkv_w2f8 = value != 0; return OFX_OK;
         default: ofx_set_error("ofx_tune: unknown knob %d", knob); return OFX_EINVAL;
     }
 }
@@ -1390,7 +1397,11 @@
 }
 extern "C" int ofx_fused_qkv_attention_w2(const void* X, const void* Wqkv2, const float* bias, const float* row_stat, const float* col_sum, void* out,
                                           int nseq, int seq_len, int width, int n_head, int ldx, int ldo, float scale, int op_dtype, ofx_stream stream) {
-    return ofx_launch_fused_qkv_attn(X, Wqkv2, bias, row_stat, col_sum, out, nseq, seq_len, width, n_head, ldx, ldo, scale, op_dtype, (hipStream_t)stream, true);
+    return ofx_launch_fused_qkv_attn(X, Wqkv2, bias, row_stat, col_sum, out, nseq, seq_len, width, n_head, ldx, ldo, scale, op_dtype, (hipStream_t)stream, FUSED_QKV_W2);
+}
+extern "C" int ofx_fused_qkv_attention_w2f8(const void* X, const void* Wqkv2, const void* W8, const void* scale8, const float* bias, const float* row_stat,
+                                            const float* col_sum, void* out, int nseq, int seq_len, int width, int n_head, int ldx, int ldo, float scale, ofx_stream stream) {
+    return ofx_launch_fused_qkv_attn(X, Wqkv2, bias, row_stat, col_sum, out, nseq, seq_len, width, n_head, ldx, ldo, scale, OFX_F16, (hipStream_t)stream, FUSED_QKV_W2F8, W8, scale8);
 }
 extern "C" int ofx_set_attention(const float* qkv, void* out, const int* cu_seqlens, int nseq, int n_head, int D, int ldo,
                                  int out_kind, int max_len, int only_row0, float scale, int op_dtype, ofx_stream stream) {
diff --git a/outfitx_amd/csrc/fused_qkv_attn.hip b/outfitx_amd/csrc/fused_qkv_attn.hip
--- a/outfitx_amd/csrc/fused_qkv_attn.hip
+++ b/outfitx_amd/csrc/fused_qkv_attn.hip
@@ -12,6 +12,7 @@
     const float* col_sum;
     int n_img, S, Wm, heads, ldx, ldo, G, nwg;
     float scale;
+    const char* W8 = nullptr; const char* scale8 = nullptr;
 };
 
 constexpr int FQ_TM = 256, FQ_TN = 192, FQ_STAGE = (FQ_TM + FQ_TN) * BK * 2;
@@ -23,6 +24,15 @@
 constexpr int FQ2_BK = 32, FQ2_A = FQ_TM * FQ2_BK * 2, FQ2_W = FQ_TN * FQ2_BK * 2, FQ2_STAGE = FQ2_A + 2 * FQ2_W, FQ2_NST = 3;
 constexpr int FQ2_LDS = FQ2_NST * FQ2_STAGE;
 static_assert(FQ2_LDS >= FQ_LDS, "q | k | v image must fit the dual-weight stages");
+constexpr int FQ8_A = FQ_TM * 32 * 2, FQ8_W = FQ_TN * 32 * 2, FQ8_STAGE = FQ8_A + FQ8_W, FQ8_NST = 4;
+constexpr int FQ8_W8BASE = FQ8_NST * FQ8_STAGE, FQ8_W8 = FQ_TN * 128;
+constexpr int FQ8_IMG = FQ8_STAGE, FQ8_CST = FQ8_IMG + FQ_LDS, FQ8_CST_WAVE = (2 * 64 + 2 * 96) * 4;
+constexpr int FQ8_LDS = FQ8_CST + 8 * FQ8_CST_WAVE;
+static_assert(FQ8_CST >= FQ8_W8BASE + FQ8_W8 && FQ8_IMG + 2 * FQ_STAGE >= FQ8_W8BASE + FQ8_W8, "the V pad rows and the constants lie behind everything LDS-DMA fills");
+static_assert(FQ8_LDS <= 160 * 1024, "one block per CU");
+
+template <typename T>
+__device__ __forceinline__ void fq_attention(OFX_LDS char* lds, const FusedK& p, int wave, int lane, int m0, int head);
 
 template <typename T, bool W2 = false>
 __global__ __launch_bounds__(512, 2) void fused_qkv_attn_kernel(FusedK p) {
@@ -234,6 +244,12 @@
     __builtin_amdgcn_s_barrier();
 
     if (wave >= n_live_img) return;
+    fq_attention<T>(lds, p, wave, lane, m0, head);
+}
+
+template <typename T>
+__device__ __forceinline__ void fq_attention(OFX_LDS char* lds, const FusedK& p, int wave, int lane, int m0, int head) {
+    typedef typename OpT<T>::v8 v8;
     constexpr int NT = FQ_NT;
     const int S = p.S, r0 = wave * S;
     const int r16 = lane & 15, q4 = lane >> 4;
@@ -263,12 +279,271 @@
     attn_pv_store<T, NT>(vl, pf, NT, true, (T*)p.out, m0 + r0, p.ldo, head * 64, S, 0);
 }
 
+typedef int fq_i32x8 __attribute__((ext_vector_type(8)));
+typedef int fq_i32x4 __attribute__((ext_vector_type(4)));
+typedef short fq_i16x2 __attribute__((ext_vector_type(2)));
+typedef _Float16 fq_f16x2 __attribute__((ext_vector_type(2)));
+
+__global__ __launch_bounds__(512, 2) void fused_qkv_attn_w2f8_kernel(FusedK p) {
+    typedef f16_t T;
+    typedef OpT<T>::v8 v8;
+    typedef OpT<T>::v4 v4;
+    constexpr int BK2 = 32, PART = FQ8_A, STAGE = FQ8_STAGE;
+    extern __shared__ __attribute__((aligned(16))) char smem[];
+    OFX_LDS char* lds = (OFX_LDS char*)smem;
+    OFX_LDS char* img = lds + FQ8_IMG;
+    const int tid = threadIdx.x, lane = tid & 63;
+    const int wave = __builtin_amdgcn_readfirstlane(tid >> 6);
+    const int wr = wave >> 1, wc = wave & 1;
+    int grp = wave >> 2;
+    asm volatile("" : "+s"(grp));
+    const int Kh = p.Wm, nk = Kh / BK2, nsup = nk >> 2;
+    const int M = p.n_img * p.S;
+    const float a_scale = 1.0f;
+    const int a_e8 = 127;
+
+    const int hh = p.heads % 2 == 0 ? p.heads / 2 : p.heads, halves = p.heads / hh, per_unit = 6 * hh;
+    auto decode = [&](int v, int& g, int& h) {
+        const int bid = xcd_remap(v, p.nwg), unit = bid / per_unit, in_unit = bid % per_unit;
+        g = (unit / halves) * 6 + in_unit / hh;
+        h = (unit % halves) * hh + in_unit % hh;
+    };
+    auto next_live = [&](int v) {
+        for (; v < p.nwg; v += (int)gridDim.x) {
+            int g, h;
+            decode(v, g, h);
+            if (g * p.G < p.n_img) break;
+        }
+        return v;
+    };
+    int vb = next_live(blockIdx.x);
+    if (vb >= p.nwg) return;
+
+    int ln = lane;
+    asm volatile("" : "+v"(ln));
+    OFX_LDS float* cst = (OFX_LDS float*)(lds + FQ8_CST + wave * FQ8_CST_WAVE);
+
+    auto load_consts = [&](int m0_, int head_, f32x2& ms, f32x4& c4, unsigned long long (&sw)[3]) {
+        ms = f32x2{0.f, 1.f};
+        c4 = f32x4{0.f, 0.f, 0.f, 0.f};
+        if (p.row_stat) ms = *(const f32x2*)(p.row_stat + 2 * (size_t)min(m0_ + wr * 64 + ln, M - 1));
+        const float* cb = ln >= 32 ? (p.row_stat ? p.col_sum : nullptr) : p.bias;
+        const int c = wc * 96 + (ln & 31) * 4;
+        if (cb && (ln & 31) < 24) c4 = *(const f32x4*)(cb + (c >> 6) * Kh + head_ * 64 + (c & 63));
+#pragma unroll
+        for (int w = 0; w < 3; ++w) sw[w] = *(const unsigned long long*)(p.scale8 + ((size_t)(w * (Kh >> 7) + (head_ >> 1)) * 16 + (ln & 15)) * 8);
+    };
+    auto stash_consts = [&](int head_, f32x2 ms, f32x4 c4, const unsigned long long (&sw)[3], int& sa, int& sb) {
+        *(OFX_LDS f32x2*)(cst + 2 * ln) = ms;
+        if ((ln & 31) < 24) *(OFX_LDS f32x4*)(cst + 128 + (ln >> 5) * 96 + (ln & 31) * 4) = c4;
+        const int sh = (head_ & 1) * 32;
+        const unsigned q_ = (unsigned)(sw[0] >> sh), k_ = (unsigned)(sw[1] >> sh), v_ = (unsigned)(sw[2] >> sh);
+        sa = (int)(wc == 0 ? q_ : (k_ >> 16) | (v_ << 16));
+        sb = (int)(wc == 0 ? k_ : v_ >> 16);
+    };
+
+    const size_t a_row = (size_t)p.ldx * 2;
+    const unsigned w_head = 64u * (2 * Kh) * 2;
+    const __amdgpu_buffer_rsrc_t r_w = make_rsrc(p.Wqkv), r_w8 = make_rsrc(p.W8);
+    int grp_t, head, sc_a, sc_b;
+    decode(vb, grp_t, head);
+    {
+        f32x2 ms; f32x4 c4; unsigned long long sw[3];
+        load_consts(grp_t * p.G * p.S, head, ms, c4, sw);
+        stash_consts(head, ms, c4, sw, sc_a, sc_b);
+    }
+    if (tid < 16 * ATTN_V_ROW / 16) *(OFX_LDS f32x4*)(img + 2 * FQ_STAGE + tid * 16) = f32x4{0.f, 0.f, 0.f, 0.f};
+    bool first = true;
+
+    for (;;) {
+        const int vn = next_live(vb + (int)gridDim.x);
+        const bool has_next = vn < p.nwg;
+        int grp_n = grp_t, head_n = head;
+        if (has_next) decode(vn, grp_n, head_n);
+        const int m0 = grp_t * p.G * p.S, m1 = grp_n * p.G * p.S;
+        const int n_live_img = min(p.G, p.n_img - grp_t * p.G);
+        int l2 = ln;
+        asm volatile("" : "+v"(l2));
+        const PpLane32 L(l2);
+        const int fr = L.fr, fq = L.fq;
+        const int wp0 = grp == 0 ? wave * 2 : 4 + wave;
+        unsigned a_off[2], w_off[2], w8_off[3];
+#pragma unroll
+        for (int i = 0; i < 2; ++i) {
+            a_off[i] = ((unsigned)((wave * 2 + i) * 16 + L.prow) * p.ldx + L.pchk * 8) * 2;
+            const int row = ((wp0 + i) * 16 + L.prow) % FQ_TN;
+            w_off[i] = (((unsigned)(row >> 6) * Kh + (row & 63)) * (2 * Kh) + L.pchk * 8) * 2;
+        }
+#pragma unroll
+        for (int q = 0; q < 3; ++q) {
+            const int P = wave * 3 + q;
+            w8_off[q] = (unsigned)((P >> 3) * Kh + (P & 7) * 8 + (l2 >> 3)) * Kh + ((((l2 & 7) ^ (((l2 >> 4) & 3) << 1)) ^ (P & 1)) << 4);
+        }
+        const int a_dst = wave * 2 * 1024, w_dst = PART + wp0 * 1024, w8_dst = FQ8_W8BASE + wave * 3 * 1024;
+        const int a_frag = (wr * 64 + fr) * 64 + L.fchk;
+        const int w_frag = PART + (wc * 96 + fr) * 64 + L.fchk;
+        const int x8 = (((fr >> 1) & 3) << 1) | (fr >> 3);
+        const int w8_frag0 = (wc * 96 + fr) * 128 + (((2 * fq) ^ x8) << 4), w8_frag1 = (wc * 96 + fr) * 128 + (((2 * fq + 1) ^ x8) << 4);
+        const __amdgpu_buffer_rsrc_t r_a = make_rsrc(p.X + (size_t)m0 * a_row, (size_t)(M - m0) * a_row), r_a1 = make_rsrc(p.X + (size_t)m1 * a_row, (size_t)(M - m1) * a_row);
+        auto issue_step = [&](int x, bool two_w) {
+            OFX_LDS char* stg = lds + (x & 3) * STAGE;
+            const bool nx = x == nk;
+            const __amdgpu_buffer_rsrc_t ra = nx ? r_a1 : r_a;
+            const unsigned koff = (unsigned)(nx ? 0 : (x > nk ? nk - 1 : x)) * BK2 * 2;
+            const unsigned sw = (unsigned)(nx ? head_n : head) * w_head + koff;
+            bload16(ra, a_off[0], koff, stg + a_dst); bload16(ra, a_off[1], koff, stg + a_dst + 1024);
+            bload16(r_w, w_off[0], sw, stg + w_dst);
+            if (two_w) bload16(r_w, w_off[1], sw, stg + w_dst + 1024);
+        };
+#define FQ8_ISSUE_W8(SUP, Q) bload16(r_w8, w8_off[Q], (unsigned)head * 64u * (unsigned)Kh + (unsigned)(SUP) * 128u, lds + w8_dst + (Q) * 1024);
+
+        f32x4 acc[4][6];
+#pragma unroll
+        for (int i = 0; i < 4; ++i)
+#pragma unroll
+            for (int j = 0; j < 6; ++j) acc[i][j] = f32x4{0.f, 0.f, 0.f, 0.f};
+        v8 af[4], wh[6];
+        fq_i32x8 a8[4];
+#pragma unroll
+        for (int i = 0; i < 4; ++i) a8[i] = fq_i32x8{0, 0, 0, 0, 0, 0, 0, 0};
+        auto read = [&](int step) {
+            OFX_LDS char* stg = lds + (step & 3) * STAGE;
+#pragma unroll
+            for (int j = 0; j < 6; ++j) wh[j] = *(OFX_LDS v8*)(stg + w_frag + j * 16 * 64);
+#pragma unroll
+            for (int i = 0; i < 4; ++i) af[i] = *(OFX_LDS v8*)(stg + a_frag + i * 16 * 64);
+        };
+#define FQ8_CVT1(I, S)                                                                                        \
+    {                                                                                                         \
+        fq_i16x2 lo_ = __builtin_bit_cast(fq_i16x2, a8[I][2 * (S)]), hi_ = __builtin_bit_cast(fq_i16x2, a8[I][2 * (S) + 1]); \
+        lo_ = __builtin_amdgcn_cvt_scalef32_pk_bf8_f16(lo_, fq_f16x2{af[I][0], af[I][1]}, a_scale, false);    \
+        lo_ = __builtin_amdgcn_cvt_scalef32_pk_bf8_f16(lo_, fq_f16x2{af[I][2], af[I][3]}, a_scale, true);     \
+        hi_ = __builtin_amdgcn_cvt_scalef32_pk_bf8_f16(hi_, fq_f16x2{af[I][4], af[I][5]}, a_scale, false);    \
+        hi_ = __builtin_amdgcn_cvt_scalef32_pk_bf8_f16(hi_, fq_f16x2{af[I][6], af[I][7]}, a_scale, true);     \
+        a8[I][2 * (S)] = __builtin_bit_cast(int, lo_); a8[I][2 * (S) + 1] = __builtin_bit_cast(int, hi_);      \
+    }
+#define FQ8_MFMA16(S)                                                                                         \
+    {                                                                                                         \
+        __builtin_amdgcn_s_setprio(1);                                                                        \
+        _Pragma("unroll") for (int j = 0; j < 6; ++j) {                                                       \
+            _Pragma("unroll") for (int i = 0; i < 4; ++i) acc[i][j] = OpT<T>::mfma16(wh[j], af[i], acc[i][j]); \
+            if (j >= 2) FQ8_CVT1(j - 2, S)                                                                    \
+        }                                                                                                     \
+        __builtin_amdgcn_s_setprio(0);                                                                        \
+    }
+#define FQ8_LD(J)                                                                                             \
+    {                                                                                                         \
+        const fq_i32x4 c0_ = *(OFX_LDS fq_i32x4*)(b8_ + w8_frag0 + (J) * 16 * 128), c1_ = *(OFX_LDS fq_i32x4*)(b8_ + w8_frag1 + (J) * 16 * 128); \
+        w8_[(J) % 3] = fq_i32x8{c0_[0], c0_[1], c0_[2], c0_[3], c1_[0], c1_[1], c1_[2], c1_[3]};              \
+    }
+#define FQ8_MF(J, SEL, SC)                                                                                    \
+    if ((J) + 2 < 6) { FQ8_LD((J) + 2) __builtin_amdgcn_sched_barrier(0); }                                   \
+    _Pragma("unroll") for (int i = 0; i < 4; ++i)                                                             \
+        acc[i][J] = __builtin_amdgcn_mfma_scale_f32_16x16x128_f8f6f4(w8_[(J) % 3], a8[i], acc[i][J], 0, 1, SEL, SC, 0, a_e8);
+#define FQ8_MFMA8()                                                                                           \
+    {                                                                                                         \
+        __builtin_amdgcn_sched_barrier(0);                                                                    \
+        OFX_LDS char* b8_ = lds + FQ8_W8BASE;                                                                 \
+        fq_i32x8 w8_[3];                                                                                      \
+        FQ8_LD(0) FQ8_LD(1)                                                                                   \
+        __builtin_amdgcn_s_setprio(1);                                                                        \
+        FQ8_MF(0, 0, sc_a) FQ8_MF(1, 1, sc_a) FQ8_MF(2, 2, sc_a) FQ8_MF(3, 3, sc_a)                           \
+        FQ8_MF(4, 0, sc_b) FQ8_MF(5, 1, sc_b)                                                                 \
+        __builtin_amdgcn_s_setprio(0);                                                                        \
+    }
+
+        if (first) {
+            issue_step(0, grp == 0); issue_step(1, grp == 0);
+            if (grp == 0) asm volatile("s_waitcnt vmcnt(4)" ::: "memory");
+            else { issue_step(2, false); asm volatile("s_waitcnt vmcnt(6)" ::: "memory"); }
+        } else {
+            issue_step(1, grp == 0);
+            if (grp != 0) issue_step(2, false);
+        }
+        asm volatile("" : "+v"(sc_a), "+v"(sc_b));
+        asm volatile("s_setreg_imm32_b32 hwreg(HW_REG_MODE, 23, 1), 1");
+        __builtin_amdgcn_s_barrier();
+        auto run = [&](auto G) {
+            constexpr int g = G.value;
+            constexpr bool w2 = g == 0;
+            pp_group_begin<g>();
+            int u = 0;
+            do {
+                const int t = 4 * u;
+                pp_slot<g, g ? 3 : 8>([&] { if (g == 0) issue_step(t + 2, w2); issue_step(t + 3, w2); }, [&] { read(t); }, [&] { FQ8_MFMA16(0) });
+                pp_slot<g, 3>([&] { FQ8_ISSUE_W8(u, 0) FQ8_ISSUE_W8(u, 1) FQ8_ISSUE_W8(u, 2) }, [&] { read(t + 1); }, [&] { FQ8_MFMA16(1) });
+                pp_slot<g, g ? 3 : 4>([&] { issue_step(t + 4, w2); }, [&] { read(t + 2); }, [&] { FQ8_MFMA16(2) });
+                pp_slot<g, g ? 6 : 4>([&] { issue_step(t + 5, w2); if (g == 1) issue_step(t + 6, w2); }, [&] { read(t + 3); }, [&] { FQ8_MFMA16(3) }, [&] { FQ8_MFMA8() });
+            } while (++u < nsup);
+            pp_group_end<g>();
+        };
+        if (grp == 0) run(std::integral_constant<int, 0>());
+        else run(std::integral_constant<int, 1>());
+#undef FQ8_MFMA16
+#undef FQ8_MFMA8
+#undef FQ8_MF
+#undef FQ8_LD
+#undef FQ8_CVT1
+#undef FQ8_ISSUE_W8
+        asm volatile("s_setreg_imm32_b32 hwreg(HW_REG_MODE, 23, 1), 0");
+        asm volatile("s_waitcnt vmcnt(0)" ::: "memory");
+        __builtin_amdgcn_s_barrier();
+
+        f32x2 ms_n; f32x4 c4_n; unsigned long long sw_n[3];
+        load_consts(m1, head_n, ms_n, c4_n, sw_n);
+
+        {
+            const KArgs none{};
+            auto emit = [&](auto FOLD) {
+                constexpr bool fold = FOLD.value;
+#pragma unroll
+                for (int j = 0; j < 6; ++j) {
+                    const int c = wc * 96 + j * 16 + fq * 4, which = c >> 6, d = c & 63;
+                    const f32x4 b4 = *(OFX_LDS const f32x4*)(cst + 128 + j * 16 + fq * 4);
+                    f32x4 cs4 = {0.f, 0.f, 0.f, 0.f};
+                    if (fold) cs4 = *(OFX_LDS const f32x4*)(cst + 224 + j * 16 + fq * 4);
+                    OFX_LDS char* reg = img + (which == 0 ? FQ_Q_OFF : which == 1 ? FQ_K_OFF : FQ_V_OFF);
+                    const int stride = which == 2 ? ATTN_V_ROW : FQ_QK_ROW;
+#pragma unroll
+                    for (int i = 0; i < 4; ++i) {
+                        const int row = wr * 64 + i * 16 + fr;
+                        float mu = 0.f, rs = 1.f;
+                        if (fold) { const f32x2 ms = *(OFX_LDS const f32x2*)(cst + 2 * (i * 16 + fr)); mu = ms[0]; rs = ms[1]; }
+                        const f32x4 v = epi_value(none, acc[i][j], OFX_ACT_NONE, fold, mu, rs, cs4, b4, false);
+                        v4 o;
+#pragma unroll
+                        for (int e = 0; e < 4; ++e) o[e] = (T)v[e];
+                        *(OFX_LDS v4*)(reg + row * stride + d * 2) = o;
+                    }
+                }
+            };
+            if (p.row_stat) emit(std::true_type());
+            else emit(std::false_type());
+        }
+        stash_consts(head_n, ms_n, c4_n, sw_n, sc_a, sc_b);
+        asm volatile("s_waitcnt lgkmcnt(0)" ::: "memory");
+        __builtin_amdgcn_s_barrier();
+
+        if (wave < n_live_img) fq_attention<T>(img, p, wave, ln, m0, head);
+        if (!has_next) break;
+        __builtin_amdgcn_s_barrier();
+        vb = vn; grp_t = grp_n; head = head_n;
+        first = false;
+    }
 }
 
+}
+
 int ofx_launch_fused_qkv_attn(const void* X, const void* Wqkv, const float* bias, const float* row_stat, const float* col_sum, void* out,
-                              int n_img, int S, int Wm, int heads, int ldx, int ldo, float scale, int op_dtype, hipStream_t s, bool w2) {
+                              int n_img, int S, int Wm, int heads, int ldx, int ldo, float scale, int op_dtype, hipStream_t s, FusedQkvForm form,
+                              const void* W8, const void* scale8) {
+    const bool w2 = form != FUSED_QKV_PLAIN, f8 = form == FUSED_QKV_W2F8;
     OFX_REQUIRE(X && Wqkv && bias && out && n_img > 0, OFX_EINVAL, "fused_qkv_attn: NULL argument");
+    OFX_REQUIRE(!f8 || (W8 && scale8), OFX_EINVAL, "fused_qkv_attn: the fp8 form needs W8 and scale8");
+    OFX_REQUIRE(!f8 || op_dtype == OFX_F16, OFX_EINVAL, "fused_qkv_attn: the fp8 form takes f16 operands");
     OFX_REQUIRE(S >= 33 && S <= 64 && Wm == heads * 64 && Wm % BK == 0 && Wm / BK >= 2, OFX_ESHAPE, "fused_qkv_attn: S=%d must be in [33,64], width %d = heads * 64", S, Wm);
+    OFX_REQUIRE(!f8 || Wm % 128 == 0, OFX_ESHAPE, "fused_qkv_attn: the fp8 form needs a width that is a multiple of 128, not %d", Wm);
+    OFX_REQUIRE(!f8 || ((size_t)FQ_TM * ldx * 2 < 0x7fffffff && (size_t)3 * Wm * Wm * 4 < 0x7fffffff), OFX_ESHAPE, "fused_qkv_attn: the fp8 form takes weights below 2 GiB");
     OFX_REQUIRE((FQ_TM / S - 1) * S + 64 - FQ_TM <= 16, OFX_ESHAPE, "fused_qkv_attn: S=%d would read %d key rows past the tile's 16 pad rows (supported: 33, 34, 37..41, 43..64)", S,
                 (FQ_TM / S - 1) * S + 64 - FQ_TM);
     OFX_REQUIRE(ldx >= Wm && ldx % 8 == 0 && ldo >= Wm && ldo % 8 == 0, OFX_ESHAPE, "fused_qkv_attn: bad strides");
@@ -276,6 +551,7 @@
     FusedK k;
     k.X = (const char*)X; k.Wqkv = (const char*)Wqkv; k.out = (char*)out; k.bias = bias; k.row_stat = row_stat; k.col_sum = col_sum;
     k.n_img = n_img; k.S = S; k.Wm = Wm; k.heads = heads; k.ldx = ldx; k.ldo = ldo; k.G = FQ_TM / S; k.scale = scale;
+    k.W8 = (const char*)W8; k.scale8 = (const char*)scale8;
     const int groups = (n_img + k.G - 1) / k.G;
     k.nwg = ((groups + 5) / 6) * 6 * heads;
     static DeviceOnce attr;
@@ -284,11 +560,15 @@
         OFX_HIP(hipFuncSetAttribute((const void*)fused_qkv_attn_kernel<f16_t, false>, hipFuncAttributeMaxDynamicSharedMemorySize, FQ_LDS));
         OFX_HIP(hipFuncSetAttribute((const void*)fused_qkv_attn_kernel<bf16_t, true>, hipFuncAttributeMaxDynamicSharedMemorySize, FQ2_LDS));
         OFX_HIP(hipFuncSetAttribute((const void*)fused_qkv_attn_kernel<f16_t, true>, hipFuncAttributeMaxDynamicSharedMemorySize, FQ2_LDS));
+        OFX_HIP(hipFuncSetAttribute((const void*)fused_qkv_attn_w2f8_kernel, hipFuncAttributeMaxDynamicSharedMemorySize, FQ8_LDS));
         return OFX_OK;
     }));
-    if (g_ofx_prof_on) ofx_prof_set_tag(n_img * S, 3 * Wm, Wm, 7, w2 ? 2 : 1, 2.0 * n_img * S * Wm + 2.0 * (w2 ? 2 : 1) * 3.0 * Wm * Wm + 2.0 * n_img * S * Wm);
-    ProfScope prof(PROF_GEMM, s, (w2 ? 2.0 : 1.0) * 2.0 * n_img * S * 3.0 * Wm * Wm + 4.0 * n_img * S * S * Wm, true);
-    if (w2) {
+    const double wbytes = f8 ? 3.0 : (w2 ? 4.0 : 2.0), products = f8 ? 1.5 : (w2 ? 2.0 : 1.0);
+    if (g_ofx_prof_on) ofx_prof_set_tag(n_img * S, 3 * Wm, Wm, 7, w2 ? 2 : 1, 2.0 * n_img * S * Wm + wbytes * 3.0 * Wm * Wm + 2.0 * n_img * S * Wm);
+    ProfScope prof(PROF_GEMM, s, products * 2.0 * n_img * S * 3.0 * Wm * Wm + 4.0 * n_img * S * S * Wm, true);
+    if (f8) {
+        OFX_PLAUNCH(true, fused_qkv_attn_w2f8_kernel, dim3(ofx_gemm_w2_grid(k.nwg)), dim3(512), FQ8_LDS, s, k);
+    } else if (w2) {
         if (op_dtype == OFX_F16) OFX_PLAUNCH(true, (fused_qkv_attn_kernel<f16_t, true>), dim3(k.nwg), dim3(512), FQ2_LDS, s, k);
         else OFX_PLAUNCH(true, (fused_qkv_attn_kernel<bf16_t, true>), dim3(k.nwg), dim3(512), FQ2_LDS, s, k);
     } else {
diff --git a/outfitx_amd/csrc/gemm.hip b/outfitx_amd/csrc/gemm.hip
--- a/outfitx_amd/csrc/gemm.hip
+++ b/outfitx_amd/csrc/gemm.hip
@@ -130,6 +130,19 @@
     }
 }
 size_t ofx_gemm_splitk_bytes(int M, int N, int K) { return gemm_splitk_slab_bytes(M, N, K, g_knobs); }
+
+static GemmShape gemm_shape(const GemmArgs& g, int op_dtype) {
+    const bool producer = g.xb_out || g.stat_part || g.xlo;
+    GemmShape sh;
+    sh.M = g.M; sh.N = g.N; sh.K = g.K; sh.lda = g.lda; sh.a_wrap = g.a_wrap; sh.k_mult = g.k_mult;
+    sh.f16 = op_dtype == OFX_F16; sh.has_w8 = g.W8 && g.w8_scale; sh.has_m_dev = g.m_dev != nullptr;
+    sh.can_split = g.slab && !producer && !g.row_stat; sh.defer = g.defer_splits != nullptr;
+    sh.ln_fusable = g.ln_gamma && g.out_kind == 0 && g.act == OFX_ACT_NONE && !g.aux_out && !g.drop.thresh;
+    sh.out_kind = g.out_kind; sh.resid = g.resid != nullptr; sh.aux = g.aux_out != nullptr; sh.xlo = g.xlo != nullptr;
+    return sh;
+}
+int ofx_gemm_plan_kind(const GemmArgs& g, int op_dtype) { return gemm_plan(gemm_shape(g, op_dtype), g_knobs, device_cu_count()).kind; }
+int ofx_gemm_w2_grid(int nwg) { return gemm_persistent_grid(nwg, g_knobs.w2_persist, false, device_cu_count()); }
 
 int ofx_launch_gemm(const GemmArgs& g, int op_dtype, hipStream_t s) {
     OFX_REQUIRE(g.M > 0 && g.N > 0 && g.K > 0, OFX_ESHAPE, "gemm: empty problem M=%d N=%d K=%d", g.M, g.N, g.K);
@@ -154,13 +167,7 @@
     OFX_REQUIRE(!(g.row_stat || producer) || !g.resid, OFX_EINVAL, "gemm: LayerNorm folding takes no residual (a producer's stream is (xb_out, xlo))");
     OFX_REQUIRE(!producer || g.act == OFX_ACT_NONE, OFX_EINVAL, "gemm: a LayerNorm-fold producer has no activation");
 
-    GemmShape sh;
-    sh.M = g.M; sh.N = g.N; sh.K = g.K; sh.lda = g.lda; sh.a_wrap = g.a_wrap; sh.k_mult = g.k_mult;
-    sh.f16 = op_dtype == OFX_F16; sh.has_w8 = g.W8 && g.w8_scale; sh.has_m_dev = g.m_dev != nullptr;
-    sh.can_split = g.slab && !producer && !g.row_stat; sh.defer = g.defer_splits != nullptr;
-    sh.ln_fusable = g.ln_gamma && g.out_kind == 0 && g.act == OFX_ACT_NONE && !g.aux_out && !g.drop.thresh;
-    sh.out_kind = g.out_kind; sh.resid = g.resid != nullptr; sh.aux = g.aux_out != nullptr; sh.xlo = g.xlo != nullptr;
-    const GemmPlan pl = gemm_plan(sh, g_knobs, device_cu_count());
+    const GemmPlan pl = gemm_plan(gemm_shape(g, op_dtype), g_knobs, device_cu_count());
     if (pl.splits > 1) OFX_REQUIRE(g.slab_bytes >= (size_t)pl.splits * g.M * g.N * 4, OFX_EWORKSPACE, "gemm: split-K slab too small");
 
     if (g_ofx_prof_on) ofx_prof_set_tag(g.M, g.N, pl.k_logical, pl.kind, pl.kmul, pl.bytes);
diff --git a/outfitx_amd/csrc/ofx_common.h b/outfitx_amd/csrc/ofx_common.h
--- a/outfitx_amd/csrc/ofx_common.h
+++ b/outfitx_amd/csrc/ofx_common.h
@@ -276,6 +276,8 @@
 int ofx_launch_gemm(const GemmArgs& g, int op_dtype , hipStream_t s);
 size_t ofx_gemm_splitk_bytes(int M, int N, int K);
 int ofx_gemm_tune(int knob, int value);
+int ofx_gemm_plan_kind(const GemmArgs& g, int op_dtype);
+int ofx_gemm_w2_grid(int nwg);
 
 struct LnArgs {
     const float* x;
@@ -365,8 +367,10 @@
     int splits = 1; size_t plane = 0; const float* bias = nullptr;
 };
 int ofx_launch_set_attention(const SetAttnArgs& a, int op_dtype, hipStream_t s);
+enum FusedQkvForm { FUSED_QKV_PLAIN = 0, FUSED_QKV_W2 = 1, FUSED_QKV_W2F8 = 2 };
 int ofx_launch_fused_qkv_attn(const void* X, const void* Wqkv, const float* bias, const float* row_stat, const float* col_sum, void* out,
-                              int n_img, int S, int Wm, int heads, int ldx, int ldo, float scale, int op_dtype, hipStream_t s, bool w2 = false);
+                              int n_img, int S, int Wm, int heads, int ldx, int ldo, float scale, int op_dtype, hipStream_t s, FusedQkvForm form = FUSED_QKV_PLAIN,
+                              const void* W8 = nullptr, const void* scale8 = nullptr);
 
 int ofx_launch_multi_copy(const void* table_host, int n, hipStream_t s);
 int ofx_launch_fill_f32(float* p, size_t n, float v, hipStream_t s);
```

Result: faster. 8231, median of 6 (+1.1%).
